# sweeneychris/TheiaSfM

Hardware: NVIDIA H100
Metric: observations/s = N_obs x LM iterations / solve time (10k-cam / 2M-pt / 20M-obs BA, ITERATIVE_SCHUR + SCHUR_JACOBI) (higher is better)
Workload: dtype f64

## Files before the change

### include/theia_ba_b200.h

```cpp
#ifndef THEIA_BA_B200_H_
#define THEIA_BA_B200_H_

#include <stdint.h>

#ifdef __cplusplus
extern "C" {
#endif

#define TBA_EXT_SIZE 6
#define TBA_INTR_STRIDE 10
#define TBA_PT_SIZE 4

enum { TBA_MODEL_PINHOLE = 0, TBA_MODEL_PINHOLE_RADIAL_TANGENTIAL = 1, TBA_MODEL_FISHEYE = 2, TBA_MODEL_FOV = 3,
       TBA_MODEL_DIVISION_UNDISTORTION = 4 };
#define TBA_MODEL_NUM_PARAMETERS(model) \
  ((model) == 0 ? 7 : (model) == 1 ? 10 : (model) == 2 ? 9 : ((model) == 3 || (model) == 4) ? 5 : -1)

enum { TBA_LOSS_TRIVIAL = 0, TBA_LOSS_HUBER = 1, TBA_LOSS_SOFTLONE = 2,
       TBA_LOSS_CAUCHY = 3, TBA_LOSS_ARCTAN = 4, TBA_LOSS_TUKEY = 5 };

enum { TBA_INTR_NONE = 0x00, TBA_INTR_FOCAL_LENGTH = 0x01,
       TBA_INTR_ASPECT_RATIO = 0x02, TBA_INTR_SKEW = 0x04,
       TBA_INTR_PRINCIPAL_POINTS = 0x08, TBA_INTR_RADIAL_DISTORTION = 0x10,
       TBA_INTR_TANGENTIAL_DISTORTION = 0x20, TBA_INTR_ALL = 0x3f };
// ... 101 lines not shown

int tba_device_count(void);

int tba_create(int device, int rank, int world_size, const void* nccl_unique_id,
               tba_context** out);
void tba_destroy(tba_context* ctx);
int tba_nccl_unique_id(void* out_128_bytes);
const char* tba_last_error(tba_context* ctx);

int tba_solve(tba_context* ctx, const tba_options* options,
              tba_problem* problem, tba_summary* summary);

int tba_solve_multi(const tba_options* options, tba_problem* problem, tba_summary* summary, int n_devices);

int tba_upload(tba_context* ctx, const tba_options* options, const tba_problem* problem);
int tba_minimize(tba_context* ctx, tba_summary* summary);
int tba_download(tba_context* ctx, tba_problem* problem);

int tba_filter_tracks(tba_context* ctx, double max_inlier_reprojection_error, double min_triangulation_angle_degrees,
                      uint8_t* status, double* mean_sq_error, int32_t* num_bad_reprojections, int32_t* num_insufficient_angles);

int tba_adjust_tracks(tba_context* ctx, const tba_options* options, uint8_t* status, double* initial_cost, double* final_cost,
                      int32_t* num_failed);
int tba_estimate_tracks(tba_context* ctx, const tba_options* ba_options, double max_acceptable_reprojection_error_pixels,
                        double min_triangulation_angle_degrees, int32_t bundle_adjustment, uint8_t* status, int32_t counts[5]);
enum { TBA_TRACK_ESTIMATED = 0, TBA_TRACK_BAD_ANGLE = 1, TBA_TRACK_TRIANGULATION_FAILED = 2, TBA_TRACK_BA_FAILED = 3,
       TBA_TRACK_BAD_REPROJECTION = 4, TBA_TRACK_SKIPPED = 255 };

int tba_adjust_views(tba_context* ctx, const tba_options* options, const int32_t* views, int32_t n_views, uint8_t* status,
                     double* initial_cost, double* final_cost, int32_t* iterations);

typedef struct tba_two_view_batch {
  int32_t n_pairs;
  const int64_t* pair_off;
  const double* ext1;
  double* ext2;
  double* intr1;
  double* intr2;
  const int32_t* model1;
  const int32_t* model2;
  const uint8_t* constant_intrinsics1;
  const uint8_t* constant_intrinsics2;
  const double* xy1;
  const double* xy2;
  double* points;
  double final_max_reprojection_error_pixels;
  uint8_t* inlier;
} tba_two_view_batch;
int tba_two_view_ba_batch(tba_context* ctx, tba_two_view_batch* batch, uint8_t* termination, double* initial_cost, double* final_cost,
                          int32_t* iterations);
int tba_two_view_ba_batch_multi(tba_two_view_batch* batch, int n_devices, uint8_t* termination, double* initial_cost, double* final_cost,
                                int32_t* iterations);

int tba_reset_parameters(tba_context* ctx, const tba_problem* problem);
int tba_set_max_iterations(tba_context* ctx, int32_t max_num_iterations);

int tba_set_profiling(tba_context* ctx, int enable);
int tba_get_profile(tba_context* ctx, double* out8);
int tba_get_profile_stages(tba_context* ctx, double* out16);

void tba_shard_points(const int32_t* pt_num_obs, int32_t n_pt, int world_size,
                      int rank, int32_t* begin, int32_t* end);

enum { TBA_VEC_GRADIENT_CAM = 0,
       TBA_VEC_GRADIENT_INTR = 1,
       TBA_VEC_GRADIENT_PT = 2,
       TBA_VEC_COLNORM2_CAM = 3,
       TBA_VEC_COLNORM2_INTR = 4,
       TBA_VEC_COLNORM2_PT = 5,
       TBA_VEC_RESIDUALS = 6,
       TBA_VEC_SCHUR_RHS_CAM = 7,
       TBA_VEC_SCHUR_RHS_INTR = 8,
       TBA_VEC_PRECOND_CAM = 9,
       TBA_VEC_PRECOND_INTR = 10,
       TBA_VEC_STEP_CAM = 11,
       TBA_VEC_STEP_INTR = 12,
       TBA_VEC_STEP_PT = 13 };
int tba_debug_pack(const tba_problem* problem, int64_t cap_slots, int64_t* sizes_out, int32_t* slot_cam, int32_t* slot_pt,
                   int16_t* slot_run, uint8_t* slot_flags, double* xy, int64_t* slot_orig, int32_t* pk2caller,
                   int32_t* tile_pt_begin, int32_t* tile_nruns, uint8_t* tile_flags, double* mask);
int tba_debug_linearize(tba_context* ctx, double* cost);
int tba_debug_linearize_raw(tba_context* ctx, int tile_kernel, int64_t* sizes_out, double* J, double* res, double* Hpp,
                            double* gp, double* lin);
int tba_debug_stream_launch(tba_context* ctx, int32_t* out);
int tba_debug_prepare_linear_system(tba_context* ctx, double radius);
int tba_debug_schur_matvec(tba_context* ctx, const double* x_cam ,
                           const double* x_intr ,
                           double* y_cam, double* y_intr);
int tba_debug_solve_linear_system(tba_context* ctx, int32_t* cg_iterations,
                                  double* model_cost_change);
int tba_debug_evaluate_step(tba_context* ctx, double* candidate_cost);
int tba_debug_read(tba_context* ctx, int which, double* out, int64_t n);

#ifdef __cplusplus
}
#endif
#endif
```

### theiasfm_b200/csrc/tba_camera_models.cuh

```cuda
#pragma once
#include <cstdint>
#include <cfloat>

#include "tba_camera_models_ext.cuh"

#ifdef __CUDA_ARCH__
#define TBA_UNROLL _Pragma("unroll")
#else
#define TBA_UNROLL
#endif

namespace tba {

constexpr int kModelPinhole = 0;
constexpr int kModelRadTan = 1;

constexpr int kCamRec = 20;

__host__ __device__ constexpr int popcount10(uint32_t m) {
  int n = 0;
  for (int i = 0; i < 10; ++i) n += (m >> i) & 1u;
  return n;
}
__host__ __device__ constexpr int nth_bit(uint32_t m, int j) {
// ... 33 lines not shown
  R[3] = B01 + Sw2;       R[4] = c + B * w1 * w1; R[5] = B12 - Sw0;
  R[6] = B02 - Sw1;       R[7] = B12 + Sw0;       R[8] = c + B * w2 * w2;
  const double th2 = w0 * w0 + w1 * w1 + w2 * w2;
  const double d = 1.0 - Cc * th2;
  const double Bw0 = B * w0, Bw1 = B * w1, Bw2 = B * w2;
  const double C01 = Cc * w0 * w1, C02 = Cc * w0 * w2, C12 = Cc * w1 * w2;
  L[0] = d + Cc * w0 * w0; L[1] = C01 - Bw2;        L[2] = C02 + Bw1;
  L[3] = C01 + Bw2;        L[4] = d + Cc * w1 * w1; L[5] = C12 - Bw0;
  L[6] = C02 - Bw1;        L[7] = C12 + Bw0;        L[8] = d + Cc * w2 * w2;
  rec[18] = B == 0.0 ? 1.0 : 0.0;
  rec[19] = 0.0;
}
__host__ __device__ inline void cam_prep(const double* __restrict__ w, double* __restrict__ rec, double* __restrict__ s4_out = nullptr) {
  double s4[4];
  cam_scalars(w, s4);
  cam_rec_expand(w[0], w[1], w[2], s4[0], s4[1], s4[2], s4[3], rec);
  if (s4_out) { s4_out[0] = s4[0]; s4_out[1] = s4[1]; s4_out[2] = s4[2]; s4_out[3] = s4[3]; }
}

__host__ __device__ inline void loss_evaluate(int type, double a, double s, double rho[3]) {
  switch (type) {
    case 1: {
      const double b = a * a;
      if (s > b) { const double r = sqrt(s); rho[0] = 2.0 * a * r - b; rho[1] = fmax(DBL_MIN, a / r); rho[2] = -rho[1] / (2.0 * s); }
      else { rho[0] = s; rho[1] = 1.0; rho[2] = 0.0; }
      break; }
    case 2: {
      const double b = a * a, c = 1.0 / b, sum = 1.0 + s * c, tmp = sqrt(sum);
      rho[0] = 2.0 * b * (tmp - 1.0); rho[1] = fmax(DBL_MIN, 1.0 / tmp); rho[2] = -(c * rho[1]) / (2.0 * sum);
      break; }
    case 3: {
      const double b = a * a, c = 1.0 / b, sum = 1.0 + s * c, inv = 1.0 / sum;
      rho[0] = b * log(sum); rho[1] = fmax(DBL_MIN, inv); rho[2] = -c * (inv * inv);
      break; }
    case 4: {
      const double b = 1.0 / (a * a), sum = 1.0 + s * s * b, inv = 1.0 / sum;
      rho[0] = a * atan2(s, a); rho[1] = fmax(DBL_MIN, inv); rho[2] = -2.0 * s * b * (inv * inv);
      break; }
    case 5: {
      const double a2 = a * a;
      if (s <= a2) { const double v = 1.0 - s / a2, v2 = v * v; rho[0] = a2 / 6.0 * (1.0 - v2 * v); rho[1] = 0.5 * v2; rho[2] = -1.0 / a2 * v; }
      else { rho[0] = a2 / 6.0; rho[1] = 0.0; rho[2] = 0.0; }
      break; }
    default: rho[0] = s; rho[1] = 1.0; rho[2] = 0.0;
  }
}

__host__ __device__ inline void project_pixel(int model, const double* __restrict__ C, const double* __restrict__ R,
                                     const double* __restrict__ k, const double X0, const double X1, const double X2, const double h,
                                     double& px, double& py, double& qz, double& a_sq) {
  const double a0 = X0 - h * C[0], a1 = X1 - h * C[1], a2 = X2 - h * C[2];
  a_sq = a0 * a0 + a1 * a1 + a2 * a2;
  const double q0 = R[0] * a0 + R[1] * a1 + R[2] * a2;
  const double q1 = R[3] * a0 + R[4] * a1 + R[5] * a2;
  const double q2 = R[6] * a0 + R[7] * a1 + R[8] * a2;
  qz = q2;
  const double u = q0 / q2, v = q1 / q2;
  const double r2 = u * u + v * v;
  double ud, vd;
  if (model == kModelPinhole) {
    const double d = 1.0 + r2 * (k[5] + k[6] * r2);
    ud = u * d; vd = v * d;
  } else {
    const double rd = 1.0 + k[5] * r2 + k[6] * r2 * r2 + k[7] * r2 * r2 * r2;
    const double tx = k[9] * (r2 + 2.0 * u * u) + 2.0 * k[8] * u * v;
    const double ty = k[8] * (r2 + 2.0 * v * v) + 2.0 * k[9] * u * v;
    ud = u * rd + tx; vd = v * rd + ty;
  }
  px = k[0] * ud + k[2] * vd + k[3];
  py = k[0] * k[1] * vd + k[4];
}

__host__ __device__ inline bool reproject(int model, const double* __restrict__ C, const double* __restrict__ R,
                                 const double* __restrict__ k, const double X0, const double X1, const double X2,
                                 const double h, const double x, const double y, double& r0, double& r1) {
  double px, py, qz, a_sq;
  project_pixel(model, C, R, k, X0, X1, X2, h, px, py, qz, a_sq);
  if (a_sq < 1e-8) return false;
  r0 = px - x;
  r1 = py - y;
  return true;
}

template <uint32_t IMASK>
__host__ __device__ inline bool linearize_obs(int model, const double* __restrict__ C, const double* __restrict__ rec,
                                     const double* __restrict__ k, const double X0, const double X1, const double X2,
                                     const double h, const double x, const double y, int loss_type, double loss_width,
                                     double r[2], double& rho0, double Ja[6], double Jw[6], double Jh[2], double* Ji) {
  constexpr int NI = popcount10(IMASK);
  const double* R = rec;
  const double* L = rec + 9;
  const bool small = rec[18] != 0.0;
  const double a0 = X0 - h * C[0], a1 = X1 - h * C[1], a2 = X2 - h * C[2];
  if (a0 * a0 + a1 * a1 + a2 * a2 < 1e-8) return false;
  const double q0 = R[0] * a0 + R[1] * a1 + R[2] * a2;
  const double q1 = R[3] * a0 + R[4] * a1 + R[5] * a2;
  const double q2 = R[6] * a0 + R[7] * a1 + R[8] * a2;
  const double iz = 1.0 / q2;
  const double u = q0 * iz, v = q1 * iz;
  const double r2 = u * u + v * v;
  double ud, vd, D00, D01, D10, D11;
  double dk[10][2];
  if (model == kModelPinhole) {
    const double d = 1.0 + r2 * (k[5] + k[6] * r2);
    const double dd = 2.0 * k[5] + 4.0 * k[6] * r2;
    ud = u * d; vd = v * d;
    D00 = d + u * u * dd; D01 = u * v * dd; D10 = D01; D11 = d + v * v * dd;
    dk[5][0] = r2 * u; dk[5][1] = r2 * v;
    dk[6][0] = r2 * r2 * u; dk[6][1] = r2 * r2 * v;
    dk[7][0] = dk[7][1] = dk[8][0] = dk[8][1] = dk[9][0] = dk[9][1] = 0.0;
  } else {
    const double r4 = r2 * r2;
    const double rd = 1.0 + k[5] * r2 + k[6] * r4 + k[7] * r4 * r2;
    const double rdp = k[5] + 2.0 * k[6] * r2 + 3.0 * k[7] * r4;
    const double t1 = k[8], t2 = k[9];
    ud = u * rd + t2 * (r2 + 2.0 * u * u) + 2.0 * t1 * u * v;
    vd = v * rd + t1 * (r2 + 2.0 * v * v) + 2.0 * t2 * u * v;
    D00 = rd + 2.0 * u * u * rdp + 6.0 * t2 * u + 2.0 * t1 * v;
    D01 = 2.0 * u * v * rdp + 2.0 * t2 * v + 2.0 * t1 * u;
    D10 = 2.0 * u * v * rdp + 2.0 * t1 * u + 2.0 * t2 * v;
    D11 = rd + 2.0 * v * v * rdp + 6.0 * t1 * v + 2.0 * t2 * u;
    dk[5][0] = r2 * u; dk[5][1] = r2 * v;
    dk[6][0] = r4 * u; dk[6][1] = r4 * v;
    dk[7][0] = r4 * r2 * u; dk[7][1] = r4 * r2 * v;
    dk[8][0] = 2.0 * u * v; dk[8][1] = r2 + 2.0 * v * v;
    dk[9][0] = r2 + 2.0 * u * u; dk[9][1] = 2.0 * u * v;
  }
  const double f = k[0], ar = k[1], sk = k[2];
  const double rr0 = f * ud + sk * vd + k[3] - x;
  const double rr1 = f * ar * vd + k[4] - y;
  const double s = rr0 * rr0 + rr1 * rr1;
  double rho[3];
  loss_evaluate(loss_type, loss_width, s, rho);
  rho0 = rho[0];
  const double sq = sqrt(rho[1]);
  double P00 = sq, P01 = 0.0, P10 = 0.0, P11 = sq, rscale = sq;
  if (!(s == 0.0 || rho[2] <= 0.0)) {
    const double Dd = 1.0 + 2.0 * s * rho[2] / rho[1];
    const double alpha = 1.0 - sqrt(Dd);
    rscale = sq / (1.0 - alpha);
    const double an = alpha / s;
    P00 = sq * (1.0 - an * rr0 * rr0); P01 = -sq * an * rr0 * rr1; P10 = P01; P11 = sq * (1.0 - an * rr1 * rr1);
  }
  r[0] = rr0 * rscale; r[1] = rr1 * rscale;
  const double K00 = f * D00 + sk * D10, K01 = f * D01 + sk * D11;
  const double K10 = f * ar * D10, K11 = f * ar * D11;
  const double A00 = P00 * K00 + P01 * K10, A01 = P00 * K01 + P01 * K11;
  const double A10 = P10 * K00 + P11 * K10, A11 = P10 * K01 + P11 * K11;
  const double Jq00 = A00 * iz, Jq01 = A01 * iz, Jq02 = -(A00 * u + A01 * v) * iz;
  const double Jq10 = A10 * iz, Jq11 = A11 * iz, Jq12 = -(A10 * u + A11 * v) * iz;
  Ja[0] = Jq00 * R[0] + Jq01 * R[3] + Jq02 * R[6];
  Ja[1] = Jq00 * R[1] + Jq01 * R[4] + Jq02 * R[7];
  Ja[2] = Jq00 * R[2] + Jq01 * R[5] + Jq02 * R[8];
  Ja[3] = Jq10 * R[0] + Jq11 * R[3] + Jq12 * R[6];
  Ja[4] = Jq10 * R[1] + Jq11 * R[4] + Jq12 * R[7];
  Ja[5] = Jq10 * R[2] + Jq11 * R[5] + Jq12 * R[8];
  Jh[0] = -(Ja[0] * C[0] + Ja[1] * C[1] + Ja[2] * C[2]);
  Jh[1] = -(Ja[3] * C[0] + Ja[4] * C[1] + Ja[5] * C[2]);
  const double b0 = small ? a0 : q0, b1 = small ? a1 : q1, b2 = small ? a2 : q2;
  const double c00 = Jq01 * b2 - Jq02 * b1, c01 = Jq02 * b0 - Jq00 * b2, c02 = Jq00 * b1 - Jq01 * b0;
  const double c10 = Jq11 * b2 - Jq12 * b1, c11 = Jq12 * b0 - Jq10 * b2, c12 = Jq10 * b1 - Jq11 * b0;
  Jw[0] = -(c00 * L[0] + c01 * L[3] + c02 * L[6]);
  Jw[1] = -(c00 * L[1] + c01 * L[4] + c02 * L[7]);
  Jw[2] = -(c00 * L[2] + c01 * L[5] + c02 * L[8]);
  Jw[3] = -(c10 * L[0] + c11 * L[3] + c12 * L[6]);
  Jw[4] = -(c10 * L[1] + c11 * L[4] + c12 * L[7]);
  Jw[5] = -(c10 * L[2] + c11 * L[5] + c12 * L[8]);
  if (NI > 0) {
    double col[10][2];
    col[0][0] = ud;  col[0][1] = ar * vd;
    col[1][0] = 0.0; col[1][1] = f * vd;
    col[2][0] = vd;  col[2][1] = 0.0;
    col[3][0] = 1.0; col[3][1] = 0.0;
    col[4][0] = 0.0; col[4][1] = 1.0;
    TBA_UNROLL
    for (int j = 5; j < 10; ++j) {
      col[j][0] = f * dk[j][0] + sk * dk[j][1];
      col[j][1] = f * ar * dk[j][1];
    }
    TBA_UNROLL
    for (int j = 0; j < NI; ++j) {
      constexpr uint32_t M = IMASK;
      const int idx = nth_bit(M, j);
      Ji[j] = P00 * col[idx][0] + P01 * col[idx][1];
      Ji[NI + j] = P10 * col[idx][0] + P11 * col[idx][1];
    }
  }
  return true;
}

__host__ __device__ inline void project_pixel_ext(int model, const double* __restrict__ C, const double* __restrict__ R,
                                                  const double* __restrict__ k, const double X0, const double X1, const double X2, const double h,
                                                  double& px, double& py, double& qz, double& a_sq) {
  const double a0 = X0 - h * C[0], a1 = X1 - h * C[1], a2 = X2 - h * C[2];
  a_sq = a0 * a0 + a1 * a1 + a2 * a2;
  double q[3], pix[2];
  q[0] = R[0] * a0 + R[1] * a1 + R[2] * a2;
  q[1] = R[3] * a0 + R[4] * a1 + R[5] * a2;
  q[2] = R[6] * a0 + R[7] * a1 + R[8] * a2;
  qz = q[2];
  camera_to_pixel_ext<double>(model, k, q, pix);
  px = pix[0]; py = pix[1];
}

template <uint32_t IMASK>
__host__ __device__ inline bool linearize_obs_ext(int model, const double* __restrict__ C, const double* __restrict__ rec,
                                                  const double* __restrict__ k, const double X0, const double X1, const double X2,
                                                  const double h, const double x, const double y, int loss_type, double loss_width,
                                                  double r[2], double& rho0, double Ja[6], double Jw[6], double Jh[2], double* Ji) {
  constexpr int NI = popcount10(IMASK);
  const double* R = rec;
  const double* L = rec + 9;
  const bool small = rec[18] != 0.0;
  const double a0 = X0 - h * C[0], a1 = X1 - h * C[1], a2 = X2 - h * C[2];
  if (a0 * a0 + a1 * a1 + a2 * a2 < 1e-8) return false;
  const double q0 = R[0] * a0 + R[1] * a1 + R[2] * a2;
  const double q1 = R[3] * a0 + R[4] * a1 + R[5] * a2;
  const double q2 = R[6] * a0 + R[7] * a1 + R[8] * a2;
  typedef Dual<13> D;
  D qd[3], kd[10], pix[2];
  const double qv[3] = {q0, q1, q2};
  for (int i = 0; i < 3; ++i) { qd[i].v = qv[i]; for (int j = 0; j < 13; ++j) qd[i].d[j] = 0.0; qd[i].d[i] = 1.0; }
  const int K = model_num_parameters(model);
  for (int i = 0; i < 10; ++i) { kd[i].v = i < K ? k[i] : 0.0; for (int j = 0; j < 13; ++j) kd[i].d[j] = 0.0; if (i < K) kd[i].d[3 + i] = 1.0; }
  camera_to_pixel_ext<D>(model, kd, qd, pix);
  const double rr0 = pix[0].v - x, rr1 = pix[1].v - y;
  const double s = rr0 * rr0 + rr1 * rr1;
  double rho[3];
  loss_evaluate(loss_type, loss_width, s, rho);
  rho0 = rho[0];
  const double sq = sqrt(rho[1]);
  double P00 = sq, P01 = 0.0, P10 = 0.0, P11 = sq, rscale = sq;
  if (!(s == 0.0 || rho[2] <= 0.0)) {
    const double Dd = 1.0 + 2.0 * s * rho[2] / rho[1];
    const double alpha = 1.0 - sqrt(Dd);
    rscale = sq / (1.0 - alpha);
    const double an = alpha / s;
    P00 = sq * (1.0 - an * rr0 * rr0); P01 = -sq * an * rr0 * rr1; P10 = P01; P11 = sq * (1.0 - an * rr1 * rr1);
  }
  r[0] = rr0 * rscale; r[1] = rr1 * rscale;
  const double Jq00 = P00 * pix[0].d[0] + P01 * pix[1].d[0], Jq01 = P00 * pix[0].d[1] + P01 * pix[1].d[1], Jq02 = P00 * pix[0].d[2] + P01 * pix[1].d[2];
  const double Jq10 = P10 * pix[0].d[0] + P11 * pix[1].d[0], Jq11 = P10 * pix[0].d[1] + P11 * pix[1].d[1], Jq12 = P10 * pix[0].d[2] + P11 * pix[1].d[2];
  Ja[0] = Jq00 * R[0] + Jq01 * R[3] + Jq02 * R[6];
  Ja[1] = Jq00 * R[1] + Jq01 * R[4] + Jq02 * R[7];
  Ja[2] = Jq00 * R[2] + Jq01 * R[5] + Jq02 * R[8];
  Ja[3] = Jq10 * R[0] + Jq11 * R[3] + Jq12 * R[6];
  Ja[4] = Jq10 * R[1] + Jq11 * R[4] + Jq12 * R[7];
  Ja[5] = Jq10 * R[2] + Jq11 * R[5] + Jq12 * R[8];
  Jh[0] = -(Ja[0] * C[0] + Ja[1] * C[1] + Ja[2] * C[2]);
  Jh[1] = -(Ja[3] * C[0] + Ja[4] * C[1] + Ja[5] * C[2]);
  const double b0 = small ? a0 : q0, b1 = small ? a1 : q1, b2 = small ? a2 : q2;
  const double c00 = Jq01 * b2 - Jq02 * b1, c01 = Jq02 * b0 - Jq00 * b2, c02 = Jq00 * b1 - Jq01 * b0;
  const double c10 = Jq11 * b2 - Jq12 * b1, c11 = Jq12 * b0 - Jq10 * b2, c12 = Jq10 * b1 - Jq11 * b0;
  Jw[0] = -(c00 * L[0] + c01 * L[3] + c02 * L[6]);
  Jw[1] = -(c00 * L[1] + c01 * L[4] + c02 * L[7]);
  Jw[2] = -(c00 * L[2] + c01 * L[5] + c02 * L[8]);
  Jw[3] = -(c10 * L[0] + c11 * L[3] + c12 * L[6]);
  Jw[4] = -(c10 * L[1] + c11 * L[4] + c12 * L[7]);
  Jw[5] = -(c10 * L[2] + c11 * L[5] + c12 * L[8]);
  if (NI > 0) {
    TBA_UNROLL
    for (int j = 0; j < NI; ++j) {
      constexpr uint32_t M = IMASK;
      const int idx = nth_bit(M, j);
      Ji[j] = P00 * pix[0].d[3 + idx] + P01 * pix[1].d[3 + idx];
      Ji[NI + j] = P10 * pix[0].d[3 + idx] + P11 * pix[1].d[3 + idx];
    }
  }
  return true;
}

template <bool EXT>
__host__ __device__ inline void project_pixel_any(int model, const double* __restrict__ C, const double* __restrict__ R,
                                                  const double* __restrict__ k, const double X0, const double X1, const double X2, const double h,
                                                  double& px, double& py, double& qz, double& a_sq) {
  if (EXT) {
    if (model >= kModelFisheye) { project_pixel_ext(model, C, R, k, X0, X1, X2, h, px, py, qz, a_sq); return; }
  }
  project_pixel(model, C, R, k, X0, X1, X2, h, px, py, qz, a_sq);
}
template <bool EXT>
__host__ __device__ inline bool reproject_any(int model, const double* __restrict__ C, const double* __restrict__ R,
                                              const double* __restrict__ k, const double X0, const double X1, const double X2,
                                              const double h, const double x, const double y, double& r0, double& r1) {
  if (EXT) {
    if (model >= kModelFisheye) {
      double px, py, qz, a_sq;
      project_pixel_ext(model, C, R, k, X0, X1, X2, h, px, py, qz, a_sq);
      if (a_sq < 1e-8) return false;
      r0 = px - x; r1 = py - y;
      return true;
    }
  }
  return reproject(model, C, R, k, X0, X1, X2, h, x, y, r0, r1);
}
template <uint32_t IMASK, bool EXT>
__host__ __device__ inline bool linearize_obs_any(int model, const double* __restrict__ C, const double* __restrict__ rec,
                                                  const double* __restrict__ k, const double X0, const double X1, const double X2,
                                                  const double h, const double x, const double y, int loss_type, double loss_width,
                                                  double r[2], double& rho0, double Ja[6], double Jw[6], double Jh[2], double* Ji) {
  if (EXT) {
    if (model >= kModelFisheye) return linearize_obs_ext<IMASK>(model, C, rec, k, X0, X1, X2, h, x, y, loss_type, loss_width, r, rho0, Ja, Jw, Jh, Ji);
  }
  return linearize_obs<IMASK>(model, C, rec, k, X0, X1, X2, h, x, y, loss_type, loss_width, r, rho0, Ja, Jw, Jh, Ji);
}

}
```

### theiasfm_b200/csrc/tba_engine.cu

```cuda
#include <dlfcn.h>
#include <nccl.h>
#include <unistd.h>

#include <algorithm>
#include <chrono>
#include <condition_variable>
#include <cmath>
#include <cstdarg>
#include <cstdio>
#include <cstdlib>
#include <cstring>
#include <atomic>
#include <mutex>
#include <thread>
#include <string>
#include <vector>

#include "../../include/theia_ba_b200.h"
#include "tba_kernels.cuh"
#include "tba_pack.h"
#include "tba_block_lm.h"

namespace tba {

// ... 131 lines not shown
  PcgState* h_st = nullptr;
};

namespace {

void set_err(tba_context* c, const char* fmt, ...) {
  char buf[512];
  va_list ap;
  va_start(ap, fmt);
  vsnprintf(buf, sizeof buf, fmt, ap);
  va_end(ap);
  c->err = buf;
}

#define CUDA_OK(c, expr)                                                                        \
  do {                                                                                          \
    cudaError_t e__ = (expr);                                                                   \
    if (e__ != cudaSuccess) {                                                                   \
      set_err(c, "CUDA error %s at %s:%d (%s)", cudaGetErrorString(e__), __FILE__, __LINE__, #expr); \
      return TBA_ERR_CUDA;                                                                      \
    }                                                                                           \
  } while (0)

#define NCCL_OK(c, expr)                                                                        \
  do {                                                                                          \
    ncclResult_t r__ = (expr);                                                                  \
    if (r__ != ncclSuccess) {                                                                   \
      set_err(c, "NCCL error %s at %s:%d", g_nccl.GetErrorString(r__), __FILE__, __LINE__);     \
      return TBA_ERR_NCCL;                                                                      \
    }                                                                                           \
  } while (0)

#ifdef TBA_EMULATE
#define LAUNCH(c, kern, grid, block, smem, ...)                                              \
  do {                                                                                       \
    if ((unsigned)(grid) == 0u) break;                             \
    emu::launch((const void*)(kern), (unsigned)(grid), (unsigned)(block), (size_t)(smem), [&] { kern(__VA_ARGS__); }); \
    if (cudaGetLastError() != cudaSuccess) {                                                 \
      set_err(c, "kernel launch failed: invalid configuration at %s:%d (%s)", __FILE__, __LINE__, #kern); \
      return TBA_ERR_CUDA;                                                                   \
    }                                                                                        \
    (c)->launches++;                                                                         \
  } while (0)
#else
#define LAUNCH(c, kern, grid, block, smem, ...)                                                              \
  do {                                                                                                       \
    if ((unsigned)(grid) == 0u) break;  \
    kern<<<(grid), (block), (smem), (c)->stream>>>(__VA_ARGS__);                                             \
    const cudaError_t le__ = cudaPeekAtLastError();                                                          \
    if (le__ != cudaSuccess) {                                                                               \
      set_err(c, "kernel launch failed: %s at %s:%d (%s)", cudaGetErrorString(le__), __FILE__, __LINE__, #kern); \
      return TBA_ERR_CUDA;                                                                                   \
    }                                                                                                        \
    (c)->launches++;                                                                                         \
  } while (0)
#endif

int prof_begin(tba_context* c) {
  if (!c->profiling) return -1;
  cudaEvent_t e;
  if (cudaEventCreate(&e) != cudaSuccess) return -1;
  c->ev_pool.push_back(e);
  cudaEventRecord(e, c->stream);
  return (int)c->ev_pool.size() - 1;
}
void prof_end(tba_context* c, int which, int begin) {
  if (begin < 0) return;
  cudaEvent_t e;
  if (cudaEventCreate(&e) != cudaSuccess) return;
  c->ev_pool.push_back(e);
  cudaEventRecord(e, c->stream);
  c->ev_spans[which].push_back({begin, (int)c->ev_pool.size() - 1});
}

const uint32_t kMasks[] = {0x000u, 0x001u, 0x061u, 0x0E1u, 0x07Fu, 0x3FFu};

#define DISPATCH_IMASK(mask, F) \
  switch (mask) {               \
    case 0x000u: F(0x000u); break; \
    case 0x001u: F(0x001u); break; \
    case 0x061u: F(0x061u); break; \
    case 0x0E1u: F(0x0E1u); break; \
    case 0x07Fu: F(0x07Fu); break; \
    default: F(0x3FFu); break;  \
  }

int allreduce_sum(tba_context* c, double* buf, size_t n) {
  if (c->world == 1) return TBA_OK;
  NCCL_OK(c, g_nccl.AllReduce(buf, buf, n, ncclDouble, ncclSum, c->comm, c->stream));
  return TBA_OK;
}
size_t schur_smem(const tba_context* c) { return (size_t)(c->NJ + 2) * TILE * sizeof(double); }

double* lin_g(tba_context* c) { return c->lin.p; }
double* lin_cn(tba_context* c) { return c->lin.p + c->P.ncs; }
double* lin_scal(tba_context* c) { return c->lin.p + 2 * (size_t)c->P.ncs; }
int small_grid(const tba_context* c, int64_t n_items) { return (int)std::max<int64_t>(1, std::min<int64_t>((n_items + 255) / 256, (int64_t)c->n_sm * 8)); }
int stream_grid(const tba_context* c, int n_slices, int NW) { return std::max(1, std::min(c->n_sm, (n_slices + NW - 1) / NW)); }

int read_scal(tba_context* c, const double* dev, int n, double* out) {
  CUDA_OK(c, cudaMemcpyAsync(c->h_scal, dev, n * sizeof(double), cudaMemcpyDeviceToHost, c->stream));
  CUDA_OK(c, cudaStreamSynchronize(c->stream));
  memcpy(out, c->h_scal, n * sizeof(double));
  return TBA_OK;
}

int stage_linearize(tba_context* c, double* cost, double* fixed, bool* ok, double* gmax = nullptr, bool tile_kernel = false) {
  DevProblem& P = c->P;
  const size_t n_lin = 2 * (size_t)P.ncs + 16 + (size_t)c->world;
  CUDA_OK(c, cudaMemsetAsync(c->lin.p, 0, n_lin * sizeof(double), c->stream));
  LAUNCH(c, k_cam_prep, (P.n_cam + 127) / 128, 128, 0, P.n_cam, P.ext, P.cam_rec, P.cam_s4);
  if (P.n_tiles > 0) {
    const int pb = prof_begin(c);
    if (c->has_ext_models) {
      auto kfn = k_linearize<0x3FFu, true>;
      LAUNCH(c, kfn, P.n_tiles, TILE, 0, P, lin_g(c), lin_cn(c), c->rep.p, 0);
    } else {
      int first_tile = 0;
      if (c->n_normal_tiles > 0 && !tile_kernel) {
        const int n_slices = c->n_normal_tiles * (TILE / 32);
#define F(M) { using Cfg = LinCfg<M>; auto kfn = k_linearize_stream<M>; \
               const int grid = stream_grid(c, n_slices, Cfg::NW); \
               LAUNCH(c, kfn, grid, Cfg::NW * 32, Cfg::SMEM, P, lin_g(c), lin_cn(c), c->rep.p, n_slices); }
        DISPATCH_IMASK(c->imask, F)
#undef F
        first_tile = c->n_normal_tiles;
      }
      const int rest = P.n_tiles - first_tile;
#define F(M) { auto kfn = k_linearize<M, false>; LAUNCH(c, kfn, rest, TILE, 0, P, lin_g(c), lin_cn(c), c->rep.p, first_tile); }
      DISPATCH_IMASK(c->imask, F)
#undef F
    }
    prof_end(c, 1, pb);
    LAUNCH(c, k_fold, 1, REPW, 0, c->rep.p, lin_g(c) + P.ne, lin_cn(c) + P.ne, lin_scal(c));
  }
  if (gmax && P.n_pt > 0) LAUNCH(c, k_gradmax_pt, small_grid(c, P.n_pt), 256, 0, P, lin_scal(c) + 16 + c->rank);
  int rc = allreduce_sum(c, c->lin.p, n_lin);
  if (rc) return rc;
  if (gmax) LAUNCH(c, k_gradmax_cs, VB, VT, 0, P.ncs, lin_g(c), c->mask.p, lin_scal(c) + 16, c->world, lin_scal(c) + 3);
  if (!c->have_scale) {
    LAUNCH(c, k_cs_scale, VB, VT, 0, P.ncs, lin_cn(c), c->mask.p, c->opt.jacobi_scaling, c->sm.p);
    if (P.n_pt > 0) LAUNCH(c, k_point_scale, (P.n_pt + 255) / 256, 256, 0, P, c->opt.jacobi_scaling);
    c->have_scale = true;
  }
  double s[4];
  rc = read_scal(c, lin_scal(c), 4, s);
  if (rc) return rc;
  *cost = s[0]; *fixed = s[1]; *ok = s[2] == 0.0;
  if (gmax) *gmax = s[3];
  return TBA_OK;
}

void p2p_release(tba_context* c) {
#ifndef TBA_EMULATE
  for (void* q : c->p2p_opened) cudaIpcCloseMemHandle(q);
#endif
  c->p2p_opened.clear();
  if (c->p2p_inbox) cudaFree(c->p2p_inbox);
  if (c->p2p_flags) cudaFree(c->p2p_flags);
  if (c->p2p_ctr) cudaFree(c->p2p_ctr);
  c->p2p_inbox = nullptr; c->p2p_flags = nullptr; c->p2p_ctr = nullptr; c->p2p_cap = 0; c->p2p_ok = false;
}

#ifndef TBA_EMULATE
struct P2pInfo {
  long long pid;
// ... 601 lines not shown
  c->opt = *options;
  if (options->linear_solver_type != TBA_ITERATIVE_SCHUR) {
    c->opt.eta = 1e-13;
    c->opt.min_linear_solver_iterations = 0;
    c->opt.max_linear_solver_iterations = std::max(c->opt.max_linear_solver_iterations, 2000);
    c->opt.preconditioner_type = TBA_PRECOND_SCHUR_JACOBI;
  }
  const int nc = p->n_cam, ng = p->n_group, np = p->n_pt;
  const int64_t no = p->n_obs;
  if (nc < 0 || ng < 0 || np < 0 || no < 0) { set_err(c, "negative sizes"); return TBA_ERR_INVALID_ARGUMENT; }
  c->has_ext_models = false;
  for (int g = 0; g < ng; ++g) {
    if (TBA_MODEL_NUM_PARAMETERS(p->group_model[g]) < 0) {
      set_err(c, "camera intrinsics model %d of group %d is not a CameraIntrinsicsModelType (0..4)", p->group_model[g], g);
      return TBA_ERR_UNSUPPORTED;
    }
    if (p->group_model[g] >= TBA_MODEL_FISHEYE) c->has_ext_models = true;
  }
  for (int i = 0; i < nc; ++i) if (p->cam_group[i] < 0 || p->cam_group[i] >= ng) { set_err(c, "cam_group out of range"); return TBA_ERR_INVALID_ARGUMENT; }
  const int T = std::max(1, std::min<int>(64, (int)std::thread::hardware_concurrency() / std::max(1, c->world)));
  HostPack& H = c->pack;
  c->slot_orig.clear();
  const bool trace = getenv("TBA_UPLOAD_TRACE") != nullptr;
  auto t_prev = std::chrono::steady_clock::now();
  auto lap = [&](const char* what) {
    if (!trace) return;
    auto t = std::chrono::steady_clock::now();
    fprintf(stderr, "[tba_upload r%d] %-28s %8.2f ms\n", c->rank, what, std::chrono::duration<double, std::milli>(t - t_prev).count());
    t_prev = t;
  };
  pack_count_and_sort(p, T, &H);
  lap("count_and_sort (A-C)");
  int local_err = TBA_OK;
  if (H.bad >= 0) { set_err(c, "observation %lld references camera %d / point %d out of range", (long long)H.bad, p->obs_cam[H.bad], p->obs_pt[H.bad]); local_err = TBA_ERR_INVALID_ARGUMENT; }
  else if (H.maxlen > TILE) { set_err(c, "track with %d observations exceeds the engine limit of %d per track", H.maxlen, TILE); local_err = TBA_ERR_UNSUPPORTED; }
  const bool collective_upload = c->world > 1 && c->preset_cnt_cam == nullptr;
  if (local_err != TBA_OK && !collective_upload) return local_err;
  if (local_err == TBA_OK) pack_points(p, &H);
  lap("pack_points");
  std::vector<double> cnt_c(nc, 0.0), cnt_g(ng, 0.0);
  if (local_err == TBA_OK) for (int i = 0; i < nc; ++i) { cnt_c[i] = H.cnt_cam[i]; cnt_g[p->cam_group[i]] += H.cnt_cam[i]; }
  c->n_free_pt = local_err == TBA_OK ? H.n_free_pt : 0;
  c->n_free_pt_global = c->n_free_pt;
  if (c->world > 1 && c->preset_cnt_cam != nullptr) {
    std::fill(cnt_g.begin(), cnt_g.end(), 0.0);
    for (int i = 0; i < nc; ++i) { cnt_c[i] = c->preset_cnt_cam[i]; cnt_g[p->cam_group[i]] += cnt_c[i]; }
    c->n_free_pt_global = c->preset_free_pt;
  } else if (c->world > 1) {
    std::vector<double> tmp(cnt_c);
    tmp.insert(tmp.end(), cnt_g.begin(), cnt_g.end());
    tmp.push_back((double)c->n_free_pt);
    tmp.push_back(local_err != TBA_OK ? 1.0 : 0.0);
    rc = [&]() -> int {
      CUDA_OK(c, c->scal2.alloc(std::max<size_t>(tmp.size(), 16)));
      CUDA_OK(c, cudaMemcpyAsync(c->scal2.p, tmp.data(), tmp.size() * 8, cudaMemcpyHostToDevice, c->stream));
      int r2 = allreduce_sum(c, c->scal2.p, tmp.size());
      if (r2) return r2;
      CUDA_OK(c, cudaMemcpyAsync(tmp.data(), c->scal2.p, tmp.size() * 8, cudaMemcpyDeviceToHost, c->stream));
      CUDA_OK(c, cudaStreamSynchronize(c->stream));
      return TBA_OK;
    }();
    if (rc) return rc;
    if (tmp.back() != 0.0) {
      if (local_err == TBA_OK) { set_err(c, "upload failed on %d other rank(s) (invalid observation indices or over-long track in their shard)", (int)tmp.back()); return TBA_ERR_INVALID_ARGUMENT; }
      return local_err;
    }
    std::copy(tmp.begin(), tmp.begin() + nc, cnt_c.begin());
    std::copy(tmp.begin() + nc, tmp.begin() + nc + ng, cnt_g.begin());
    c->n_free_pt_global = (int64_t)tmp[tmp.size() - 2];
  }
  pack_masks_and_tiles(p, cnt_c, cnt_g, &H);
  lap("masks_and_tiles (D)");
  const int ne = nc * 6, ncs = ne + ng * 10;
  const std::vector<double>& mask = H.mask;
  const std::vector<double>& blk_free = H.blk_free;
  std::vector<int>& tile_pt_begin = H.tile_pt_begin;
  std::vector<int>& tile_nruns = H.tile_nruns;
  std::vector<uint8_t>& tile_flags = H.tile_flags;
  c->n_free_cs = H.n_free_cs;
  c->imask = 0x3FFu;
  for (uint32_t m : kMasks) if ((H.union_free & ~m) == 0) { c->imask = m; break; }
  if (c->has_ext_models) c->imask = 0x3FFu;
  c->NI = popcount10(c->imask);
  c->NJ = 14 + 2 * c->NI;
  const int npk = (int)H.pk2caller.size();
  const int n_long = H.n_long;
  const int n_tiles = H.n_tiles;
  const int64_t n_slots = H.n_slots;
  const size_t stage_bytes = (size_t)n_slots * (4 + 4 + 2 + 1 + 16) + (size_t)npk * (32 + 1 + 8 + 4) + 10 * 256;
  if (c->stage_cap < stage_bytes) {
    if (c->stage) cudaFreeHost(c->stage);
    c->stage = nullptr; c->stage_cap = 0;
    CUDA_OK(c, cudaMallocHost(&c->stage, stage_bytes + stage_bytes / 8));
    c->stage_cap = stage_bytes + stage_bytes / 8;
  }
  uint8_t* sp8 = (uint8_t*)c->stage;
  auto carve = [&](size_t bytes) { uint8_t* r0 = sp8; sp8 += (bytes + 255) / 256 * 256; return r0; };
  double* h_xy = (double*)carve((size_t)n_slots * 16);
  double* h_pt = (double*)carve((size_t)npk * 32);
  int* h_slot_cam = (int*)carve((size_t)n_slots * 4);
  int* h_slot_pt = (int*)carve((size_t)n_slots * 4);
  int16_t* h_slot_run = (int16_t*)carve((size_t)n_slots * 2);
  uint8_t* h_slot_flags = carve((size_t)n_slots);
  uint8_t* h_pt_const = carve((size_t)npk);
  long long* h_pt_slot = (long long*)carve((size_t)npk * 8);
  int* h_pt_len = (int*)carve((size_t)npk * 4);
  lap("staging");
  PackDest d;
  d.xy = h_xy; d.pt = h_pt; d.slot_cam = h_slot_cam; d.slot_pt = h_slot_pt; d.slot_run = h_slot_run; d.slot_flags = h_slot_flags;
  d.pt_const = h_pt_const; d.slot_orig = nullptr;
  c->n_long_points = n_long;
  c->n_cam = nc; c->n_group = ng; c->n_pt = npk; c->n_pt_caller = np; c->n_tiles = n_tiles; c->n_obs = no; c->n_slots = n_slots;
  const int npd = npk;
  c->h2d_bytes = 0; c->d2h_bytes = 0; c->launches = 0;
#define ALLOC(buf, n) CUDA_OK(c, c->buf.alloc(n))
  ALLOC(ext, (size_t)ne); ALLOC(ext_c, (size_t)ne); ALLOC(intr, (size_t)ng * 10); ALLOC(intr_c, (size_t)ng * 10);
  ALLOC(pt, (size_t)npd * 4); ALLOC(pt_c, (size_t)npd * 4); ALLOC(cam_rec, (size_t)nc * kCamRec); ALLOC(cam_rec_c, (size_t)nc * kCamRec); ALLOC(cam_s4, (size_t)nc * 4); ALLOC(cam_s4_c, (size_t)nc * 4);
  ALLOC(xy, (size_t)n_slots * 2); ALLOC(J, (size_t)n_slots * c->NJ); ALLOC(res, (size_t)n_slots * 2);
  ALLOC(Hpp, (size_t)npd * 10); ALLOC(gp, (size_t)npd * 4); ALLOC(Mp, (size_t)npd * 10); ALLOC(sp, (size_t)npd * 4); ALLOC(dpt, (size_t)npd * 4);
  ALLOC(cam_group, (size_t)nc); ALLOC(group_model, (size_t)ng); ALLOC(slot_cam, (size_t)n_slots); ALLOC(slot_pt, (size_t)n_slots);
  ALLOC(tile_pt_begin, (size_t)n_tiles + 1); ALLOC(tile_nruns, (size_t)n_tiles); ALLOC(slot_flags, (size_t)n_slots);
  ALLOC(slot_run, (size_t)n_slots); ALLOC(pt_const, (size_t)npd); ALLOC(tile_flags, (size_t)n_tiles);
  ALLOC(pt_slot, (size_t)npd); ALLOC(pt_len, (size_t)npd); ALLOC(pt_stat, (size_t)npd);
  ALLOC(lin, 2 * (size_t)ncs + 16 + (size_t)std::max(1, c->world)); ALLOC(mask, (size_t)ncs); ALLOC(blk_free, (size_t)nc + ng); ALLOC(sm, (size_t)ncs); ALLOC(D2, (size_t)ncs);
  ALLOC(Sblk, (size_t)nc * 21 + (size_t)ng * 55 + 2 + (size_t)ncs); ALLOC(Minv_c, (size_t)nc * 36); ALLOC(Minv_i, (size_t)ng * 100);
  ALLOC(b, (size_t)ncs); ALLOC(x, (size_t)ncs); ALLOC(r, (size_t)ncs); ALLOC(p, (size_t)ncs); ALLOC(z, (size_t)ncs); ALLOC(z2, (size_t)ncs); ALLOC(xs, (size_t)ncs); ALLOC(y, (size_t)ncs);
  ALLOC(part, 3 * VB); ALLOC(gmax, 2); ALLOC(flag, 1); ALLOC(scal2, std::max<size_t>(16, (size_t)nc + ng)); ALLOC(st, 2); ALLOC(done_flag, 1); ALLOC(pcg_bar, 2); ALLOC(rep, (size_t)NREP * REPW);
#undef ALLOC
  lap("device alloc");
#define H2D(buf, src, n)                                                                                      \
  do {                                                                                                        \
    CUDA_OK(c, cudaMemcpyAsync(c->buf.p, (src), (n) * sizeof(*c->buf.p), cudaMemcpyHostToDevice, c->stream)); \
    c->h2d_bytes += (double)((n) * sizeof(*c->buf.p));                                                        \
  } while (0)
  H2D(ext, p->ext, (size_t)ne); H2D(intr, p->intr, (size_t)ng * 10);
  H2D(ext_c, p->ext, (size_t)ne); H2D(intr_c, p->intr, (size_t)ng * 10);
  H2D(cam_group, p->cam_group, (size_t)nc); H2D(group_model, p->group_model, (size_t)ng);
  H2D(tile_pt_begin, tile_pt_begin.data(), (size_t)n_tiles + 1); H2D(tile_nruns, tile_nruns.data(), (size_t)n_tiles);
  H2D(tile_flags, tile_flags.data(), (size_t)n_tiles);
  CUDA_OK(c, cudaMemsetAsync(c->rep.p, 0, (size_t)NREP * REPW * sizeof(double), c->stream));
  CUDA_OK(c, cudaMemsetAsync(c->pcg_bar.p, 0, 2 * sizeof(int), c->stream));
  CUDA_OK(c, cudaMemsetAsync(c->J.p, 0, (size_t)n_slots * c->NJ * sizeof(double), c->stream));
  CUDA_OK(c, cudaMemsetAsync(c->dpt.p, 0, (size_t)npd * 4 * sizeof(double), c->stream));
  CUDA_OK(c, cudaMemsetAsync(c->Mp.p, 0, (size_t)npd * 10 * sizeof(double), c->stream));
  CUDA_OK(c, cudaMemsetAsync(c->Hpp.p, 0, (size_t)npd * 10 * sizeof(double), c->stream));
  CUDA_OK(c, cudaMemsetAsync(c->gp.p, 0, (size_t)npd * 4 * sizeof(double), c->stream));
  CUDA_OK(c, cudaMemsetAsync(c->Minv_c.p, 0, (size_t)nc * 36 * sizeof(double), c->stream));
  CUDA_OK(c, cudaMemsetAsync(c->Minv_i.p, 0, (size_t)ng * 100 * sizeof(double), c->stream));
  {
    int n_chunks = n_tiles >= 32768 ? 16 : n_tiles >= 8192 ? 8 : 1;
    if (const char* e = getenv("TBA_UPLOAD_CHUNKS")) n_chunks = std::max(1, std::min(atoi(e), std::max(1, n_tiles)));
#define H2D_RANGE(buf, src, off, n)                                                                                              \
  do {                                                                                                                           \
    if ((n) > 0) {                                                                                                               \
      CUDA_OK(c, cudaMemcpyAsync(c->buf.p + (off), (src) + (off), (n) * sizeof(*c->buf.p), cudaMemcpyHostToDevice, c->stream));  \
      c->h2d_bytes += (double)((n) * sizeof(*c->buf.p));                                                                         \
    }                                                                                                                            \
  } while (0)
    for (int ch = 0; ch < n_chunks; ++ch) {
      const int64_t t0 = (int64_t)n_tiles * ch / n_chunks, t1 = (int64_t)n_tiles * (ch + 1) / n_chunks;
      if (t1 <= t0) continue;
      pack_fill(p, H, T, d, t0, t1);
      const size_t s0 = (size_t)t0 * TILE, ns = (size_t)(t1 - t0) * TILE;
      const size_t q0 = (size_t)tile_pt_begin[t0], nq = (size_t)tile_pt_begin[t1] - q0;
      H2D_RANGE(slot_cam, h_slot_cam, s0, ns); H2D_RANGE(slot_pt, h_slot_pt, s0, ns);
      H2D_RANGE(slot_flags, h_slot_flags, s0, ns); H2D_RANGE(slot_run, h_slot_run, s0, ns);
      H2D_RANGE(xy, h_xy, s0 * 2, ns * 2);
// ... 750 lines not shown
    });
  for (auto& t : th) t.join();
  for (int r = 0; r < n_devices; ++r)
    if (sh[r].rc != TBA_OK) { *summary = sh[r].s; summary->iterations = itbuf; summary->iterations_capacity = itcap; return sh[r].rc; }
  memcpy(problem->ext, sh[0].ext.data(), (size_t)problem->n_cam * 48);
  memcpy(problem->intr, sh[0].intr.data(), (size_t)problem->n_group * 80);
  for (int r = 0; r < n_devices; ++r) memcpy(problem->pt + (size_t)sh[r].b * 4, sh[r].pt.data(), (size_t)(sh[r].e - sh[r].b) * 32);
  *summary = sh[0].s;
  for (int r = 1; r < n_devices; ++r) {
    summary->num_kernel_launches += sh[r].s.num_kernel_launches;
    summary->h2d_bytes += sh[r].s.h2d_bytes;
    summary->d2h_bytes += sh[r].s.d2h_bytes;
    summary->setup_time_in_seconds = std::max(summary->setup_time_in_seconds, sh[r].s.setup_time_in_seconds);
    summary->solve_time_in_seconds = std::max(summary->solve_time_in_seconds, sh[r].s.solve_time_in_seconds);
  }
  return TBA_OK;
}

int tba_debug_pack(const tba_problem* p, int64_t cap_slots, int64_t* sizes_out, int32_t* slot_cam, int32_t* slot_pt, int16_t* slot_run,
                   uint8_t* slot_flags, double* xy, int64_t* slot_orig, int32_t* pk2caller, int32_t* tile_pt_begin,
                   int32_t* tile_nruns, uint8_t* tile_flags, double* mask) {
  if (!p || !sizes_out) return TBA_ERR_INVALID_ARGUMENT;
  for (int i = 0; i < p->n_cam; ++i) if (p->cam_group[i] < 0 || p->cam_group[i] >= p->n_group) return TBA_ERR_INVALID_ARGUMENT;
  static std::mutex mu;
  static HostPack H;
  std::lock_guard<std::mutex> lk(mu);
  pack_count_and_sort(p, 4, &H);
  if (H.bad >= 0) return TBA_ERR_INVALID_ARGUMENT;
  if (H.maxlen > TILE) return TBA_ERR_UNSUPPORTED;
  pack_points(p, &H);
  std::vector<double> cnt_c(p->n_cam, 0.0), cnt_g(p->n_group, 0.0);
  for (int i = 0; i < p->n_cam; ++i) { cnt_c[i] = H.cnt_cam[i]; cnt_g[p->cam_group[i]] += H.cnt_cam[i]; }
  pack_masks_and_tiles(p, cnt_c, cnt_g, &H);
  uint32_t imask = 0x3FFu;
  for (uint32_t m : kMasks) if ((H.union_free & ~m) == 0) { imask = m; break; }
  sizes_out[0] = H.n_tiles; sizes_out[1] = H.n_slots; sizes_out[2] = (int64_t)H.pk2caller.size(); sizes_out[3] = H.n_long;
  sizes_out[4] = popcount10(imask); sizes_out[5] = imask;
  if (H.n_slots > cap_slots) return TBA_ERR_INVALID_ARGUMENT;
  std::vector<double> pt((size_t)H.pk2caller.size() * 4);
  std::vector<uint8_t> ptc(H.pk2caller.size());
  for (int64_t s = 0; s < H.n_slots; ++s) slot_orig[s] = -1;
  PackDest d;
  d.xy = xy; d.pt = pt.data(); d.slot_cam = slot_cam; d.slot_pt = slot_pt; d.slot_run = slot_run; d.slot_flags = slot_flags;
  d.pt_const = ptc.data(); d.slot_orig = slot_orig;
  pack_fill(p, H, 4, d);
  for (size_t k = 0; k < H.pk2caller.size(); ++k) pk2caller[k] = H.pk2caller[k];
  for (int t = 0; t <= H.n_tiles; ++t) tile_pt_begin[t] = H.tile_pt_begin[t];
  for (int t = 0; t < H.n_tiles; ++t) { tile_nruns[t] = H.tile_nruns[t]; tile_flags[t] = H.tile_flags[t]; }
  for (size_t i = 0; i < H.mask.size(); ++i) mask[i] = H.mask[i];
  return TBA_OK;
}

int tba_debug_linearize(tba_context* c, double* cost) {
  if (!c || !c->uploaded) return TBA_ERR_INVALID_ARGUMENT;
  CUDA_OK(c, cudaSetDevice(c->device));
  bool ok;
  double x, f;
  int rc = stage_linearize(c, &x, &f, &ok);
  if (rc) return rc;
  c->x_cost = x; c->fixed_cost = f;
  if (cost) *cost = x + f;
  return ok ? TBA_OK : TBA_ERR_INVALID_ARGUMENT;
}

int tba_debug_linearize_raw(tba_context* c, int tile_kernel, int64_t* sizes_out, double* J, double* res, double* Hpp, double* gp, double* lin) {
  if (!c || !c->uploaded || !sizes_out) return TBA_ERR_INVALID_ARGUMENT;
  CUDA_OK(c, cudaSetDevice(c->device));
  const DevProblem& P = c->P;
  sizes_out[0] = c->n_slots; sizes_out[1] = c->NJ; sizes_out[2] = P.n_pt; sizes_out[3] = P.ncs;
  if (!J || !res || !Hpp || !gp || !lin) return TBA_OK;
  bool ok;
  double x, f;
  const int rc = stage_linearize(c, &x, &f, &ok, nullptr, tile_kernel != 0);
  if (rc) return rc;
  CUDA_OK(c, cudaMemcpyAsync(J, P.J, (size_t)c->n_slots * c->NJ * 8, cudaMemcpyDeviceToHost, c->stream));
  CUDA_OK(c, cudaMemcpyAsync(res, P.res, (size_t)c->n_slots * 2 * 8, cudaMemcpyDeviceToHost, c->stream));
  CUDA_OK(c, cudaMemcpyAsync(Hpp, P.Hpp, (size_t)P.n_pt * 10 * 8, cudaMemcpyDeviceToHost, c->stream));
  CUDA_OK(c, cudaMemcpyAsync(gp, P.gp, (size_t)P.n_pt * 4 * 8, cudaMemcpyDeviceToHost, c->stream));
  CUDA_OK(c, cudaMemcpyAsync(lin, c->lin.p, (2 * (size_t)P.ncs + 3) * 8, cudaMemcpyDeviceToHost, c->stream));
  CUDA_OK(c, cudaStreamSynchronize(c->stream));
  return TBA_OK;
}

int tba_debug_stream_launch(tba_context* c, int32_t* out) {
  if (!c || !c->uploaded || !out) return TBA_ERR_INVALID_ARGUMENT;
  const int n_slices = c->n_normal_tiles * (TILE / 32);
  out[0] = c->n_sm; out[1] = n_slices; out[2] = (int32_t)c->imask; out[3] = c->has_ext_models ? 1 : 0;
  auto put = [&](int k, int NW, int NS) { out[4 + 3 * k] = stream_grid(c, n_slices, NW); out[5 + 3 * k] = NW; out[6 + 3 * k] = NS; };
#define F(M) { put(0, LinCfg<M>::NW, LinCfg<M>::NS); put(1, PrepCfg<M>::NW, PrepCfg<M>::NS); \
               put(2, StreamCfg<M, 0>::NW, StreamCfg<M, 0>::NS); put(3, StreamCfg<M, 1>::NW, StreamCfg<M, 1>::NS); }
  DISPATCH_IMASK(c->imask, F)
#undef F
  return TBA_OK;
}

int tba_debug_prepare_linear_system(tba_context* c, double radius) {
  if (!c || !c->uploaded) return TBA_ERR_INVALID_ARGUMENT;
  CUDA_OK(c, cudaSetDevice(c->device));
  bool ok;
  int rc = stage_prepare(c, radius, &ok);
  if (rc) return rc;
  return ok ? TBA_OK : TBA_ERR_INVALID_ARGUMENT;
}

int tba_debug_schur_matvec(tba_context* c, const double* x_cam, const double* x_intr, double* y_cam, double* y_intr) {
  if (!c || !c->uploaded) return TBA_ERR_INVALID_ARGUMENT;
  CUDA_OK(c, cudaSetDevice(c->device));
  DevProblem& P = c->P;
  CUDA_OK(c, cudaMemcpyAsync(c->p.p, x_cam, (size_t)P.ne * 8, cudaMemcpyHostToDevice, c->stream));
  CUDA_OK(c, cudaMemcpyAsync(c->p.p + P.ne, x_intr, (size_t)P.n_group * 10 * 8, cudaMemcpyHostToDevice, c->stream));
  LAUNCH(c, k_cs_mul, VB, VT, 0, P.ncs, c->sm.p, c->p.p, c->xs.p);
  CUDA_OK(c, cudaMemsetAsync(c->y.p, 0, (size_t)P.ncs * 8, c->stream));
  LAUNCH(c, k_set_flag, 1, 1, 0, c->done_flag.p, 0);
  int rc = launch_matvec(c, c->done_flag.p);
  if (rc) return rc;
  LAUNCH(c, k_set_flag, 1, 1, 0, const_cast<int*>(st_done(c->st.p)), 0);
  PcgVectors V = pcg_vectors(c);
  V.fold_rep = nullptr;
  int cur = 0;
  rc = launch_pcg(c, V, cur, PCG_A, 0, p2p_none());
  if (rc) return rc;
  CUDA_OK(c, cudaMemcpyAsync(y_cam, c->z.p, (size_t)P.ne * 8, cudaMemcpyDeviceToHost, c->stream));
  CUDA_OK(c, cudaMemcpyAsync(y_intr, c->z.p + P.ne, (size_t)P.n_group * 10 * 8, cudaMemcpyDeviceToHost, c->stream));
  CUDA_OK(c, cudaStreamSynchronize(c->stream));
  return TBA_OK;
}

int tba_debug_solve_linear_system(tba_context* c, int32_t* cg_iterations, double* model_cost_change) {
  if (!c || !c->uploaded) return TBA_ERR_INVALID_ARGUMENT;
  CUDA_OK(c, cudaSetDevice(c->device));
  int iters = 0, status = 0;
  int rc = stage_pcg(c, &iters, &status);
  if (rc) return rc;
  rc = stage_backsub(c);
  if (rc) return rc;
  int r2 = allreduce_sum(c, c->scal2.p + 3, 1);
  if (r2) return r2;
  double s[8];
  rc = read_scal(c, c->scal2.p, 8, s);
  if (rc) return rc;
  if (cg_iterations) *cg_iterations = iters;
  if (model_cost_change) *model_cost_change = s[3];
  return status == 2 ? TBA_ERR_INVALID_ARGUMENT : TBA_OK;
}

int tba_debug_evaluate_step(tba_context* c, double* candidate_cost) {
  if (!c || !c->uploaded) return TBA_ERR_INVALID_ARGUMENT;
  CUDA_OK(c, cudaSetDevice(c->device));
  DevProblem& P = c->P;
  CUDA_OK(c, cudaMemsetAsync(c->scal2.p, 0, 3 * sizeof(double), c->stream));
  LAUNCH(c, k_cam_prep, (P.n_cam + 127) / 128, 128, 0, P.n_cam, P.ext_c, P.cam_rec_c, P.cam_s4_c);
  if (P.n_tiles > 0) {
    if (c->has_ext_models) { auto kfn = k_cost<true>; LAUNCH(c, kfn, P.n_tiles, TILE, 0, P, P.ext_c, P.cam_s4_c, P.intr_c, P.pt_c, c->rep.p); }
    else { auto kfn = k_cost<false>; LAUNCH(c, kfn, P.n_tiles, TILE, 0, P, P.ext_c, P.cam_s4_c, P.intr_c, P.pt_c, c->rep.p); }
    LAUNCH(c, k_fold, 1, REPW, 0, c->rep.p, nullptr, nullptr, c->scal2.p);
  }
  int rc = allreduce_sum(c, c->scal2.p, 3);
  if (rc) return rc;
  double s[3];
  rc = read_scal(c, c->scal2.p, 3, s);
  if (rc) return rc;
  if (candidate_cost) *candidate_cost = s[0] + s[1];
  return s[2] == 0.0 ? TBA_OK : TBA_ERR_INVALID_ARGUMENT;
}

int tba_debug_read(tba_context* c, int which, double* out, int64_t n) {
  if (!c || !c->uploaded || !out) return TBA_ERR_INVALID_ARGUMENT;
  CUDA_OK(c, cudaSetDevice(c->device));
  DevProblem& P = c->P;
  const int64_t ne = P.ne, ni = (int64_t)P.n_group * 10, np4 = (int64_t)P.n_pt * 4;
// ... 63 lines not shown
```

### theiasfm_b200/csrc/tba_kernels.cuh

```cuda
#pragma once
#include <cstdint>
#include <cuda_runtime.h>

#include "tba_camera_models.cuh"
#include "tba_segments.h"
#include "tba_filter.cuh"
#include "tba_track_estimator.cuh"
#include "tba_two_view.cuh"
#include "tba_view_ba.cuh"

namespace tba {

constexpr int TILE = 256;
constexpr int MAXP = 256;
constexpr int VB = 64;
constexpr int VT = 256;

struct DevProblem {
  int n_cam, n_group, n_pt, n_tiles;
  int ne;
  int ncs;
  int single_group;
  int loss_type; double loss_width;
  int ablate;
  double *ext, *intr, *pt, *ext_c, *intr_c, *pt_c;
  const int* cam_group; const int* group_model;
  double* cam_rec;
  double* cam_rec_c;
  double* cam_s4;
  double* cam_s4_c;
  const int* slot_cam;
  const int* slot_pt;
  const uint8_t* slot_flags;
  const int16_t* slot_run;
  const int* tile_pt_begin;
  const int* tile_nruns;
  const uint8_t* tile_flags;
  const double* xy;
  double* J;
  double* res;
  double* Hpp;
  double* gp;
  double* Mp;
  double* sp;
  double* dpt;
  const uint8_t* pt_const;
};

__device__ __forceinline__ double warp_sum(double v) {
#pragma unroll
  for (int o = 16; o > 0; o >>= 1) v += __shfl_down_sync(0xffffffffu, v, o);
  return v;
}

__device__ __forceinline__ double block_sum(double v, double* s_red ) {
  const int lane = threadIdx.x & 31, wid = threadIdx.x >> 5;
  v = warp_sum(v);
  __syncthreads();
  if (lane == 0) s_red[wid] = v;
  __syncthreads();
  double t = 0.0;
  if (wid == 0) {
    t = lane < (blockDim.x >> 5) ? s_red[lane] : 0.0;
    t = warp_sum(t);
  }
  return t;
}

__device__ __forceinline__ double seg_reduce(double v, int key, int lane) {
#pragma unroll
  for (int o = 1; o < 32; o <<= 1) {
    const double ov = __shfl_down_sync(0xffffffffu, v, o);
    const int ok = __shfl_down_sync(0xffffffffu, key, o);
    if (lane + o < 32 && ok == key) v += ov;
  }
  return v;
}

__device__ __forceinline__ double seg_reduce_to(double v, int run_last, int lane) {
#pragma unroll
  for (int o = 1; o < 32; o <<= 1) {
    const double ov = __shfl_down_sync(0xffffffffu, v, o);
    if (lane + o <= run_last) v += ov;
  }
  return v;
}

__device__ __forceinline__ void red_add(double* p, double v) {
#ifdef TBA_EMULATE
  atomicAdd(p, v);
#else
  asm volatile("red.global.add.f64 [%0], %1;" ::"l"(p), "d"(v) : "memory");
#endif
}

template <int N>
__device__ __forceinline__ void warp_stage_row(double* __restrict__ stage, int* __restrict__ sbase, const double (&v)[N], int base, int lane) {
#pragma unroll
  for (int j = 0; j < N; ++j) stage[lane * N + j] = v[j];
  sbase[lane] = base;
}
template <int N>
__device__ __forceinline__ void warp_red_rows(double* __restrict__ dst, const double* __restrict__ stage, const int* __restrict__ sbase, int lane) {
#pragma unroll
  for (int k = 0; k < N; ++k) {
    const int e = k * 32 + lane;
    const int o = e / N;
    const int b = sbase[o];
    if (b >= 0) red_add(dst + (size_t)b + (e - o * N), stage[e]);
  }
}

__global__ void k_cam_prep(int n_cam, const double* __restrict__ ext, double* __restrict__ rec, double* __restrict__ s4 = nullptr) {
  const int c = blockIdx.x * blockDim.x + threadIdx.x;
  if (c < n_cam) cam_prep(ext + (size_t)c * 6 + 3, rec + (size_t)c * kCamRec, s4 ? s4 + (size_t)c * 4 : nullptr);
}
__device__ __forceinline__ void gather_camera(const double* __restrict__ ext, const double* __restrict__ s4, int cam, double Cw[6], double rec[kCamRec]) {
  const double2* e2 = reinterpret_cast<const double2*>(ext + (size_t)cam * 6);
  const double2 e0 = __ldg(e2), e1 = __ldg(e2 + 1), e3 = __ldg(e2 + 2);
  const double2* q2 = reinterpret_cast<const double2*>(s4 + (size_t)cam * 4);
  const double2 q0 = __ldg(q2), q1 = __ldg(q2 + 1);
  Cw[0] = e0.x; Cw[1] = e0.y; Cw[2] = e1.x; Cw[3] = e1.y; Cw[4] = e3.x; Cw[5] = e3.y;
  cam_rec_expand(e1.y, e3.x, e3.y, q0.x, q0.y, q1.x, q1.y, rec);
}

constexpr int NREP = 256;
constexpr int REPW = 32;
__device__ __forceinline__ double* rep_row(double* rep) {
  return rep + (size_t)((blockIdx.x * (TILE / 32) + (threadIdx.x >> 5)) & (NREP - 1)) * REPW;
}
__global__ void k_fold(double* __restrict__ rep, double* __restrict__ dst_a, double* __restrict__ dst_b, double* __restrict__ dst_s) {
  const int j = threadIdx.x;
  if (j >= REPW) return;
  double v = 0.0;
  for (int r = 0; r < NREP; ++r) { v += rep[(size_t)r * REPW + j]; rep[(size_t)r * REPW + j] = 0.0; }
  if (j < 10) { if (dst_a) dst_a[j] += v; }
  else if (j < 20) { if (dst_b) dst_b[j - 10] += v; }
  else if (j < 24) { if (dst_s) dst_s[j - 20] += v; }
}

__device__ __forceinline__ int run_head_lane(unsigned heads, int lane) { return 31 - __clz(heads & (0xffffffffu >> (31 - lane))); }

__device__ __forceinline__ size_t wslice(int tile, int warp, int rows) { return ((size_t)tile * (TILE / 32) + warp) * rows * 32; }

__device__ __forceinline__ void sym4_mul(const double* __restrict__ M, const double t[4], double u[4]) {
  u[0] = M[0] * t[0] + M[1] * t[1] + M[2] * t[2] + M[3] * t[3];
  u[1] = M[1] * t[0] + M[4] * t[1] + M[5] * t[2] + M[6] * t[3];
  u[2] = M[2] * t[0] + M[5] * t[1] + M[7] * t[2] + M[8] * t[3];
  u[3] = M[3] * t[0] + M[6] * t[1] + M[8] * t[2] + M[9] * t[3];
}


template <int NI, int SP, int SC>
__device__ __forceinline__ void obs_apply_F(const double* ja, const double* jw, const double* ji, double h, double2 xa, double2 xb,
                                            double2 xc, const double* xi, double& w0, double& w1) {
  w0 = -h * (ja[0] * xa.x + ja[SP] * xa.y + ja[2 * SP] * xb.x) + jw[0] * xb.y + jw[SC] * xc.x + jw[2 * SC] * xc.y;
  w1 = -h * (ja[3 * SP] * xa.x + ja[4 * SP] * xa.y + ja[5 * SP] * xb.x) + jw[3 * SC] * xb.y + jw[4 * SC] * xc.x + jw[5 * SC] * xc.y;
#pragma unroll
  for (int j = 0; j < NI; ++j) { w0 += ji[j * SC] * xi[j]; w1 += ji[(NI + j) * SC] * xi[j]; }
}
template <int SP>
__device__ __forceinline__ void obs_JpT(const double* ja, const double* jh, double w0, double w1, double t[4]) {
  t[0] = ja[0] * w0 + ja[3 * SP] * w1; t[1] = ja[SP] * w0 + ja[4 * SP] * w1; t[2] = ja[2 * SP] * w0 + ja[5 * SP] * w1;
  t[3] = jh[0] * w0 + jh[SP] * w1;
}
template <int SP>
__device__ __forceinline__ void obs_sub_Jp(const double* ja, const double* jh, double w0, double w1, const double u[4], double& z0, double& z1) {
  z0 = w0 - (ja[0] * u[0] + ja[SP] * u[1] + ja[2 * SP] * u[2] + jh[0] * u[3]);
  z1 = w1 - (ja[3 * SP] * u[0] + ja[4 * SP] * u[1] + ja[5 * SP] * u[2] + jh[SP] * u[3]);
}
template <int SP, int SC>
__device__ __forceinline__ void obs_JcT(const double* ja, const double* jw, double h, double z0, double z1, double y[6]) {
#pragma unroll
  for (int j = 0; j < 3; ++j) y[j] = -h * (ja[j * SP] * z0 + ja[(3 + j) * SP] * z1);
#pragma unroll
  for (int j = 0; j < 3; ++j) y[3 + j] = jw[j * SC] * z0 + jw[(3 + j) * SC] * z1;
}
template <int NI, int SC>
__device__ __forceinline__ void obs_JiT(const double* ji, double z0, double z1, double y[]) {
#pragma unroll
  for (int j = 0; j < NI; ++j) y[j] = ji[j * SC] * z0 + ji[(NI + j) * SC] * z1;
}
__device__ __forceinline__ double obs_model_cost_change(double r0, double r1, double z0, double z1) {
  const double m0 = -(r0 - z0), m1 = -(r1 - z1);
  return -(m0 * (r0 + 0.5 * m0) + m1 * (r1 + 0.5 * m1));
}
__device__ __forceinline__ void obs_cam_block(const double* __restrict__ M, const double ja[6], const double jh[2], const double jw[6], double h,
                                              double v[21]) {
  const double jp0[4] = {ja[0], ja[1], ja[2], jh[0]}, jp1[4] = {ja[3], ja[4], ja[5], jh[1]};
  double m0[4], m1[4];
  sym4_mul(M, jp0, m0);
  sym4_mul(M, jp1, m1);
  const double q00 = 1.0 - (jp0[0] * m0[0] + jp0[1] * m0[1] + jp0[2] * m0[2] + jp0[3] * m0[3]);
  const double q01 = -(jp0[0] * m1[0] + jp0[1] * m1[1] + jp0[2] * m1[2] + jp0[3] * m1[3]);
  const double q11 = 1.0 - (jp1[0] * m1[0] + jp1[1] * m1[1] + jp1[2] * m1[2] + jp1[3] * m1[3]);
  double c0[6], c1[6];
#pragma unroll
  for (int j = 0; j < 3; ++j) { c0[j] = -h * ja[j]; c1[j] = -h * ja[3 + j]; c0[3 + j] = jw[j]; c1[3 + j] = jw[3 + j]; }
  int n = 0;
#pragma unroll
  for (int a = 0; a < 6; ++a) {
    const double qa0 = q00 * c0[a] + q01 * c1[a], qa1 = q01 * c0[a] + q11 * c1[a];
#pragma unroll
    for (int b = a; b < 6; ++b) { v[n] = qa0 * c0[b] + qa1 * c1[b]; ++n; }
  }
}
template <int NI>
__device__ __forceinline__ void obs_JiT_Ji(const double* ji, double g[]) {
  int n = 0;
#pragma unroll
  for (int a = 0; a < NI; ++a)
#pragma unroll
    for (int b = a; b < NI; ++b) { g[n] = ji[a] * ji[b] + ji[NI + a] * ji[NI + b]; ++n; }
}
template <int NI>
__device__ __forceinline__ void run_WT_M_W(const double* __restrict__ M, const double* W, double sub[]) {
  double MW[4][NI + 1];
#pragma unroll
  for (int j = 0; j < NI; ++j) {
    const double t[4] = {W[0 * NI + j], W[1 * NI + j], W[2 * NI + j], W[3 * NI + j]};
    double u[4];
    sym4_mul(M, t, u);
    MW[0][j] = u[0]; MW[1][j] = u[1]; MW[2][j] = u[2]; MW[3][j] = u[3];
  }
  int n = 0;
#pragma unroll
  for (int a = 0; a < NI; ++a)
#pragma unroll
    for (int b = a; b < NI; ++b) {
      sub[n] = W[0 * NI + a] * MW[0][b] + W[1 * NI + a] * MW[1][b] + W[2 * NI + a] * MW[2][b] + W[3 * NI + a] * MW[3][b];
      ++n;
    }
}
__device__ __forceinline__ int tri10(int ia, int ib) { return ia * 10 - ia * (ia - 1) / 2 + (ib - ia); }

template <int NI>
__device__ __forceinline__ void obs_settle(bool ok, bool is_fixed, double rho0, double& cost, double& fixed, double& failed, double Ja[6],
                                           double Jw[6], double Jh[2], double Ji[], double r[2]) {
  if (!ok) failed += 1.0;
  else if (is_fixed) fixed += 0.5 * rho0;
  else cost += 0.5 * rho0;
  if (!ok || is_fixed) {
#pragma unroll
    for (int j = 0; j < 6; ++j) { Ja[j] = 0.0; Jw[j] = 0.0; }
    Jh[0] = Jh[1] = 0.0; r[0] = r[1] = 0.0;
#pragma unroll
    for (int j = 0; j < 2 * NI; ++j) Ji[j] = 0.0;
  }
}
template <int NI>
__device__ __forceinline__ void obs_store(double* Jt, double* rt, const double Ja[6], const double Jw[6], const double Jh[2], const double Ji[],
                                          const double r[2]) {
#pragma unroll
  for (int j = 0; j < 6; ++j) Jt[j * 32] = Ja[j];
#pragma unroll
  for (int j = 0; j < 6; ++j) Jt[(6 + j) * 32] = Jw[j];
  Jt[12 * 32] = Jh[0];
  Jt[13 * 32] = Jh[1];
#pragma unroll
  for (int j = 0; j < 2 * NI; ++j) Jt[(14 + j) * 32] = Ji[j];
  rt[0] = r[0];
  rt[32] = r[1];
}
__device__ __forceinline__ void obs_point_terms(const double Ja[6], const double Jh[2], const double r[2], double acc[14]) {
  const double jp0[4] = {Ja[0], Ja[1], Ja[2], Jh[0]}, jp1[4] = {Ja[3], Ja[4], Ja[5], Jh[1]};
  int n = 0;
#pragma unroll
  for (int a = 0; a < 4; ++a)
#pragma unroll
    for (int b = a; b < 4; ++b) acc[n++] = jp0[a] * jp0[b] + jp1[a] * jp1[b];
#pragma unroll
  for (int a = 0; a < 4; ++a) acc[10 + a] = jp0[a] * r[0] + jp1[a] * r[1];
}
__device__ __forceinline__ void obs_cam_grad(const double Ja[6], const double Jw[6], double h, const double r[2], double g[6], double cn[6]) {
#pragma unroll
  for (int j = 0; j < 3; ++j) {
    const double c0 = -h * Ja[j], c1 = -h * Ja[3 + j];
    g[j] = c0 * r[0] + c1 * r[1];
    cn[j] = c0 * c0 + c1 * c1;
    g[3 + j] = Jw[j] * r[0] + Jw[3 + j] * r[1];
    cn[3 + j] = Jw[j] * Jw[j] + Jw[3 + j] * Jw[3 + j];
  }
}
template <int NI>
__device__ __forceinline__ void obs_intr_grad(const double Ji[], const double r[2], int j, double& g, double& cn) {
  g = Ji[j] * r[0] + Ji[NI + j] * r[1];
  cn = Ji[j] * Ji[j] + Ji[NI + j] * Ji[NI + j];
}

template <uint32_t IMASK, bool EXT = false>
__global__ void __launch_bounds__(TILE, EXT ? 1 : 3) k_linearize(DevProblem P, double* __restrict__ g_cs, double* __restrict__ cn_cs,
                                                           double* __restrict__ rep, int tile0) {
  constexpr bool STAGED_RED = !EXT;
  constexpr int NI = popcount10(IMASK);
  constexpr int NJ = 14 + 2 * NI;
  __shared__ double s_acc[MAXP][14];
  const int tile = tile0 + blockIdx.x, tid = threadIdx.x, lane = tid & 31, warp = tid >> 5;
  const bool long_tile = (P.tile_flags[tile] & 1) != 0;
  const int p0 = P.tile_pt_begin[tile], npt = P.tile_pt_begin[tile + 1] - p0;
  if (long_tile) {
    for (int i = tid; i < npt * 14; i += TILE) (&s_acc[0][0])[i] = 0.0;
    __syncthreads();
  }
  const size_t slot = (size_t)tile * TILE + tid;
  const int cam = P.slot_cam[slot];
  const bool valid = cam >= 0;
  double cost = 0.0, fixed = 0.0, failed = 0.0;
  double Ja[6] = {0, 0, 0, 0, 0, 0}, Jw[6] = {0, 0, 0, 0, 0, 0}, Jh[2] = {0, 0}, r[2] = {0, 0};
  double Ji[2 * NI + 1];
#pragma unroll
  for (int j = 0; j < 2 * NI; ++j) Ji[j] = 0.0;
  int pl = -1 - lane, grp = 0;
  double h = 0.0;
  if (valid) {
    const int pt = P.slot_pt[slot];
    pl = pt - p0;
    grp = P.cam_group[cam];
    const double4 X = *reinterpret_cast<const double4*>(P.pt + (size_t)pt * 4);
    h = X.w;
    const double* xyw = P.xy + wslice(tile, warp, 2) + lane;
    const double x = xyw[0], y = xyw[32];
    double rho0 = 0.0;
    double Cw[6], rec[kCamRec];
    gather_camera(P.ext, P.cam_s4, cam, Cw, rec);
    const bool ok = linearize_obs_any<IMASK, EXT>(P.group_model[grp], Cw, rec,
                                         P.intr + (size_t)grp * 10, X.x, X.y, X.z, X.w, x, y, P.loss_type, P.loss_width,
                                         r, rho0, Ja, Jw, Jh, Ji);
    obs_settle<NI>(ok, (P.slot_flags[slot] & 1) != 0, rho0, cost, fixed, failed, Ja, Jw, Jh, Ji, r);
  }
  obs_store<NI>(P.J + wslice(tile, warp, NJ) + lane, P.res + wslice(tile, warp, 2) + lane, Ja, Jw, Jh, Ji, r);
  {
    double acc[14];
    obs_point_terms(Ja, Jh, r, acc);
    const int prev = __shfl_up_sync(0xffffffffu, pl, 1);
    const bool head = valid && (lane == 0 || prev != pl);
#pragma unroll
    for (int j = 0; j < 14; ++j) acc[j] = seg_reduce(acc[j], pl, lane);
    if (head) {
      if (long_tile) {
#pragma unroll
        for (int j = 0; j < 14; ++j) atomicAdd(&s_acc[pl][j], acc[j]);
      } else {
        double2* H2 = reinterpret_cast<double2*>(P.Hpp + (size_t)(p0 + pl) * 10);
#pragma unroll
        for (int j = 0; j < 5; ++j) H2[j] = make_double2(acc[2 * j], acc[2 * j + 1]);
        double2* G2 = reinterpret_cast<double2*>(P.gp + (size_t)(p0 + pl) * 4);
        G2[0] = make_double2(acc[10], acc[11]);
        G2[1] = make_double2(acc[12], acc[13]);
      }
    }
  }
  double gv[6], cv[6];
  if (STAGED_RED && !long_tile) {
    obs_cam_grad(Ja, Jw, h, r, gv, cv);
    static_assert(MAXP * 14 >= (TILE / 32) * (2 * 32 * 6 + 16), "s_acc too small for the row staging");
    double* stage = &s_acc[0][0] + warp * (2 * 32 * 6 + 16);
    int* sbase = reinterpret_cast<int*>(stage + 2 * 32 * 6);
    warp_stage_row<6>(stage, sbase, gv, valid ? cam * 6 : -1, lane);
    warp_stage_row<6>(stage + 32 * 6, sbase, cv, valid ? cam * 6 : -1, lane);
    __syncwarp();
    warp_red_rows<6>(g_cs, stage, sbase, lane);
    warp_red_rows<6>(cn_cs, stage + 32 * 6, sbase, lane);
  } else if (valid) {
    obs_cam_grad(Ja, Jw, h, r, gv, cv);
#pragma unroll
    for (int j = 0; j < 6; ++j) {
      red_add(g_cs + (size_t)cam * 6 + j, gv[j]);
      red_add(cn_cs + (size_t)cam * 6 + j, cv[j]);
    }
  }
  double* rr = rep_row(rep);
  if (NI > 0) {
    double g, c;
    if (P.single_group) {
#pragma unroll
      for (int j = 0; j < NI; ++j) {
        obs_intr_grad<NI>(Ji, r, j, g, c);
        const double gsum = warp_sum(g);
        const double csum = warp_sum(c);
        if (lane == 0) { red_add(rr + nth_bit(IMASK, j), gsum); red_add(rr + 10 + nth_bit(IMASK, j), csum); }
      }
    } else if (valid) {
#pragma unroll
      for (int j = 0; j < NI; ++j) {
        obs_intr_grad<NI>(Ji, r, j, g, c);
        red_add(g_cs + P.ne + (size_t)grp * 10 + nth_bit(IMASK, j), g);
        red_add(cn_cs + P.ne + (size_t)grp * 10 + nth_bit(IMASK, j), c);
      }
    }
  }
  {
    const double c = warp_sum(cost), f = warp_sum(fixed), e = warp_sum(failed);
    if (lane == 0) {
      red_add(rr + 20, c);
      if (f != 0.0) red_add(rr + 21, f);
      if (e != 0.0) red_add(rr + 22, e);
    }
  }
  if (long_tile) {
    __syncthreads();
    for (int i = tid; i < npt * 14; i += TILE) {
      const int p = i / 14, j = i - p * 14;
      if (j < 10) P.Hpp[(size_t)(p0 + p) * 10 + j] = s_acc[p][j];
      else P.gp[(size_t)(p0 + p) * 4 + (j - 10)] = s_acc[p][j];
    }
  }
}

template <bool EXT = false>
__global__ void __launch_bounds__(TILE) k_cost(DevProblem P, const double* __restrict__ ext, const double* __restrict__ s4,
                                               const double* __restrict__ intr, const double* __restrict__ pt,
                                               double* __restrict__ rep) {
  const int tile = blockIdx.x, tid = threadIdx.x, lane = tid & 31, warp = tid >> 5;
// ... 166 lines not shown
  for (int j = 0; j < 4; ++j) P.sp[(size_t)p * 4 + j] = c ? 0.0 : (use_scaling ? 1.0 / (1.0 + sqrt(d[j])) : 1.0);
}

__global__ void k_point_blocks(DevProblem P, double radius, double lo, double hi, double* __restrict__ flag) {
  const int p = blockIdx.x * blockDim.x + threadIdx.x;
  if (p >= P.n_pt) return;
  double* M = P.Mp + (size_t)p * 10;
  if (P.pt_const[p]) {
#pragma unroll
    for (int j = 0; j < 10; ++j) M[j] = 0.0;
    return;
  }
  const double* H = P.Hpp + (size_t)p * 10;
  const double4 s4 = *reinterpret_cast<const double4*>(P.sp + (size_t)p * 4);
  const double s[4] = {s4.x, s4.y, s4.z, s4.w};
  double A[10], Ai[10];
  int n = 0;
#pragma unroll
  for (int a = 0; a < 4; ++a)
#pragma unroll
    for (int b = a; b < 4; ++b) { A[n] = s[a] * H[n] * s[b]; ++n; }
  const int dg[4] = {0, 4, 7, 9};
#pragma unroll
  for (int a = 0; a < 4; ++a) A[dg[a]] += fmin(fmax(A[dg[a]], lo), hi) / radius;
  if (!spd4_inverse(A, Ai)) {
    atomicAdd(flag, 1.0);
#pragma unroll
    for (int j = 0; j < 10; ++j) M[j] = 0.0;
    return;
  }
  n = 0;
#pragma unroll
  for (int a = 0; a < 4; ++a)
#pragma unroll
    for (int b = a; b < 4; ++b) { M[n] = s[a] * Ai[n] * s[b]; ++n; }
}

#ifdef TBA_EMULATE
__device__ __forceinline__ void mbar_init(uint64_t* bar, uint32_t) { *bar = 0; }
__device__ __forceinline__ void mbar_expect_tx(uint64_t* bar, uint32_t) { *bar += 1; }
__device__ __forceinline__ void bulk_g2s(void* dst, const void* src, uint32_t bytes, uint64_t*) { memcpy(dst, src, bytes); }
__device__ __forceinline__ void mbar_wait(uint64_t* bar, uint32_t parity) { while ((*bar & 1u) == parity) emu_yield(); }
__device__ __forceinline__ void fence_proxy_async_smem() {}
#else
__device__ __forceinline__ uint32_t smem_u32(const void* p) { return (uint32_t)__cvta_generic_to_shared(p); }
__device__ __forceinline__ void mbar_init(uint64_t* bar, uint32_t count) {
  asm volatile("mbarrier.init.shared::cta.b64 [%0], %1;" ::"r"(smem_u32(bar)), "r"(count) : "memory");
  asm volatile("fence.mbarrier_init.release.cluster;" ::: "memory");
}
__device__ __forceinline__ void mbar_expect_tx(uint64_t* bar, uint32_t bytes) {
  asm volatile("mbarrier.arrive.expect_tx.shared::cta.b64 _, [%0], %1;" ::"r"(smem_u32(bar)), "r"(bytes) : "memory");
}
__device__ __forceinline__ void bulk_g2s(void* dst, const void* src, uint32_t bytes, uint64_t* bar) {
  asm volatile("cp.async.bulk.shared::cluster.global.mbarrier::complete_tx::bytes [%0], [%1], %2, [%3];" ::"r"(smem_u32(dst)),
               "l"(src), "r"(bytes), "r"(smem_u32(bar))
               : "memory");
}
__device__ __forceinline__ bool mbar_try_wait(uint64_t* bar, uint32_t parity) {
  uint32_t ok;
  asm volatile(
      "{\n\t.reg .pred p;\n\t"
      "mbarrier.try_wait.parity.shared::cta.b64 p, [%1], %2;\n\t"
      "selp.u32 %0, 1, 0, p;\n\t}"
      : "=r"(ok)
      : "r"(smem_u32(bar)), "r"(parity)
      : "memory");
  return ok != 0;
}
__device__ __forceinline__ void mbar_wait(uint64_t* bar, uint32_t parity) {
  if (mbar_try_wait(bar, parity)) return;
  const long long t0 = clock64();
  while (!mbar_try_wait(bar, parity)) {
    if (clock64() - t0 > 4000000000ll) {
      printf("tba: mbarrier wait timed out (block %d thread %d parity %u)\n", (int)blockIdx.x, (int)threadIdx.x, parity);
      __trap();
    }
  }
}
__device__ __forceinline__ void fence_proxy_async_smem() { asm volatile("fence.proxy.async.shared::cta;" ::: "memory"); }

#endif

template <uint32_t IMASK, int MODE>
__global__ void __launch_bounds__(TILE, (14 + 2 * popcount10(IMASK)) <= 20 ? 4 : 2) k_schur(DevProblem P, const double* __restrict__ xs, double* __restrict__ y,
                                                double* __restrict__ rep, const int* __restrict__ done_flag, int tile0) {
  constexpr int NI = popcount10(IMASK);
  constexpr int NJ = 14 + 2 * NI;
  constexpr int WS = (NJ + 2) * 32;
  if (done_flag != nullptr && *done_flag) return;
#ifdef TBA_EMULATE
  double* s_dyn = emu::dyn_smem<double>();
#else
  extern __shared__ __align__(128) double s_dyn[];
#endif
  __shared__ double s_t[MAXP][4];
  __shared__ __align__(8) uint64_t s_bar[TILE / 32];
  const int tile = tile0 + blockIdx.x, tid = threadIdx.x, lane = tid & 31, warp = tid >> 5;
  double* sJ = s_dyn + (size_t)warp * WS;
  double* sR = sJ + NJ * 32;
  if (lane == 0) {
    mbar_init(&s_bar[warp], 1);
    constexpr uint32_t jbytes = NJ * 32 * 8, rbytes = (MODE != 0) ? 2 * 32 * 8 : 0;
    mbar_expect_tx(&s_bar[warp], jbytes + rbytes);
    bulk_g2s(sJ, P.J + wslice(tile, warp, NJ), jbytes, &s_bar[warp]);
    if (MODE != 0) bulk_g2s(sR, P.res + wslice(tile, warp, 2), rbytes, &s_bar[warp]);
  }
  const int p0 = P.tile_pt_begin[tile], npt = P.tile_pt_begin[tile + 1] - p0;
  for (int i = tid; i < npt * 4; i += TILE) (&s_t[0][0])[i] = 0.0;
  const size_t slot = (size_t)tile * TILE + tid;
  const int cam = P.slot_cam[slot];
  const bool valid = cam >= 0;
  int pl = -1 - lane, grp = 0;
  double h = 0.0;
  double2 xa = make_double2(0.0, 0.0), xb = xa, xc = xa;
  double xi[NI + 1];
  if (valid) {
    pl = P.slot_pt[slot] - p0;
    grp = P.single_group ? 0 : P.cam_group[cam];
    h = P.pt[(size_t)(p0 + pl) * 4 + 3];
    if (MODE != 1) {
      const double2* x2 = reinterpret_cast<const double2*>(xs + (size_t)cam * 6);
      xa = __ldg(x2); xb = __ldg(x2 + 1); xc = __ldg(x2 + 2);
      if (NI > 0) {
        const double* xg = xs + P.ne + (size_t)grp * 10;
#pragma unroll
        for (int j = 0; j < NI; ++j) xi[j] = __ldg(xg + nth_bit(IMASK, j));
      }
    }
  }
  const int prev = __shfl_up_sync(0xffffffffu, pl, 1);
  const bool head = lane == 0 || prev != pl;
  __syncthreads();
  mbar_wait(&s_bar[warp], 0);
  const double *ja = sJ + lane, *jw = ja + 6 * 32, *jh = ja + 12 * 32, *ji = ja + 14 * 32;
  double w0 = 0.0, w1 = 0.0, r0 = 0.0, r1 = 0.0;
  if (valid) {
    if (MODE != 0) { r0 = sR[lane]; r1 = sR[32 + lane]; }
    if (MODE != 1) obs_apply_F<NI, 32, 32>(ja, jw, ji, h, xa, xb, xc, xi, w0, w1);
    if (MODE == 1) { w0 = r0; w1 = r1; }
    if (MODE == 2) { w0 = r0 - w0; w1 = r1 - w1; }
  }
  double t[4] = {0.0, 0.0, 0.0, 0.0};
  if (valid) obs_JpT<32>(ja, jh, w0, w1, t);
#pragma unroll
  for (int j = 0; j < 4; ++j) t[j] = seg_reduce(t[j], pl, lane);
  if (head && valid) {
#pragma unroll
    for (int j = 0; j < 4; ++j) atomicAdd(&s_t[pl][j], t[j]);
  }
  __syncthreads();
  if (tid < npt) {
    const double tt[4] = {s_t[tid][0], s_t[tid][1], s_t[tid][2], s_t[tid][3]};
    double uu[4];
    sym4_mul(P.Mp + (size_t)(p0 + tid) * 10, tt, uu);
    s_t[tid][0] = uu[0]; s_t[tid][1] = uu[1]; s_t[tid][2] = uu[2]; s_t[tid][3] = uu[3];
    if (MODE == 2) {
      double* d = P.dpt + (size_t)(p0 + tid) * 4;
      d[0] = -uu[0]; d[1] = -uu[1]; d[2] = -uu[2]; d[3] = -uu[3];
    }
  }
  __syncthreads();
  double u[4] = {0.0, 0.0, 0.0, 0.0};
  if (valid) { u[0] = s_t[pl][0]; u[1] = s_t[pl][1]; u[2] = s_t[pl][2]; u[3] = s_t[pl][3]; }
  double z0 = 0.0, z1 = 0.0;
  if (valid) obs_sub_Jp<32>(ja, jh, w0, w1, u, z0, z1);
  double* rr = rep_row(rep);
  if (MODE == 2) {
    double mcc = 0.0;
    if (valid && !(P.slot_flags[slot] & 1)) mcc = obs_model_cost_change(r0, r1, z0, z1);
    mcc = warp_sum(mcc);
    if (lane == 0) red_add(rr + 23, mcc);
  } else {
    double yv[6], yi[NI + 1];
    obs_JcT<32, 32>(ja, jw, h, z0, z1, yv);
    obs_JiT<NI, 32>(ji, z0, z1, yi);
#pragma unroll
    for (int j = 0; j < 6; ++j) yv[j] = valid ? yv[j] : 0.0;
#pragma unroll
    for (int j = 0; j < NI; ++j) yi[j] = valid ? yi[j] : 0.0;
    __syncwarp();
    int* sbase = reinterpret_cast<int*>(sJ + 32 * 6);
    warp_stage_row<6>(sJ, sbase, yv, valid ? cam * 6 : -1, lane);
    __syncwarp();
    warp_red_rows<6>(y, sJ, sbase, lane);
    if (NI > 0) {
      if (P.single_group) {
#pragma unroll
        for (int j = 0; j < NI; ++j) {
          const double v = warp_sum(yi[j]);
          if (lane == 0) red_add(rr + nth_bit(IMASK, j), v);
        }
      } else if (valid) {
#pragma unroll
        for (int j = 0; j < NI; ++j) red_add(y + P.ne + (size_t)grp * 10 + nth_bit(IMASK, j), yi[j]);
      }
    }
  }
}

struct P2pDev {
  int world = 1, rank = 0;
  unsigned long long seq = 0;
  size_t cap = 0;
  double* const* inbox = nullptr;
  unsigned long long* const* flags = nullptr;
  int* ctr = nullptr;
};
#ifdef TBA_EMULATE
__device__ __forceinline__ void st_release_sys(unsigned long long* p, unsigned long long v) { *p = v; }
__device__ __forceinline__ unsigned long long ld_acquire_sys(const unsigned long long* p) { return *p; }
__device__ __forceinline__ double ld_cg(const double* p) { return *p; }
#else
__device__ __forceinline__ void st_release_sys(unsigned long long* p, unsigned long long v) {
  asm volatile("st.release.sys.global.u64 [%0], %1;" ::"l"(p), "l"(v) : "memory");
}
__device__ __forceinline__ unsigned long long ld_acquire_sys(const unsigned long long* p) {
  unsigned long long v;
  asm volatile("ld.acquire.sys.global.u64 %0, [%1];" : "=l"(v) : "l"(p) : "memory");
  return v;
}
__device__ __forceinline__ double ld_cg(const double* p) { return __ldcg(p); }
#endif
__device__ __forceinline__ void p2p_wait(const P2pDev& pp) {
  if ((int)threadIdx.x < pp.world) {
    const unsigned long long* f = pp.flags[pp.rank] + threadIdx.x;
#ifndef TBA_EMULATE
    const long long t0 = clock64();
#endif
    while (ld_acquire_sys(f) < pp.seq) {
#ifdef TBA_EMULATE
      emu_yield();
#else
      if (clock64() - t0 > 20000000000ll) { printf("tba: rank %d waited 10 s for the partial sums of rank %d (exchange %llu)\n", pp.rank, (int)threadIdx.x, pp.seq); __trap(); }
#endif
    }
  }
  __syncthreads();
}
__device__ __forceinline__ double p2p_sum(const P2pDev& pp, int i) {
  const double* base = pp.inbox[pp.rank] + (size_t)(pp.seq & 1ull) * pp.world * pp.cap + i;
  double v = 0.0;
  for (int q = 0; q < pp.world; ++q) v += ld_cg(base + (size_t)q * pp.cap);
  return v;
}

__device__ __forceinline__ int run_last_lane_dev(unsigned heads, int lane) {
#ifdef TBA_EMULATE
  return run_last_lane(heads, lane);
#else
  const unsigned above = lane >= 31 ? 0u : (heads & ~((2u << lane) - 1u));
  return above == 0u ? 31 : __ffs(above) - 2;
#endif
}

template <uint32_t IMASK, int N>
__device__ __forceinline__ void warp_red_rows_cols(double* __restrict__ dst, const double* __restrict__ stage, const int* __restrict__ sbase, int lane) {
#pragma unroll
  for (int k = 0; k < N; ++k) {
    const int e = k * 32 + lane;
    const int o = e / N, j = e - o * N;
    const int b = sbase[o];
    int col = 0;
#pragma unroll
    for (int q = 0; q < N; ++q) if (q == j) col = nth_bit(IMASK, q);
    if (b >= 0) red_add(dst + (size_t)b + col, stage[e]);
  }
}

template <uint32_t IMASK, int MODE>
struct StreamCfg {
  static constexpr int NI = popcount10(IMASK);
  static constexpr int NJ = 14 + 2 * NI;
  static constexpr int STG = NJ * 32 + (MODE != 0 ? 64 : 0) + 32;
  static constexpr int NS = 3;
  static constexpr int NW = (220 * 1024 / (NS * STG * 8)) > 12 ? 12 : (220 * 1024 / (NS * STG * 8));
  static constexpr size_t SMEM = (size_t)NW * NS * STG * 8 + (size_t)NW * NS * 8;
};

template <uint32_t IMASK, int MODE>
__global__ void __launch_bounds__(StreamCfg<IMASK, MODE>::NW * 32, 1)
k_schur_stream(DevProblem P, const double* __restrict__ xs, double* __restrict__ y, double* __restrict__ rep,
               const int* __restrict__ done_flag, int n_slices, P2pDev pp) {
  using Cfg = StreamCfg<IMASK, MODE>;
  constexpr int NI = Cfg::NI, NJ = Cfg::NJ, STG = Cfg::STG, NS = Cfg::NS, NW = Cfg::NW;
  if (done_flag != nullptr && *done_flag) return;
#ifdef TBA_EMULATE
  double* s_dyn = emu::dyn_smem<double>();
#else
  extern __shared__ __align__(128) double s_dyn[];
#endif
  const int lane = threadIdx.x & 31, warp = threadIdx.x >> 5;
  const int gw = blockIdx.x * NW + warp, GW = gridDim.x * NW;
  const int s_begin = (int)((long long)n_slices * gw / GW), s_end = (int)((long long)n_slices * (gw + 1) / GW);
  const bool active = s_begin < s_end;
  double* ring = s_dyn + (size_t)warp * NS * STG;
  uint64_t* bars = reinterpret_cast<uint64_t*>(s_dyn + (size_t)NW * NS * STG) + warp * NS;
  constexpr uint32_t jbytes = NJ * 32 * 8, rbytes = (MODE != 0) ? 2 * 32 * 8 : 0;
  auto issue = [&](int stage, int slice) {
    double* st = ring + (size_t)stage * STG;
    mbar_expect_tx(&bars[stage], jbytes + rbytes + 256);
    bulk_g2s(st, P.J + (size_t)slice * NJ * 32, jbytes, &bars[stage]);
    if (MODE != 0) bulk_g2s(st + NJ * 32, P.res + (size_t)slice * 64, rbytes, &bars[stage]);
    int* idx = reinterpret_cast<int*>(st + NJ * 32 + (MODE != 0 ? 64 : 0));
    bulk_g2s(idx, P.slot_cam + (size_t)slice * 32, 128, &bars[stage]);
    bulk_g2s(idx + 32, P.slot_pt + (size_t)slice * 32, 128, &bars[stage]);
  };
  if (lane == 0 && active) {
#pragma unroll
    for (int k = 0; k < NS; ++k) mbar_init(&bars[k], 1);
#pragma unroll
    for (int k = 0; k < NS; ++k) if (s_begin + k < s_end) issue(k, s_begin + k);
  }
  __syncwarp();
  double xi_u[NI + 1];
  if (NI > 0 && MODE != 1 && P.single_group) {
#pragma unroll
    for (int j = 0; j < NI; ++j) xi_u[j] = __ldg(xs + P.ne + nth_bit(IMASK, j));
  }
  double yi_acc[NI + 1];
#pragma unroll
  for (int j = 0; j < NI; ++j) yi_acc[j] = 0.0;
  double mcc_acc = 0.0;
  int cam_n = -1, pt_n = 0, grp_n = 0;
  unsigned heads_n = 0xffffffffu;
  double2 xa_n = make_double2(0.0, 0.0), xb_n = xa_n, xc_n = xa_n;
  double xi_n[NI + 1];
  double h_n = 0.0;
  double2 m01_n = xa_n, m23_n = xa_n, m45_n = xa_n, m67_n = xa_n, m89_n = xa_n;
  uint8_t flag_n = 0;
  auto prefetch = [&](int slice, int it) {
    const int stage = it % NS;
    mbar_wait(&bars[stage], (uint32_t)((it / NS) & 1));
    const int* idx = reinterpret_cast<const int*>(ring + (size_t)stage * STG + NJ * 32 + (MODE != 0 ? 64 : 0));
    cam_n = idx[lane];
    pt_n = idx[32 + lane];
    const bool valid = cam_n >= 0;
    const int key = valid ? pt_n : -1 - lane;
    const int prev = __shfl_up_sync(0xffffffffu, key, 1);
    const bool head = lane == 0 || prev != key;
    heads_n = __ballot_sync(0xffffffffu, head);
    if (valid) {
      h_n = __ldg(P.pt + (size_t)pt_n * 4 + 3);
      if (MODE != 1) {
        const double2* x2 = reinterpret_cast<const double2*>(xs + (size_t)((MODE == 0 && (P.ablate & 2)) ? lane : cam_n) * 6);
        xa_n = __ldg(x2); xb_n = __ldg(x2 + 1); xc_n = __ldg(x2 + 2);
      }
      if (NI > 0 && !P.single_group) {
        grp_n = __ldg(P.cam_group + cam_n);
        if (MODE != 1) {
          const double* xg = xs + P.ne + (size_t)grp_n * 10;
#pragma unroll
          for (int j = 0; j < NI; ++j) xi_n[j] = __ldg(xg + nth_bit(IMASK, j));
        }
      }
      if (head) {
        const double2* M2 = reinterpret_cast<const double2*>(P.Mp + (size_t)pt_n * 10);
        m01_n = __ldg(M2); m23_n = __ldg(M2 + 1); m45_n = __ldg(M2 + 2); m67_n = __ldg(M2 + 3); m89_n = __ldg(M2 + 4);
      }
      if (MODE == 2) flag_n = P.slot_flags[(size_t)slice * 32 + lane];
    }
  };
  if (active) prefetch(s_begin, 0);
  for (int s = s_begin, it = 0; s < s_end; ++s, ++it) {
    const int cam = cam_n, pt = pt_n, grp = grp_n;
    const unsigned heads = heads_n;
    const double2 xa = xa_n, xb = xb_n, xc = xc_n, m01 = m01_n, m23 = m23_n, m45 = m45_n, m67 = m67_n, m89 = m89_n;
    const double h = h_n;
    const uint8_t flag = flag_n;
    double xi[NI + 1];
#pragma unroll
    for (int j = 0; j < NI; ++j) xi[j] = (NI > 0 && MODE != 1) ? (P.single_group ? xi_u[j] : xi_n[j]) : 0.0;
    const bool valid = cam >= 0;
    if (s + 1 < s_end) prefetch(s + 1, it + 1);
    const int stage = it % NS;
    double* sJ = ring + (size_t)stage * STG;
    const double* sR = sJ + NJ * 32;
    const double *jw = sJ + lane + 6 * 32, *ji = sJ + lane + 14 * 32;
    double w0 = 0.0, w1 = 0.0, r0 = 0.0, r1 = 0.0;
    double ja[6], jh[2];
#pragma unroll
    for (int j = 0; j < 6; ++j) ja[j] = sJ[j * 32 + lane];
    jh[0] = sJ[12 * 32 + lane]; jh[1] = sJ[13 * 32 + lane];
    if (valid) {
      if (MODE != 0) { r0 = sR[lane]; r1 = sR[32 + lane]; }
      if (MODE != 1) obs_apply_F<NI, 1, 32>(ja, jw, ji, h, xa, xb, xc, xi, w0, w1);
      if (MODE == 1) { w0 = r0; w1 = r1; }
      if (MODE == 2) { w0 = r0 - w0; w1 = r1 - w1; }
    }
    double t[4] = {0.0, 0.0, 0.0, 0.0};
    if (valid) obs_JpT<1>(ja, jh, w0, w1, t);
    if (!(MODE == 0 && (P.ablate & 8))) {
      const int last = run_last_lane_dev(heads, lane);
#pragma unroll
      for (int j = 0; j < 4; ++j) t[j] = seg_reduce_to(t[j], last, lane);
    }
    double u[4];
    u[0] = m01.x * t[0] + m01.y * t[1] + m23.x * t[2] + m23.y * t[3];
    u[1] = m01.y * t[0] + m45.x * t[1] + m45.y * t[2] + m67.x * t[3];
    u[2] = m23.x * t[0] + m45.y * t[1] + m67.y * t[2] + m89.x * t[3];
    u[3] = m23.y * t[0] + m67.x * t[1] + m89.x * t[2] + m89.y * t[3];
    const bool head = (heads >> lane) & 1u;
    if (MODE == 2 && head && valid) {
      double2* d = reinterpret_cast<double2*>(P.dpt + (size_t)pt * 4);
      d[0] = make_double2(-u[0], -u[1]);
      d[1] = make_double2(-u[2], -u[3]);
    }
    const int hl = run_head_lane(heads, lane);
#pragma unroll
    for (int j = 0; j < 4; ++j) u[j] = __shfl_sync(0xffffffffu, u[j], hl);
    double z0 = 0.0, z1 = 0.0;
    if (valid) obs_sub_Jp<1>(ja, jh, w0, w1, u, z0, z1);
    if (MODE == 2) {
      if (valid && !(flag & 1)) mcc_acc += obs_model_cost_change(r0, r1, z0, z1);
    } else {
      double yv[6], yi[NI + 1];
      obs_JcT<1, 32>(ja, jw, h, z0, z1, yv);
      obs_JiT<NI, 32>(ji, z0, z1, yi);
#pragma unroll
      for (int j = 0; j < 6; ++j) yv[j] = valid ? yv[j] : 0.0;
#pragma unroll
      for (int j = 0; j < NI; ++j) yi[j] = valid ? yi[j] : 0.0;
      __syncwarp();
      int* sbase = reinterpret_cast<int*>(sJ + 32 * 6);
      warp_stage_row<6>(sJ, sbase, yv, valid ? cam * 6 : -1, lane);
      __syncwarp();
      if (!(MODE == 0 && (P.ablate & 1))) warp_red_rows<6>(y, sJ, sbase, lane);
      if (NI > 0) {
        if (P.single_group) {
#pragma unroll
          for (int j = 0; j < NI; ++j) yi_acc[j] += yi[j];
        } else {
          static_assert(32 * 6 + 16 + 32 * NI + 16 <= NJ * 32, "stage too small for the intrinsics staging");
          double* si = sJ + 32 * 6 + 16;
          int* sibase = reinterpret_cast<int*>(si + 32 * NI);
          __syncwarp();
#pragma unroll
          for (int j = 0; j < NI; ++j) si[lane * NI + j] = yi[j];
          sibase[lane] = valid ? P.ne + grp * 10 : -1;
          __syncwarp();
          if (!(MODE == 0 && (P.ablate & 1))) warp_red_rows_cols<IMASK, (NI > 0 ? NI : 1)>(y, si, sibase, lane);
        }
      }
    }
    __syncwarp();
    if (lane == 0 && s + NS < s_end) {
      fence_proxy_async_smem();
      issue(stage, s + NS);
    }
  }
  double* rr = rep + (size_t)(gw & (NREP - 1)) * REPW;
  if (!active) {
  } else if (MODE == 2) {
    const double m = warp_sum(mcc_acc);
    if (lane == 0) red_add(rr + 23, m);
  } else if (NI > 0 && P.single_group) {
#pragma unroll
    for (int j = 0; j < NI; ++j) {
      const double v = warp_sum(yi_acc[j]);
      if (lane == 0) red_add(rr + nth_bit(IMASK, j), v);
    }
  }
  if (MODE == 0 && pp.world > 1) {
    __shared__ int s_last;
    __threadfence();
    __syncthreads();
    if (threadIdx.x == 0) {
      atomicAdd(pp.ctr, 1);
#ifndef TBA_EMULATE
      const long long t0 = clock64();
      while (atomicAdd(pp.ctr, 0) < (int)gridDim.x) {
        if (clock64() - t0 > 4000000000ll) { printf("tba: grid barrier of the matvec timed out (block %d)\n", (int)blockIdx.x); __trap(); }
      }
#endif
    }
    __syncthreads();
    __threadfence();
    const size_t slot = ((size_t)(pp.seq & 1ull) * pp.world + pp.rank) * pp.cap;
    const bool fold = NI > 0 && P.single_group;
    if (fold && blockIdx.x == 0 && threadIdx.x < 10) {
      double v = ld_cg(y + P.ne + threadIdx.x);
      for (int r = 0; r < NREP; ++r) { v += ld_cg(rep + (size_t)r * REPW + threadIdx.x); rep[(size_t)r * REPW + threadIdx.x] = 0.0; }
      y[P.ne + threadIdx.x] = v;
      for (int q = 0; q < pp.world; ++q) pp.inbox[q][slot + P.ne + threadIdx.x] = v;
    }
    const int n_push = fold ? P.ne : P.ncs;
    const int n2 = (n_push + 1) / 2;
    const int per = (n2 + (int)gridDim.x - 1) / (int)gridDim.x;
    const int i0 = (int)blockIdx.x * per, i1 = (i0 + per < n2) ? i0 + per : n2;
    for (int i = i0 + (int)threadIdx.x; i < i1; i += (int)blockDim.x) {
      const double a = ld_cg(y + 2 * i), b = 2 * i + 1 < n_push ? ld_cg(y + 2 * i + 1) : 0.0;
      for (int q = 0; q < pp.world; ++q) reinterpret_cast<double2*>(pp.inbox[q] + slot)[i] = make_double2(a, b);
    }
    __syncthreads();
    if (threadIdx.x == 0) { __threadfence_system(); s_last = atomicAdd(pp.ctr + 1, 1) == (int)gridDim.x - 1; }
    __syncthreads();
    if (s_last) {
      __threadfence_system();
      if ((int)threadIdx.x < pp.world) st_release_sys(pp.flags[threadIdx.x] + pp.rank, pp.seq);
    }
  }
}

template <uint32_t IMASK>
struct PrepCfg {
  static constexpr int NI = popcount10(IMASK);
  static constexpr int NJ = 14 + 2 * NI;
  static constexpr int NSI = NI * (NI + 1) / 2;
  static constexpr int STG = NJ * 32 + 64 + 32;
  static constexpr int NS = 3;
  static constexpr int NWMAX = NI <= 4 ? 10 : 6;
  static constexpr int NW = (216 * 1024 / (NS * STG * 8)) > NWMAX ? NWMAX : (216 * 1024 / (NS * STG * 8));
  static constexpr size_t SMEM = (size_t)NW * NS * STG * 8 + (size_t)NW * NS * 8 + (size_t)NW * (NSI + 1) * 8;
};

template <uint32_t IMASK>
__global__ void __launch_bounds__(PrepCfg<IMASK>::NW * 32, 1)
k_prepare_stream(DevProblem P, double* __restrict__ y, double* __restrict__ Sc, double* __restrict__ Si, double* __restrict__ rep, int n_slices) {
  using Cfg = PrepCfg<IMASK>;
  constexpr int NI = Cfg::NI, NJ = Cfg::NJ, STG = Cfg::STG, NS = Cfg::NS, NW = Cfg::NW, NSI = Cfg::NSI;
#ifdef TBA_EMULATE
  double* s_dyn = emu::dyn_smem<double>();
#else
  extern __shared__ __align__(128) double s_dyn[];
#endif
  const int lane = threadIdx.x & 31, warp = threadIdx.x >> 5;
  const int gw = blockIdx.x * NW + warp, GW = gridDim.x * NW;
  const int s_begin = (int)((long long)n_slices * gw / GW), s_end = (int)((long long)n_slices * (gw + 1) / GW);
  double* ring = s_dyn + (size_t)warp * NS * STG;
  uint64_t* bars = reinterpret_cast<uint64_t*>(s_dyn + (size_t)NW * NS * STG) + warp * NS;
  double* s_si = s_dyn + (size_t)NW * NS * STG + (size_t)NW * NS;
  constexpr uint32_t jbytes = NJ * 32 * 8, rbytes = 2 * 32 * 8;
  auto issue = [&](int stage, int slice) {
    double* st = ring + (size_t)stage * STG;
    mbar_expect_tx(&bars[stage], jbytes + rbytes + 256);
    bulk_g2s(st, P.J + (size_t)slice * NJ * 32, jbytes, &bars[stage]);
    bulk_g2s(st + NJ * 32, P.res + (size_t)slice * 64, rbytes, &bars[stage]);
    int* idx = reinterpret_cast<int*>(st + NJ * 32 + 64);
    bulk_g2s(idx, P.slot_cam + (size_t)slice * 32, 128, &bars[stage]);
    bulk_g2s(idx + 32, P.slot_pt + (size_t)slice * 32, 128, &bars[stage]);
  };
  if (lane == 0 && s_begin < s_end) {
#pragma unroll
    for (int k = 0; k < NS; ++k) mbar_init(&bars[k], 1);
#pragma unroll
    for (int k = 0; k < NS; ++k) if (s_begin + k < s_end) issue(k, s_begin + k);
  }
  __syncwarp();
  double yi_acc[NI + 1], si_acc[NSI + 1];
#pragma unroll
  for (int j = 0; j < NI; ++j) yi_acc[j] = 0.0;
#pragma unroll
  for (int j = 0; j < NSI; ++j) si_acc[j] = 0.0;
  int cam_n = -1, pt_n = 0, grp_n = 0;
  unsigned heads_n = 0xffffffffu, rheads_n = 0xffffffffu;
  double h_n = 0.0;
  double2 m01_n = make_double2(0.0, 0.0), m23_n = m01_n, m45_n = m01_n, m67_n = m01_n, m89_n = m01_n;
  auto prefetch = [&](int it) {
    const int stage = it % NS;
    mbar_wait(&bars[stage], (uint32_t)((it / NS) & 1));
    const int* idx = reinterpret_cast<const int*>(ring + (size_t)stage * STG + NJ * 32 + 64);
    cam_n = idx[lane];
    pt_n = idx[32 + lane];
    const bool valid = cam_n >= 0;
    grp_n = 0;
    if (valid && NI > 0 && !P.single_group) grp_n = __ldg(P.cam_group + cam_n);
    const int key = valid ? pt_n : -1 - lane;
    const int prev = __shfl_up_sync(0xffffffffu, key, 1);
    const int prevg = __shfl_up_sync(0xffffffffu, grp_n, 1);
    const bool head = lane == 0 || prev != key;
    heads_n = __ballot_sync(0xffffffffu, head);
    rheads_n = __ballot_sync(0xffffffffu, head || prevg != grp_n);
    if (valid) {
      h_n = __ldg(P.pt + (size_t)pt_n * 4 + 3);
      const double2* M2 = reinterpret_cast<const double2*>(P.Mp + (size_t)pt_n * 10);
      m01_n = __ldg(M2); m23_n = __ldg(M2 + 1); m45_n = __ldg(M2 + 2); m67_n = __ldg(M2 + 3); m89_n = __ldg(M2 + 4);
    }
  };
  if (s_begin < s_end) prefetch(0);
  for (int s = s_begin, it = 0; s < s_end; ++s, ++it) {
    const int cam = cam_n, grp = grp_n;
    const unsigned heads = heads_n, rheads = rheads_n;
    const double M[10] = {m01_n.x, m01_n.y, m23_n.x, m23_n.y, m45_n.x, m45_n.y, m67_n.x, m67_n.y, m89_n.x, m89_n.y};
    const double h = h_n;
    const bool valid = cam >= 0;
    if (s + 1 < s_end) prefetch(it + 1);
    const int stage = it % NS;
    double* sJ = ring + (size_t)stage * STG;
    const double* sR = sJ + NJ * 32;
    const double* Jt = sJ + lane;
    double ja[6], jh[2], jw[6], ji[2 * NI + 1];
#pragma unroll
    for (int j = 0; j < 6; ++j) { ja[j] = Jt[j * 32]; jw[j] = Jt[(6 + j) * 32]; }
    jh[0] = Jt[12 * 32]; jh[1] = Jt[13 * 32];
#pragma unroll
    for (int j = 0; j < 2 * NI; ++j) ji[j] = Jt[(14 + j) * 32];
    double r0 = 0.0, r1 = 0.0;
    if (valid) { r0 = sR[lane]; r1 = sR[32 + lane]; }
    if (!valid) {
#pragma unroll
      for (int j = 0; j < 6; ++j) { ja[j] = 0.0; jw[j] = 0.0; }
      jh[0] = jh[1] = 0.0;
#pragma unroll
      for (int j = 0; j < 2 * NI; ++j) ji[j] = 0.0;
    }
    __syncwarp();
    const int last = run_last_lane_dev(heads, lane);
    const int hl = run_head_lane(heads, lane);
    {
      double t[4];
      obs_JpT<1>(ja, jh, r0, r1, t);
#pragma unroll
      for (int j = 0; j < 4; ++j) t[j] = seg_reduce_to(t[j], last, lane);
      double u[4];
      sym4_mul(M, t, u);
#pragma unroll
      for (int j = 0; j < 4; ++j) u[j] = __shfl_sync(0xffffffffu, u[j], hl);
      double z0, z1, yv[6], yi[NI + 1];
      obs_sub_Jp<1>(ja, jh, r0, r1, u, z0, z1);
      obs_JcT<1, 1>(ja, jw, h, z0, z1, yv);
      obs_JiT<NI, 1>(ji, z0, z1, yi);
      int* sbase = reinterpret_cast<int*>(sJ + 32 * 6);
      warp_stage_row<6>(sJ, sbase, yv, valid ? cam * 6 : -1, lane);
      __syncwarp();
      warp_red_rows<6>(y, sJ, sbase, lane);
      if (NI > 0) {
        if (P.single_group) {
#pragma unroll
          for (int j = 0; j < NI; ++j) yi_acc[j] += yi[j];
        } else if (valid) {
#pragma unroll
          for (int j = 0; j < NI; ++j) red_add(y + P.ne + (size_t)grp * 10 + nth_bit(IMASK, j), yi[j]);
        }
      }
      __syncwarp();
    }
    {
      double v[21];
      obs_cam_block(M, ja, jh, jw, h, v);
      int* sbase = reinterpret_cast<int*>(sJ + 32 * 7);
#pragma unroll
      for (int g3 = 0; g3 < 3; ++g3) {
        const double vv[7] = {v[7 * g3], v[7 * g3 + 1], v[7 * g3 + 2], v[7 * g3 + 3], v[7 * g3 + 4], v[7 * g3 + 5], v[7 * g3 + 6]};
        warp_stage_row<7>(sJ, sbase, vv, valid ? cam * 21 + 7 * g3 : -1, lane);
        __syncwarp();
        warp_red_rows<7>(Sc, sJ, sbase, lane);
        __syncwarp();
      }
    }
    if (NI > 0) {
      const int rlast = run_last_lane_dev(rheads, lane);
      const bool rhead = (rheads >> lane) & 1u;
      double W[4 * NI + 1];
#pragma unroll
      for (int a = 0; a < 4; ++a) {
        const double p0 = a < 3 ? ja[a] : jh[0], p1 = a < 3 ? ja[3 + a] : jh[1];
#pragma unroll
        for (int j = 0; j < NI; ++j) W[a * NI + j] = seg_reduce_to(p0 * ji[j] + p1 * ji[NI + j], rlast, lane);
      }
      double sub[NSI + 1], acc[NSI + 1];
#pragma unroll
      for (int j = 0; j < NSI; ++j) sub[j] = 0.0;
      if (rhead && valid) run_WT_M_W<NI>(M, W, sub);
      obs_JiT_Ji<NI>(ji, acc);
      int n = 0;
#pragma unroll
      for (int a = 0; a < NI; ++a)
#pragma unroll
        for (int b = a; b < NI; ++b) {
          if (P.single_group) si_acc[n] += acc[n] - sub[n];
          else if (valid) red_add(Si + (size_t)grp * 55 + tri10(nth_bit(IMASK, a), nth_bit(IMASK, b)), acc[n] - sub[n]);
          ++n;
        }
    }
    __syncwarp();
    if (lane == 0 && s + NS < s_end) {
      fence_proxy_async_smem();
      issue(stage, s + NS);
    }
  }
  if (NI > 0 && P.single_group) {
    double* rr = rep + (size_t)(gw & (NREP - 1)) * REPW;
#pragma unroll
    for (int j = 0; j < NI; ++j) {
      const double vsum = warp_sum(yi_acc[j]);
      if (lane == 0) red_add(rr + nth_bit(IMASK, j), vsum);
    }
#pragma unroll
    for (int j = 0; j < NSI; ++j) {
      const double vsum = warp_sum(si_acc[j]);
      if (lane == 0) s_si[warp * (NSI + 1) + j] = vsum;
    }
    __syncthreads();
    if ((int)threadIdx.x < NSI) {
      double vsum = 0.0;
      for (int w = 0; w < NW; ++w) vsum += s_si[w * (NSI + 1) + threadIdx.x];
      int n = 0, idx = 0;
      for (int a = 0; a < NI; ++a)
        for (int b = a; b < NI; ++b) {
          if (n == (int)threadIdx.x) idx = tri10(nth_bit(IMASK, a), nth_bit(IMASK, b));
          ++n;
        }
      red_add(Si + idx, vsum);
    }
  }
}

template <uint32_t IMASK>
struct LinCfg {
  static constexpr int NI = popcount10(IMASK);
  static constexpr int NJ = 14 + 2 * NI;
  static constexpr int STG = 64 + 16 + 16 + 4;
  static constexpr int RSTG = 2 * 32 * 6 + 16;
  static constexpr int NS = 4;
  static constexpr int NW = 8;
  static constexpr size_t SMEM = (size_t)NW * (NS * STG + RSTG) * 8 + (size_t)NW * NS * 8;
};

template <uint32_t IMASK>
__global__ void __launch_bounds__(LinCfg<IMASK>::NW * 32, 1)
k_linearize_stream(DevProblem P, double* __restrict__ g_cs, double* __restrict__ cn_cs, double* __restrict__ rep, int n_slices) {
  using Cfg = LinCfg<IMASK>;
  constexpr int NI = Cfg::NI, NJ = Cfg::NJ, STG = Cfg::STG, RSTG = Cfg::RSTG, NS = Cfg::NS, NW = Cfg::NW;
#ifdef TBA_EMULATE
  double* s_dyn = emu::dyn_smem<double>();
#else
  extern __shared__ __align__(128) double s_dyn[];
#endif
  const int lane = threadIdx.x & 31, warp = threadIdx.x >> 5;
  const int gw = blockIdx.x * NW + warp, GW = gridDim.x * NW;
  const int s_begin = (int)((long long)n_slices * gw / GW), s_end = (int)((long long)n_slices * (gw + 1) / GW);
  double* ring = s_dyn + (size_t)warp * NS * STG;
  double* rows = s_dyn + (size_t)NW * NS * STG + (size_t)warp * RSTG;
  int* rbase = reinterpret_cast<int*>(rows + 2 * 32 * 6);
  uint64_t* bars = reinterpret_cast<uint64_t*>(s_dyn + (size_t)NW * (NS * STG + RSTG)) + warp * NS;
  auto issue = [&](int stage, int slice) {
    double* st = ring + (size_t)stage * STG;
    mbar_expect_tx(&bars[stage], 512 + 128 + 128 + 32);
    bulk_g2s(st, P.xy + (size_t)slice * 64, 512, &bars[stage]);
    int* idx = reinterpret_cast<int*>(st + 64);
    bulk_g2s(idx, P.slot_cam + (size_t)slice * 32, 128, &bars[stage]);
    bulk_g2s(idx + 32, P.slot_pt + (size_t)slice * 32, 128, &bars[stage]);
    bulk_g2s(st + 96, P.slot_flags + (size_t)slice * 32, 32, &bars[stage]);
  };
  if (lane == 0 && s_begin < s_end) {
#pragma unroll
    for (int k = 0; k < NS; ++k) mbar_init(&bars[k], 1);
#pragma unroll
    for (int k = 0; k < NS; ++k) if (s_begin + k < s_end) issue(k, s_begin + k);
  }
  __syncwarp();
  double gi_acc[NI + 1], ci_acc[NI + 1];
#pragma unroll
  for (int j = 0; j < NI; ++j) { gi_acc[j] = 0.0; ci_acc[j] = 0.0; }
  double cost_acc = 0.0, fixed_acc = 0.0, failed_acc = 0.0;
  int cam_n = -1, pt_n = 0, grp_n = 0;
  unsigned heads_n = 0xffffffffu;
  double2 e0_n = make_double2(0.0, 0.0), e1_n = e0_n, e3_n = e0_n, q0_n = e0_n, q1_n = e0_n, X01_n = e0_n, X23_n = e0_n;
  auto prefetch = [&](int it) {
    const int stage = it % NS;
    mbar_wait(&bars[stage], (uint32_t)((it / NS) & 1));
    const int* idx = reinterpret_cast<const int*>(ring + (size_t)stage * STG + 64);
    cam_n = idx[lane];
    pt_n = idx[32 + lane];
    const bool valid = cam_n >= 0;
    const int key = valid ? pt_n : -1 - lane;
    const int prev = __shfl_up_sync(0xffffffffu, key, 1);
    heads_n = __ballot_sync(0xffffffffu, lane == 0 || prev != key);
    if (valid) {
      const double2* e2 = reinterpret_cast<const double2*>(P.ext + (size_t)cam_n * 6);
      e0_n = __ldg(e2); e1_n = __ldg(e2 + 1); e3_n = __ldg(e2 + 2);
      const double2* q2 = reinterpret_cast<const double2*>(P.cam_s4 + (size_t)cam_n * 4);
      q0_n = __ldg(q2); q1_n = __ldg(q2 + 1);
      const double2* X2 = reinterpret_cast<const double2*>(P.pt + (size_t)pt_n * 4);
      X01_n = __ldg(X2); X23_n = __ldg(X2 + 1);
      grp_n = P.single_group ? 0 : __ldg(P.cam_group + cam_n);
    }
  };
  if (s_begin < s_end) prefetch(0);
  for (int s = s_begin, it = 0; s < s_end; ++s, ++it) {
    const int cam = cam_n, pt = pt_n, grp = grp_n;
    const unsigned heads = heads_n;
    const double2 e0 = e0_n, e1 = e1_n, e3 = e3_n, q0 = q0_n, q1 = q1_n, X01 = X01_n, X23 = X23_n;
    const bool valid = cam >= 0;
    if (s + 1 < s_end) prefetch(it + 1);
    const int stage = it % NS;
    const double* st = ring + (size_t)stage * STG;
    double Ja[6] = {0, 0, 0, 0, 0, 0}, Jw[6] = {0, 0, 0, 0, 0, 0}, Jh[2] = {0, 0}, r[2] = {0, 0};
    double Ji[2 * NI + 1];
#pragma unroll
    for (int j = 0; j < 2 * NI; ++j) Ji[j] = 0.0;
    if (valid) {
      const double Cw[6] = {e0.x, e0.y, e1.x, e1.y, e3.x, e3.y};
      double rec[kCamRec];
      cam_rec_expand(e1.y, e3.x, e3.y, q0.x, q0.y, q1.x, q1.y, rec);
#ifndef TBA_EMULATE
      {
        const double w0 = e1.y, w1 = e3.x, w2 = e3.y, B = q1.x, Cc = q1.y;
        const double C02 = __dmul_rn(__dmul_rn(Cc, w0), w2);
        rec[9 + 2] = fma(B, w1, C02);
        rec[9 + 6] = fma(-B, w1, C02);
      }
#endif
      double rho0 = 0.0;
      const bool ok = linearize_obs_any<IMASK, false>(P.group_model[grp], Cw, rec, P.intr + (size_t)grp * 10, X01.x, X01.y, X23.x,
                                                      X23.y, st[lane], st[32 + lane], P.loss_type, P.loss_width, r, rho0, Ja, Jw, Jh, Ji);
      obs_settle<NI>(ok, (reinterpret_cast<const uint8_t*>(st + 96)[lane] & 1) != 0, rho0, cost_acc, fixed_acc, failed_acc, Ja, Jw, Jh,
                     Ji, r);
    }
    obs_store<NI>(P.J + (size_t)s * NJ * 32 + lane, P.res + (size_t)s * 64 + lane, Ja, Jw, Jh, Ji, r);
    {
      double acc[14];
      obs_point_terms(Ja, Jh, r, acc);
      const int last = run_last_lane_dev(heads, lane);
#pragma unroll
      for (int j = 0; j < 14; ++j) acc[j] = seg_reduce_to(acc[j], last, lane);
      if (valid && ((heads >> lane) & 1u)) {
        double2* H2 = reinterpret_cast<double2*>(P.Hpp + (size_t)pt * 10);
#pragma unroll
        for (int j = 0; j < 5; ++j) H2[j] = make_double2(acc[2 * j], acc[2 * j + 1]);
        double2* G2 = reinterpret_cast<double2*>(P.gp + (size_t)pt * 4);
        G2[0] = make_double2(acc[10], acc[11]);
        G2[1] = make_double2(acc[12], acc[13]);
      }
    }
    {
      double gv[6], cv[6];
      obs_cam_grad(Ja, Jw, X23.y, r, gv, cv);
      __syncwarp();
      warp_stage_row<6>(rows, rbase, gv, valid ? cam * 6 : -1, lane);
      warp_stage_row<6>(rows + 32 * 6, rbase, cv, valid ? cam * 6 : -1, lane);
      __syncwarp();
      warp_red_rows<6>(g_cs, rows, rbase, lane);
      warp_red_rows<6>(cn_cs, rows + 32 * 6, rbase, lane);
    }
    if (NI > 0) {
      double g, c;
      if (P.single_group) {
#pragma unroll
        for (int j = 0; j < NI; ++j) {
          obs_intr_grad<NI>(Ji, r, j, g, c);
          gi_acc[j] += g;
          ci_acc[j] += c;
        }
      } else if (valid) {
#pragma unroll
        for (int j = 0; j < NI; ++j) {
          obs_intr_grad<NI>(Ji, r, j, g, c);
          red_add(g_cs + P.ne + (size_t)grp * 10 + nth_bit(IMASK, j), g);
          red_add(cn_cs + P.ne + (size_t)grp * 10 + nth_bit(IMASK, j), c);
        }
      }
    }
    __syncwarp();
    if (lane == 0 && s + NS < s_end) {
      fence_proxy_async_smem();
      issue(stage, s + NS);
    }
  }
  if (s_begin < s_end) {
    double* rr = rep + (size_t)(gw & (NREP - 1)) * REPW;
    if (NI > 0 && P.single_group) {
#pragma unroll
      for (int j = 0; j < NI; ++j) {
        const double gsum = warp_sum(gi_acc[j]), csum = warp_sum(ci_acc[j]);
        if (lane == 0) { red_add(rr + nth_bit(IMASK, j), gsum); red_add(rr + 10 + nth_bit(IMASK, j), csum); }
      }
    }
    const double c = warp_sum(cost_acc), f = warp_sum(fixed_acc), e = warp_sum(failed_acc);
    if (lane == 0) {
      red_add(rr + 20, c);
      if (f != 0.0) red_add(rr + 21, f);
      if (e != 0.0) red_add(rr + 22, e);
    }
  }
}

template <uint32_t IMASK>
__global__ void __launch_bounds__(TILE) k_precond_ext(DevProblem P, double* __restrict__ Sc, int tile0) {
  constexpr int NI = popcount10(IMASK);
  constexpr int NJ = 14 + 2 * NI;
  const int tile = tile0 + blockIdx.x, tid = threadIdx.x, lane = tid & 31, warp = tid >> 5;
  const size_t slot = (size_t)tile * TILE + tid;
  const int cam = P.slot_cam[slot];
  __shared__ double s_stage[TILE / 32][32 * 21];
  __shared__ int s_base[TILE / 32][32];
  double v[21];
#pragma unroll
  for (int j = 0; j < 21; ++j) v[j] = 0.0;
  if (cam >= 0) {
    const double* Jt = P.J + wslice(tile, warp, NJ) + lane;
    double Ja[6], Jw[6], Jh[2];
#pragma unroll
    for (int j = 0; j < 6; ++j) Ja[j] = Jt[j * 32];
#pragma unroll
    for (int j = 0; j < 6; ++j) Jw[j] = Jt[(6 + j) * 32];
    Jh[0] = Jt[12 * 32];
    Jh[1] = Jt[13 * 32];
    const int pt = P.slot_pt[slot];
    obs_cam_block(P.Mp + (size_t)pt * 10, Ja, Jh, Jw, P.pt[(size_t)pt * 4 + 3], v);
  }
  warp_stage_row<21>(s_stage[warp], s_base[warp], v, cam >= 0 ? cam * 21 : -1, lane);
  __syncwarp();
  warp_red_rows<21>(Sc, s_stage[warp], s_base[warp], lane);
}

template <uint32_t IMASK>
__global__ void __launch_bounds__(TILE) k_precond_intr(DevProblem P, double* __restrict__ Si, int tile0) {
  constexpr int NI = popcount10(IMASK);
  constexpr int NJ = 14 + 2 * NI;
  constexpr int NW = 4 * NI;
  constexpr int NS = NI * (NI + 1) / 2;
#ifdef TBA_EMULATE
  double* s_w = emu::dyn_smem<double>();
#else
  extern __shared__ double s_w[];
#endif
  __shared__ double s_red[32];
  const int tile = tile0 + blockIdx.x, tid = threadIdx.x, lane = tid & 31, warp = tid >> 5;
  const int nruns = P.tile_nruns[tile];
  int* s_grp = reinterpret_cast<int*>(s_w + (size_t)TILE * NW);
  int* s_pt = s_grp + TILE;
  for (int i = tid; i < nruns * NW; i += TILE) s_w[i] = 0.0;
  __syncthreads();
  const size_t slot = (size_t)tile * TILE + tid;
  const int cam = P.slot_cam[slot];
  const bool valid = cam >= 0;
  double acc[NS + 1];
#pragma unroll
  for (int j = 0; j < NS; ++j) acc[j] = 0.0;
  int grp = 0;
  if (valid) {
    const double* Jt = P.J + wslice(tile, warp, NJ) + lane;
    double jp0[4], jp1[4], Ji[2 * NI + 1];
#pragma unroll
    for (int j = 0; j < 3; ++j) { jp0[j] = Jt[j * 32]; jp1[j] = Jt[(3 + j) * 32]; }
    jp0[3] = Jt[12 * 32];
    jp1[3] = Jt[13 * 32];
#pragma unroll
    for (int j = 0; j < 2 * NI; ++j) Ji[j] = Jt[(14 + j) * 32];
    grp = P.cam_group[cam];
    const int run = P.slot_run[slot];
    if (run >= 0) {
      s_grp[run] = grp;
      s_pt[run] = P.slot_pt[slot];
      double* W = s_w + (size_t)run * NW;
#pragma unroll
      for (int a = 0; a < 4; ++a)
#pragma unroll
        for (int j = 0; j < NI; ++j) atomicAdd(W + a * NI + j, jp0[a] * Ji[j] + jp1[a] * Ji[NI + j]);
    }
    obs_JiT_Ji<NI>(Ji, acc);
  }
  __syncthreads();
  int rgrp = grp;
  double sub[NS + 1];
#pragma unroll
  for (int j = 0; j < NS; ++j) sub[j] = 0.0;
  const bool has_run = tid < nruns;
  if (has_run) {
    rgrp = s_grp[tid];
    run_WT_M_W<NI>(P.Mp + (size_t)s_pt[tid] * 10, s_w + (size_t)tid * NW, sub);
  }
  int n = 0;
#pragma unroll
  for (int a = 0; a < NI; ++a)
#pragma unroll
    for (int b = a; b < NI; ++b) {
      const int idx = tri10(nth_bit(IMASK, a), nth_bit(IMASK, b));
      if (P.single_group) {
        const double v = block_sum(acc[n] - sub[n], s_red);
        if (tid == 0) red_add(Si + idx, v);
      } else {
        if (valid) red_add(Si + (size_t)grp * 55 + idx, acc[n]);
        if (has_run) red_add(Si + (size_t)rgrp * 55 + idx, -sub[n]);
      }
      ++n;
    }
}

template <int N>
__device__ inline bool spd_inverse_n(double* A) {
  double L[N * N], Li[N * N];
#pragma unroll
  for (int i = 0; i < N; ++i)
#pragma unroll
    for (int j = 0; j <= i; ++j) {
      double s = A[i * N + j];
      for (int k = 0; k < j; ++k) s -= L[i * N + k] * L[j * N + k];
      if (i == j) { if (!(s > 0.0)) return false; L[i * N + i] = sqrt(s); }
      else L[i * N + j] = s / L[j * N + j];
    }
  for (int i = 0; i < N * N; ++i) Li[i] = 0.0;
  for (int j = 0; j < N; ++j) {
    Li[j * N + j] = 1.0 / L[j * N + j];
    for (int i = j + 1; i < N; ++i) {
      double s = 0.0;
      for (int k = j; k < i; ++k) s -= L[i * N + k] * Li[k * N + j];
      Li[i * N + j] = s / L[i * N + i];
    }
  }
  for (int i = 0; i < N; ++i)
    for (int j = 0; j < N; ++j) {
      double s = 0.0;
      for (int k = (i > j ? i : j); k < N; ++k) s += Li[k * N + i] * Li[k * N + j];
      A[i * N + j] = s;
    }
  return true;
}

__global__ void k_precond_finish(DevProblem P, const double* __restrict__ Sc, const double* __restrict__ Si,
                                 const double* __restrict__ sm, const double* __restrict__ D2, double* __restrict__ Minv_c,
                                 double* __restrict__ Minv_i, double* __restrict__ flag) {
  const int i = blockIdx.x * blockDim.x + threadIdx.x;
  if (i < P.n_cam) {
    double A[36];
    const double* S = Sc + (size_t)i * 21;
    const double* s = sm + (size_t)i * 6;
    const double* d = D2 + (size_t)i * 6;
    int n = 0;
    for (int a = 0; a < 6; ++a)
      for (int b = a; b < 6; ++b) { const double v = s[a] * S[n] * s[b]; A[a * 6 + b] = v; A[b * 6 + a] = v; ++n; }
    for (int a = 0; a < 6; ++a) { if (s[a] != 0.0) A[a * 6 + a] += d[a]; else A[a * 6 + a] = 1.0; }
    if (!spd_inverse_n<6>(A)) { atomicAdd(flag, 1.0); for (int a = 0; a < 36; ++a) A[a] = (a % 7 == 0) ? 1.0 : 0.0; }
    for (int a = 0; a < 36; ++a) Minv_c[(size_t)i * 36 + a] = A[a];
  } else if (i < P.n_cam + P.n_group) {
    const int g = i - P.n_cam;
    double A[100];
    const double* S = Si + (size_t)g * 55;
    const double* s = sm + P.ne + (size_t)g * 10;
    const double* d = D2 + P.ne + (size_t)g * 10;
    int n = 0;
    for (int a = 0; a < 10; ++a)
      for (int b = a; b < 10; ++b) { const double v = s[a] * S[n] * s[b]; A[a * 10 + b] = v; A[b * 10 + a] = v; ++n; }
    for (int a = 0; a < 10; ++a) { if (s[a] != 0.0) A[a * 10 + a] += d[a]; else A[a * 10 + a] = 1.0; }
    if (!spd_inverse_n<10>(A)) { atomicAdd(flag, 1.0); for (int a = 0; a < 100; ++a) A[a] = (a % 11 == 0) ? 1.0 : 0.0; }
    for (int a = 0; a < 100; ++a) Minv_i[(size_t)g * 100 + a] = A[a];
  }
}

__global__ void k_cs_scale(int ncs, const double* __restrict__ cn, const double* __restrict__ mask, int use_scaling,
                           double* __restrict__ sm) {
  for (int i = blockIdx.x * blockDim.x + threadIdx.x; i < ncs; i += gridDim.x * blockDim.x)
    sm[i] = mask[i] != 0.0 ? (use_scaling ? 1.0 / (1.0 + sqrt(cn[i])) : 1.0) : 0.0;
}
__global__ void k_cs_diag(int ncs, const double* __restrict__ cn, const double* __restrict__ sm, double radius, double lo,
                          double hi, double* __restrict__ D2) {
  for (int i = blockIdx.x * blockDim.x + threadIdx.x; i < ncs; i += gridDim.x * blockDim.x)
    D2[i] = sm[i] != 0.0 ? fmin(fmax(sm[i] * sm[i] * cn[i], lo), hi) / radius : 0.0;
}

struct PcgState {
  double rho, last_rho, beta, alpha, pq, Q0, Q1, norm_b2;
  int iters;
  int done;
  int status;
  int pending_q;
  int min_iters, max_iters;
  double eta;
};

// ... 393 lines not shown
```

### theiasfm_b200/engine.py

```python
import ctypes as C
import os

import numpy as np

from . import _abi

_HERE = os.path.dirname(os.path.abspath(__file__))
LIB_PATH = os.environ.get("THEIA_BA_B200_LIB") or os.path.join(_HERE, "libtheia_ba_b200.so")
_LIB = None

EXPORTED_SYMBOLS = [
    "tba_options_init", "tba_device_count", "tba_create", "tba_destroy", "tba_nccl_unique_id", "tba_last_error",
    "tba_solve", "tba_upload", "tba_minimize", "tba_download", "tba_shard_points", "tba_debug_linearize", "tba_debug_linearize_raw",
    "tba_debug_stream_launch",
    "tba_debug_prepare_linear_system", "tba_debug_schur_matvec", "tba_debug_solve_linear_system",
    "tba_debug_evaluate_step", "tba_debug_read", "tba_reset_parameters", "tba_set_max_iterations", "tba_set_profiling", "tba_get_profile", "tba_get_profile_stages", "tba_solve_multi", "tba_debug_pack", "tba_filter_tracks", "tba_adjust_tracks", "tba_adjust_views", "tba_estimate_tracks", "tba_two_view_ba_batch", "tba_two_view_ba_batch_multi",
]


class EngineError(RuntimeError):
    def __init__(self, code, message):
        super().__init__("tba error %d: %s" % (code, message))
        self.code = code


def lib():
    global _LIB
    if _LIB is None:
        if not os.path.exists(LIB_PATH):
            raise ImportError("%s is missing: build it with `python -c 'import __graft_entry__ as g; g.build()'` "
                              "(make -C theiasfm_b200/csrc). There is no CPU fallback." % LIB_PATH)
        L = C.CDLL(LIB_PATH)
        dp = C.POINTER(C.c_double)
        L.tba_options_init.argtypes = [C.POINTER(_abi.tba_options)]
        L.tba_device_count.restype = C.c_int
        L.tba_create.argtypes = [C.c_int, C.c_int, C.c_int, C.c_void_p, C.POINTER(C.c_void_p)]
        L.tba_destroy.argtypes = [C.c_void_p]
        L.tba_nccl_unique_id.argtypes = [C.c_void_p]
        L.tba_last_error.restype = C.c_char_p
        L.tba_last_error.argtypes = [C.c_void_p]
        L.tba_solve.argtypes = [C.c_void_p, C.POINTER(_abi.tba_options), C.POINTER(_abi.tba_problem), C.POINTER(_abi.tba_summary)]
        L.tba_upload.argtypes = [C.c_void_p, C.POINTER(_abi.tba_options), C.POINTER(_abi.tba_problem)]
        L.tba_minimize.argtypes = [C.c_void_p, C.POINTER(_abi.tba_summary)]
        L.tba_download.argtypes = [C.c_void_p, C.POINTER(_abi.tba_problem)]
        L.tba_shard_points.argtypes = [C.POINTER(C.c_int32), C.c_int32, C.c_int, C.c_int, C.POINTER(C.c_int32), C.POINTER(C.c_int32)]
        L.tba_debug_linearize.argtypes = [C.c_void_p, dp]
        L.tba_debug_linearize_raw.argtypes = [C.c_void_p, C.c_int, C.POINTER(C.c_int64), dp, dp, dp, dp, dp]
        L.tba_debug_stream_launch.argtypes = [C.c_void_p, C.POINTER(C.c_int32)]
        L.tba_debug_prepare_linear_system.argtypes = [C.c_void_p, C.c_double]
        L.tba_debug_schur_matvec.argtypes = [C.c_void_p, dp, dp, dp, dp]
        L.tba_debug_solve_linear_system.argtypes = [C.c_void_p, C.POINTER(C.c_int32), dp]
        L.tba_debug_evaluate_step.argtypes = [C.c_void_p, dp]
        L.tba_debug_read.argtypes = [C.c_void_p, C.c_int, dp, C.c_int64]
        L.tba_abi_sizes.argtypes = [C.POINTER(C.c_int32)]
        L.tba_solve_multi.argtypes = [C.POINTER(_abi.tba_options), C.POINTER(_abi.tba_problem), C.POINTER(_abi.tba_summary), C.c_int]
        L.tba_debug_pack.restype = C.c_int
        L.tba_adjust_tracks.argtypes = [C.c_void_p, C.POINTER(_abi.tba_options), C.POINTER(C.c_uint8), dp, dp, C.POINTER(C.c_int32)]
        L.tba_adjust_views.argtypes = [C.c_void_p, C.POINTER(_abi.tba_options), C.POINTER(C.c_int32), C.c_int32, C.POINTER(C.c_uint8), dp, dp,
                                       C.POINTER(C.c_int32)]
        L.tba_estimate_tracks.argtypes = [C.c_void_p, C.POINTER(_abi.tba_options), C.c_double, C.c_double, C.c_int32, C.POINTER(C.c_uint8), C.POINTER(C.c_int32)]
        L.tba_two_view_ba_batch_multi.argtypes = [C.POINTER(_abi.tba_two_view_batch), C.c_int, C.POINTER(C.c_uint8), dp, dp, C.POINTER(C.c_int32)]
        L.tba_two_view_ba_batch.argtypes = [C.c_void_p, C.POINTER(_abi.tba_two_view_batch), C.POINTER(C.c_uint8), dp, dp, C.POINTER(C.c_int32)]
        L.tba_filter_tracks.argtypes = [C.c_void_p, C.c_double, C.c_double, C.POINTER(C.c_uint8), dp, C.POINTER(C.c_int32), C.POINTER(C.c_int32)]
        L.tba_reset_parameters.argtypes = [C.c_void_p, C.POINTER(_abi.tba_problem)]
        L.tba_set_max_iterations.argtypes = [C.c_void_p, C.c_int32]
        L.tba_set_profiling.argtypes = [C.c_void_p, C.c_int]
        L.tba_get_profile.argtypes = [C.c_void_p, dp]
        L.tba_get_profile_stages.argtypes = [C.c_void_p, dp]
        _LIB = L
    return _LIB


def _dp(a):
    return a.ctypes.data_as(C.POINTER(C.c_double))


def default_options(**kw):
    o = _abi.tba_options()
    lib().tba_options_init(C.byref(o))
    for k, v in kw.items():
        if not hasattr(o, k):
            raise AttributeError(k)
        setattr(o, k, v)
    return o


def device_count():
    return lib().tba_device_count()


def nccl_unique_id():
    buf = C.create_string_buffer(128)
    rc = lib().tba_nccl_unique_id(buf)
    if rc != 0:
        raise EngineError(rc, "ncclGetUniqueId failed")
    return buf.raw


def shard_points(pt_num_obs, world_size, rank):
    a = np.ascontiguousarray(pt_num_obs, dtype=np.int32)
    b, e = C.c_int32(), C.c_int32()
    lib().tba_shard_points(a.ctypes.data_as(C.POINTER(C.c_int32)), len(a), world_size, rank, C.byref(b), C.byref(e))
    return b.value, e.value


class Summary:
    def __init__(self, s, iters):
        for f, _ in _abi.tba_summary._fields_:
            if f not in ("iterations", "message"):
                setattr(self, f, getattr(s, f))
        self.message = s.message.decode(errors="replace")
        n = min(s.num_iterations, len(iters))
        self.iterations = [{f: getattr(iters[i], f) for f, _ in _abi.tba_iteration._fields_} for i in range(n)]

    @property
    def costs(self):
        return np.array([it["cost"] for it in self.iterations])


def debug_pack(problem):
    cap = (problem.n_obs // 200 + problem.n_pt // 8 + 8) * 256 + problem.n_obs * 2
    sizes = np.zeros(6, np.int64)
    out = dict(slot_cam=np.zeros(cap, np.int32), slot_pt=np.zeros(cap, np.int32), slot_run=np.zeros(cap, np.int16),
               slot_flags=np.zeros(cap, np.uint8), xy=np.zeros(cap * 2), slot_orig=np.zeros(cap, np.int64),
               pk2caller=np.zeros(max(problem.n_pt, 1), np.int32), tile_pt_begin=np.zeros(cap // 256 + 2, np.int32),
               tile_nruns=np.zeros(cap // 256 + 2, np.int32), tile_flags=np.zeros(cap // 256 + 2, np.uint8),
               mask=np.zeros(problem.n_cam * 6 + problem.n_group * 10))
    st = problem.as_struct()
    P = C.POINTER
    rc = lib().tba_debug_pack(C.byref(st), cap, sizes.ctypes.data_as(P(C.c_int64)), out["slot_cam"].ctypes.data_as(P(C.c_int32)),
                              out["slot_pt"].ctypes.data_as(P(C.c_int32)), out["slot_run"].ctypes.data_as(P(C.c_int16)),
# ... 103 lines not shown
    def download(self, problem=None):
        problem = problem or self._problem
        st = problem.as_struct()
        self._check(lib().tba_download(self._h, C.byref(st)))

    def filter_tracks(self, max_inlier_reprojection_error, min_triangulation_angle_degrees):
        n = self._problem.n_pt
        status = np.zeros(max(n, 1), np.uint8); mean = np.zeros(max(n, 1))
        nb, ni = C.c_int32(), C.c_int32()
        self._check(lib().tba_filter_tracks(self._h, max_inlier_reprojection_error, min_triangulation_angle_degrees,
                                            status.ctypes.data_as(C.POINTER(C.c_uint8)), _dp(mean), C.byref(nb), C.byref(ni)))
        return status[:n], mean[:n], nb.value, ni.value

    def adjust_tracks(self, options):
        n = max(self._problem.n_pt, 1)
        status = np.zeros(n, np.uint8); ic = np.zeros(n); fc = np.zeros(n); nf = C.c_int32()
        self._check(lib().tba_adjust_tracks(self._h, C.byref(options), status.ctypes.data_as(C.POINTER(C.c_uint8)), _dp(ic), _dp(fc), C.byref(nf)))
        n = self._problem.n_pt
        return status[:n], ic[:n], fc[:n], nf.value

    def adjust_views(self, options, views):
        v = np.ascontiguousarray(views, dtype=np.int32).reshape(-1)
        n = len(v)
        status = np.zeros(max(n, 1), np.uint8); ic = np.zeros(max(n, 1)); fc = np.zeros(max(n, 1)); it = np.zeros(max(n, 1), np.int32)
        self._check(lib().tba_adjust_views(self._h, C.byref(options), v.ctypes.data_as(C.POINTER(C.c_int32)), n,
                                           status.ctypes.data_as(C.POINTER(C.c_uint8)), _dp(ic), _dp(fc), it.ctypes.data_as(C.POINTER(C.c_int32))))
        return status[:n], ic[:n], fc[:n], it[:n]

    def estimate_tracks(self, options, max_reprojection_error_pixels=5.0, min_triangulation_angle_degrees=3.0, bundle_adjustment=True):
        status = np.zeros(max(self._problem.n_pt, 1), np.uint8); counts = np.zeros(5, np.int32)
        self._check(lib().tba_estimate_tracks(self._h, C.byref(options), max_reprojection_error_pixels, min_triangulation_angle_degrees,
                                              int(bundle_adjustment), status.ctypes.data_as(C.POINTER(C.c_uint8)),
                                              counts.ctypes.data_as(C.POINTER(C.c_int32))))
        return status[:self._problem.n_pt], counts

    def two_view_ba_batch(self, batch):
        n = max(batch.n_pairs, 1)
        term = np.zeros(n, np.uint8); ic = np.zeros(n); fc = np.zeros(n); it = np.zeros(n, np.int32)
        st = batch.as_struct()
        self._check(lib().tba_two_view_ba_batch(self._h, C.byref(st), term.ctypes.data_as(C.POINTER(C.c_uint8)), _dp(ic), _dp(fc),
                                                it.ctypes.data_as(C.POINTER(C.c_int32))))
        n = batch.n_pairs
        return term[:n], ic[:n], fc[:n], it[:n]

    def reset_parameters(self, problem):
        st = problem.as_struct()
        self._check(lib().tba_reset_parameters(self._h, C.byref(st)))

    def set_max_iterations(self, n):
        self._check(lib().tba_set_max_iterations(self._h, int(n)))

    def set_profiling(self, enable=True):
        self._check(lib().tba_set_profiling(self._h, int(enable)))

    def profile(self):
        out = np.zeros(8)
        self._check(lib().tba_get_profile(self._h, _dp(out)))
        return dict(matvec_ms=out[0], matvec_launches=int(out[1]), linearize_ms=out[2], linearize_launches=int(out[3]),
                    slots=int(out[4]), observations=int(out[5]), points=int(out[6]), doubles_per_obs=int(out[7]))

    STAGES = ("matvec", "linearize", "precond_ext", "precond_intr", "rhs", "backsub", "candidate_cost", "prepare_fused")

    def profile_stages(self):
        out = np.zeros(16)
        self._check(lib().tba_get_profile_stages(self._h, _dp(out)))
        return {k: {"ms": float(out[2 * i]), "launches": int(out[2 * i + 1])} for i, k in enumerate(self.STAGES)}

    def linearize(self):
        c = C.c_double()
        rc = lib().tba_debug_linearize(self._h, C.byref(c))
        return rc == 0, c.value

    def linearize_raw(self, tile_kernel=False):
        sizes = np.zeros(4, np.int64)
        self._check(lib().tba_debug_linearize_raw(self._h, int(tile_kernel), sizes.ctypes.data_as(C.POINTER(C.c_int64)), None, None, None, None, None))
        n_slots, nj, n_pt, ncs = (int(v) for v in sizes)
        J, res = np.zeros((n_slots // 32, nj, 32)), np.zeros((n_slots // 32, 2, 32))
        Hpp, gp, lin = np.zeros((n_pt, 10)), np.zeros((n_pt, 4)), np.zeros(2 * ncs + 3)
        self._check(lib().tba_debug_linearize_raw(self._h, int(tile_kernel), sizes.ctypes.data_as(C.POINTER(C.c_int64)),
                                                  _dp(J), _dp(res), _dp(Hpp), _dp(gp), _dp(lin)))
        return dict(J=J, res=res, Hpp=Hpp, gp=gp, g=lin[:ncs], cn=lin[ncs:2 * ncs], cost=lin[2 * ncs], fixed=lin[2 * ncs + 1],
                    failed=lin[2 * ncs + 2])

    STREAM_KERNELS = ("linearize", "prepare", "matvec", "rhs_backsub")

    def stream_launch(self):
        out = np.zeros(16, np.int32)
        self._check(lib().tba_debug_stream_launch(self._h, out.ctypes.data_as(C.POINTER(C.c_int32))))
        d = dict(n_sm=int(out[0]), n_slices=int(out[1]), imask=int(out[2]), has_ext_models=bool(out[3]))
        for k, name in enumerate(self.STREAM_KERNELS):
            d[name] = dict(grid=int(out[4 + 3 * k]), NW=int(out[5 + 3 * k]), NS=int(out[6 + 3 * k]))
        return d

    def prepare_linear_system(self, radius):
        return lib().tba_debug_prepare_linear_system(self._h, radius) == 0

    def schur_matvec(self, x_cam, x_intr):
        x_cam = np.ascontiguousarray(x_cam, np.float64); x_intr = np.ascontiguousarray(x_intr, np.float64)
        y_cam = np.zeros_like(x_cam); y_intr = np.zeros_like(x_intr)
        self._check(lib().tba_debug_schur_matvec(self._h, _dp(x_cam), _dp(x_intr), _dp(y_cam), _dp(y_intr)))
        return y_cam, y_intr

    def solve_linear_system(self):
        it, m = C.c_int32(), C.c_double()
        rc = lib().tba_debug_solve_linear_system(self._h, C.byref(it), C.byref(m))
        return rc == 0, it.value, m.value

    def evaluate_step(self):
        c = C.c_double()
        rc = lib().tba_debug_evaluate_step(self._h, C.byref(c))
        return rc == 0, c.value

    def read(self, which):
        p = self._problem
        n = {_abi.VEC_GRADIENT_CAM: p.n_cam * 6, _abi.VEC_GRADIENT_INTR: p.n_group * 10, _abi.VEC_GRADIENT_PT: p.n_pt * 4,
             _abi.VEC_COLNORM2_CAM: p.n_cam * 6, _abi.VEC_COLNORM2_INTR: p.n_group * 10, _abi.VEC_COLNORM2_PT: p.n_pt * 4,
             _abi.VEC_RESIDUALS: p.n_obs * 2, _abi.VEC_SCHUR_RHS_CAM: p.n_cam * 6, _abi.VEC_SCHUR_RHS_INTR: p.n_group * 10,
             _abi.VEC_PRECOND_CAM: p.n_cam * 36, _abi.VEC_PRECOND_INTR: p.n_group * 100, _abi.VEC_STEP_CAM: p.n_cam * 6,
             _abi.VEC_STEP_INTR: p.n_group * 10, _abi.VEC_STEP_PT: p.n_pt * 4}[which]
        out = np.zeros(n)
        self._check(lib().tba_debug_read(self._h, which, _dp(out), n))
        return out
```

Baseline: 653.2 million.

## Store normalized (u,v) instead of intrinsic Jacobian columns and rebuild on the fly

When there is a single camera group, no extended models, trivial loss and at least two free intrinsics, the stored per-observation Jacobian slice keeps only the two normalized coordinates (u,v) in place of 2*NI intrinsic columns. The Schur matvec, prepare and preconditioner kernels recompute the intrinsic columns from (u,v) and the shared intrinsics. This cuts Jacobian storage and the memory bandwidth spent re-reading it on every CG iteration, at the cost of extra FLOPs per observation. Explicitly rounded intrinsics keep the rebuilt values bit-identical to the stored ones, and a debug entry point is added for checking.

```diff
diff --git a/include/theia_ba_b200.h b/include/theia_ba_b200.h
--- a/include/theia_ba_b200.h
+++ b/include/theia_ba_b200.h
@@ -207,6 +207,7 @@
 int tba_debug_linearize(tba_context* ctx, double* cost);
 int tba_debug_linearize_raw(tba_context* ctx, int tile_kernel, int64_t* sizes_out, double* J, double* res, double* Hpp,
                             double* gp, double* lin);
+int tba_debug_intr_cols(tba_context* ctx, int64_t* sizes_out, double* Ji);
 int tba_debug_stream_launch(tba_context* ctx, int32_t* out);
 int tba_debug_prepare_linear_system(tba_context* ctx, double radius);
 int tba_debug_schur_matvec(tba_context* ctx, const double* x_cam ,
diff --git a/theiasfm_b200/csrc/tba_camera_models.cuh b/theiasfm_b200/csrc/tba_camera_models.cuh
--- a/theiasfm_b200/csrc/tba_camera_models.cuh
+++ b/theiasfm_b200/csrc/tba_camera_models.cuh
@@ -139,11 +139,83 @@
   return true;
 }
 
+__host__ __device__ inline double mul_rn(double a, double b) {
+#ifdef __CUDA_ARCH__
+  return __dmul_rn(a, b);
+#else
+  return a * b;
+#endif
+}
+__host__ __device__ inline double add_rn(double a, double b) {
+#ifdef __CUDA_ARCH__
+  return __dadd_rn(a, b);
+#else
+  return a + b;
+#endif
+}
+__host__ __device__ inline double fma_rn(double a, double b, double c) {
+#ifdef __CUDA_ARCH__
+  return __fma_rn(a, b, c);
+#else
+  return fma(a, b, c);
+#endif
+}
+
+template <uint32_t IMASK>
+__host__ __device__ inline void obs_intr_cols(int model, double u, double v, const double* __restrict__ k, double P00, double P01,
+                                              double P10, double P11, double* Ji) {
+  constexpr int NI = popcount10(IMASK);
+  if (NI == 0) return;
+  const double f = k[0], ar = k[1], sk = k[2];
+  const double r2 = add_rn(mul_rn(u, u), mul_rn(v, v));
+  double ud, vd, dk[10][2];
+  if (model == kModelPinhole) {
+    const double d = fma_rn(r2, fma_rn(k[6], r2, k[5]), 1.0);
+    ud = mul_rn(u, d); vd = mul_rn(v, d);
+    const double r4 = mul_rn(r2, r2);
+    dk[5][0] = mul_rn(r2, u); dk[5][1] = mul_rn(r2, v);
+    dk[6][0] = mul_rn(r4, u); dk[6][1] = mul_rn(r4, v);
+    dk[7][0] = dk[7][1] = dk[8][0] = dk[8][1] = dk[9][0] = dk[9][1] = 0.0;
+  } else {
+    const double r4 = mul_rn(r2, r2), r6 = mul_rn(r4, r2);
+    const double rd = fma_rn(mul_rn(k[7], r4), r2, fma_rn(k[6], r4, fma_rn(k[5], r2, 1.0)));
+    const double t1 = k[8], t2 = k[9];
+    const double uv2 = mul_rn(2.0 * u, v), eu = fma_rn(2.0 * u, u, r2), ev = fma_rn(2.0 * v, v, r2);
+    ud = fma_rn(mul_rn(2.0 * t1, u), v, fma_rn(u, rd, mul_rn(t2, eu)));
+    vd = fma_rn(mul_rn(2.0 * t2, u), v, fma_rn(v, rd, mul_rn(t1, ev)));
+    dk[5][0] = mul_rn(r2, u); dk[5][1] = mul_rn(r2, v);
+    dk[6][0] = mul_rn(r4, u); dk[6][1] = mul_rn(r4, v);
+    dk[7][0] = mul_rn(r6, u); dk[7][1] = mul_rn(r6, v);
+    dk[8][0] = uv2; dk[8][1] = ev;
+    dk[9][0] = add_rn(r2, mul_rn(2.0 * u, u)); dk[9][1] = uv2;
+  }
+  const double far = mul_rn(f, ar);
+  double col[10][2];
+  col[0][0] = ud;  col[0][1] = mul_rn(ar, vd);
+  col[1][0] = 0.0; col[1][1] = mul_rn(f, vd);
+  col[2][0] = vd;  col[2][1] = 0.0;
+  col[3][0] = 1.0; col[3][1] = 0.0;
+  col[4][0] = 0.0; col[4][1] = 1.0;
+  TBA_UNROLL
+  for (int j = 5; j < 10; ++j) {
+    col[j][0] = fma_rn(f, dk[j][0], mul_rn(sk, dk[j][1]));
+    col[j][1] = mul_rn(far, dk[j][1]);
+  }
+  TBA_UNROLL
+  for (int j = 0; j < NI; ++j) {
+    constexpr uint32_t M = IMASK;
+    const int idx = nth_bit(M, j);
+    Ji[j] = fma_rn(P00, col[idx][0], mul_rn(P01, col[idx][1]));
+    Ji[NI + j] = fma_rn(P10, col[idx][0], mul_rn(P11, col[idx][1]));
+  }
+}
+
 template <uint32_t IMASK>
 __host__ __device__ inline bool linearize_obs(int model, const double* __restrict__ C, const double* __restrict__ rec,
                                      const double* __restrict__ k, const double X0, const double X1, const double X2,
                                      const double h, const double x, const double y, int loss_type, double loss_width,
-                                     double r[2], double& rho0, double Ja[6], double Jw[6], double Jh[2], double* Ji) {
+                                     double r[2], double& rho0, double Ja[6], double Jw[6], double Jh[2], double* Ji,
+                                     double* uv = nullptr) {
   constexpr int NI = popcount10(IMASK);
   const double* R = rec;
   const double* L = rec + 9;
@@ -157,15 +229,11 @@
   const double u = q0 * iz, v = q1 * iz;
   const double r2 = u * u + v * v;
   double ud, vd, D00, D01, D10, D11;
-  double dk[10][2];
   if (model == kModelPinhole) {
     const double d = 1.0 + r2 * (k[5] + k[6] * r2);
     const double dd = 2.0 * k[5] + 4.0 * k[6] * r2;
     ud = u * d; vd = v * d;
     D00 = d + u * u * dd; D01 = u * v * dd; D10 = D01; D11 = d + v * v * dd;
-    dk[5][0] = r2 * u; dk[5][1] = r2 * v;
-    dk[6][0] = r2 * r2 * u; dk[6][1] = r2 * r2 * v;
-    dk[7][0] = dk[7][1] = dk[8][0] = dk[8][1] = dk[9][0] = dk[9][1] = 0.0;
   } else {
     const double r4 = r2 * r2;
     const double rd = 1.0 + k[5] * r2 + k[6] * r4 + k[7] * r4 * r2;
@@ -177,11 +245,6 @@
     D01 = 2.0 * u * v * rdp + 2.0 * t2 * v + 2.0 * t1 * u;
     D10 = 2.0 * u * v * rdp + 2.0 * t1 * u + 2.0 * t2 * v;
     D11 = rd + 2.0 * v * v * rdp + 6.0 * t1 * v + 2.0 * t2 * u;
-    dk[5][0] = r2 * u; dk[5][1] = r2 * v;
-    dk[6][0] = r4 * u; dk[6][1] = r4 * v;
-    dk[7][0] = r4 * r2 * u; dk[7][1] = r4 * r2 * v;
-    dk[8][0] = 2.0 * u * v; dk[8][1] = r2 + 2.0 * v * v;
-    dk[9][0] = r2 + 2.0 * u * u; dk[9][1] = 2.0 * u * v;
   }
   const double f = k[0], ar = k[1], sk = k[2];
   const double rr0 = f * ud + sk * vd + k[3] - x;
@@ -223,26 +286,8 @@
   Jw[3] = -(c10 * L[0] + c11 * L[3] + c12 * L[6]);
   Jw[4] = -(c10 * L[1] + c11 * L[4] + c12 * L[7]);
   Jw[5] = -(c10 * L[2] + c11 * L[5] + c12 * L[8]);
-  if (NI > 0) {
-    double col[10][2];
-    col[0][0] = ud;  col[0][1] = ar * vd;
-    col[1][0] = 0.0; col[1][1] = f * vd;
-    col[2][0] = vd;  col[2][1] = 0.0;
-    col[3][0] = 1.0; col[3][1] = 0.0;
-    col[4][0] = 0.0; col[4][1] = 1.0;
-    TBA_UNROLL
-    for (int j = 5; j < 10; ++j) {
-      col[j][0] = f * dk[j][0] + sk * dk[j][1];
-      col[j][1] = f * ar * dk[j][1];
-    }
-    TBA_UNROLL
-    for (int j = 0; j < NI; ++j) {
-      constexpr uint32_t M = IMASK;
-      const int idx = nth_bit(M, j);
-      Ji[j] = P00 * col[idx][0] + P01 * col[idx][1];
-      Ji[NI + j] = P10 * col[idx][0] + P11 * col[idx][1];
-    }
-  }
+  obs_intr_cols<IMASK>(model, u, v, k, P00, P01, P10, P11, Ji);
+  if (uv) { uv[0] = u; uv[1] = v; }
   return true;
 }
 
@@ -355,11 +400,12 @@
 __host__ __device__ inline bool linearize_obs_any(int model, const double* __restrict__ C, const double* __restrict__ rec,
                                                   const double* __restrict__ k, const double X0, const double X1, const double X2,
                                                   const double h, const double x, const double y, int loss_type, double loss_width,
-                                                  double r[2], double& rho0, double Ja[6], double Jw[6], double Jh[2], double* Ji) {
+                                                  double r[2], double& rho0, double Ja[6], double Jw[6], double Jh[2], double* Ji,
+                                                  double* uv = nullptr) {
   if (EXT) {
     if (model >= kModelFisheye) return linearize_obs_ext<IMASK>(model, C, rec, k, X0, X1, X2, h, x, y, loss_type, loss_width, r, rho0, Ja, Jw, Jh, Ji);
   }
-  return linearize_obs<IMASK>(model, C, rec, k, X0, X1, X2, h, x, y, loss_type, loss_width, r, rho0, Ja, Jw, Jh, Ji);
-}
-
-}
+  return linearize_obs<IMASK>(model, C, rec, k, X0, X1, X2, h, x, y, loss_type, loss_width, r, rho0, Ja, Jw, Jh, Ji, uv);
+}
+
+}
diff --git a/theiasfm_b200/csrc/tba_engine.cu b/theiasfm_b200/csrc/tba_engine.cu
--- a/theiasfm_b200/csrc/tba_engine.cu
+++ b/theiasfm_b200/csrc/tba_engine.cu
@@ -237,6 +237,10 @@
     case 0x061u: F(0x061u); break; \
     case 0x0E1u: F(0x0E1u); break; \
     case 0x07Fu: F(0x07Fu); break; \
+    case 0x061u | kCompactIntr: F(0x061u | kCompactIntr); break; \
+    case 0x0E1u | kCompactIntr: F(0x0E1u | kCompactIntr); break; \
+    case 0x07Fu | kCompactIntr: F(0x07Fu | kCompactIntr); break; \
+    case 0x3FFu | kCompactIntr: F(0x3FFu | kCompactIntr); break; \
     default: F(0x3FFu); break;  \
   }
 
@@ -1004,7 +1008,8 @@
   for (uint32_t m : kMasks) if ((H.union_free & ~m) == 0) { c->imask = m; break; }
   if (c->has_ext_models) c->imask = 0x3FFu;
   c->NI = popcount10(c->imask);
-  c->NJ = 14 + 2 * c->NI;
+  if (!c->has_ext_models && ng == 1 && options->loss_function_type == TBA_LOSS_TRIVIAL && c->NI >= 2) c->imask |= kCompactIntr;
+  c->NJ = nj_of(c->imask);
   const int npk = (int)H.pk2caller.size();
   const int n_long = H.n_long;
   const int n_tiles = H.n_tiles;
@@ -1921,10 +1926,26 @@
   return TBA_OK;
 }
 
+int tba_debug_intr_cols(tba_context* c, int64_t* sizes_out, double* Ji) {
+  if (!c || !c->uploaded || !sizes_out) return TBA_ERR_INVALID_ARGUMENT;
+  CUDA_OK(c, cudaSetDevice(c->device));
+  sizes_out[0] = c->n_slots; sizes_out[1] = c->NI;
+  if (!Ji || c->NI == 0 || c->n_slots == 0) return TBA_OK;
+  DevBuf<double> d;
+  CUDA_OK(c, d.alloc((size_t)c->n_slots * 2 * c->NI));
+  const int grid = (int)((c->n_slots + 255) / 256);
+#define F(M) { auto kfn = k_debug_intr_cols<M>; LAUNCH(c, kfn, grid, 256, 0, c->P, (long long)c->n_slots, d.p); }
+  DISPATCH_IMASK(c->imask, F)
+#undef F
+  CUDA_OK(c, cudaMemcpyAsync(Ji, d.p, (size_t)c->n_slots * 2 * c->NI * 8, cudaMemcpyDeviceToHost, c->stream));
+  CUDA_OK(c, cudaStreamSynchronize(c->stream));
+  return TBA_OK;
+}
+
 int tba_debug_stream_launch(tba_context* c, int32_t* out) {
   if (!c || !c->uploaded || !out) return TBA_ERR_INVALID_ARGUMENT;
   const int n_slices = c->n_normal_tiles * (TILE / 32);
-  out[0] = c->n_sm; out[1] = n_slices; out[2] = (int32_t)c->imask; out[3] = c->has_ext_models ? 1 : 0;
+  out[0] = c->n_sm; out[1] = n_slices; out[2] = (int32_t)(c->imask & ~kCompactIntr); out[3] = c->has_ext_models ? 1 : 0;
   auto put = [&](int k, int NW, int NS) { out[4 + 3 * k] = stream_grid(c, n_slices, NW); out[5 + 3 * k] = NW; out[6 + 3 * k] = NS; };
 #define F(M) { put(0, LinCfg<M>::NW, LinCfg<M>::NS); put(1, PrepCfg<M>::NW, PrepCfg<M>::NS); \
                put(2, StreamCfg<M, 0>::NW, StreamCfg<M, 0>::NS); put(3, StreamCfg<M, 1>::NW, StreamCfg<M, 1>::NS); }
diff --git a/theiasfm_b200/csrc/tba_kernels.cuh b/theiasfm_b200/csrc/tba_kernels.cuh
--- a/theiasfm_b200/csrc/tba_kernels.cuh
+++ b/theiasfm_b200/csrc/tba_kernels.cuh
@@ -15,6 +15,10 @@
 constexpr int MAXP = 256;
 constexpr int VB = 64;
 constexpr int VT = 256;
+
+constexpr uint32_t kCompactIntr = 1u << 16;
+__host__ __device__ constexpr bool compact_intr(uint32_t imask) { return (imask & kCompactIntr) != 0; }
+__host__ __device__ constexpr int nj_of(uint32_t imask) { return compact_intr(imask) ? 16 : 14 + 2 * popcount10(imask); }
 
 struct DevProblem {
   int n_cam, n_group, n_pt, n_tiles;
@@ -151,13 +155,13 @@
 }
 
 
-template <int NI, int SP, int SC>
+template <int NI, int SP, int SC, int SI = SC>
 __device__ __forceinline__ void obs_apply_F(const double* ja, const double* jw, const double* ji, double h, double2 xa, double2 xb,
                                             double2 xc, const double* xi, double& w0, double& w1) {
   w0 = -h * (ja[0] * xa.x + ja[SP] * xa.y + ja[2 * SP] * xb.x) + jw[0] * xb.y + jw[SC] * xc.x + jw[2 * SC] * xc.y;
   w1 = -h * (ja[3 * SP] * xa.x + ja[4 * SP] * xa.y + ja[5 * SP] * xb.x) + jw[3 * SC] * xb.y + jw[4 * SC] * xc.x + jw[5 * SC] * xc.y;
 #pragma unroll
-  for (int j = 0; j < NI; ++j) { w0 += ji[j * SC] * xi[j]; w1 += ji[(NI + j) * SC] * xi[j]; }
+  for (int j = 0; j < NI; ++j) { w0 += ji[j * SI] * xi[j]; w1 += ji[(NI + j) * SI] * xi[j]; }
 }
 template <int SP>
 __device__ __forceinline__ void obs_JpT(const double* ja, const double* jh, double w0, double w1, double t[4]) {
@@ -236,7 +240,7 @@
 
 template <int NI>
 __device__ __forceinline__ void obs_settle(bool ok, bool is_fixed, double rho0, double& cost, double& fixed, double& failed, double Ja[6],
-                                           double Jw[6], double Jh[2], double Ji[], double r[2]) {
+                                           double Jw[6], double Jh[2], double Ji[], double uv[2], double r[2]) {
   if (!ok) failed += 1.0;
   else if (is_fixed) fixed += 0.5 * rho0;
   else cost += 0.5 * rho0;
@@ -246,19 +250,26 @@
     Jh[0] = Jh[1] = 0.0; r[0] = r[1] = 0.0;
 #pragma unroll
     for (int j = 0; j < 2 * NI; ++j) Ji[j] = 0.0;
-  }
-}
-template <int NI>
+    uv[0] = uv[1] = nan("");
+  }
+}
+template <uint32_t IMASK>
 __device__ __forceinline__ void obs_store(double* Jt, double* rt, const double Ja[6], const double Jw[6], const double Jh[2], const double Ji[],
-                                          const double r[2]) {
+                                          const double uv[2], const double r[2]) {
+  constexpr int NI = popcount10(IMASK);
 #pragma unroll
   for (int j = 0; j < 6; ++j) Jt[j * 32] = Ja[j];
 #pragma unroll
   for (int j = 0; j < 6; ++j) Jt[(6 + j) * 32] = Jw[j];
   Jt[12 * 32] = Jh[0];
   Jt[13 * 32] = Jh[1];
-#pragma unroll
-  for (int j = 0; j < 2 * NI; ++j) Jt[(14 + j) * 32] = Ji[j];
+  if (compact_intr(IMASK)) {
+    Jt[14 * 32] = uv[0];
+    Jt[15 * 32] = uv[1];
+  } else {
+#pragma unroll
+    for (int j = 0; j < 2 * NI; ++j) Jt[(14 + j) * 32] = Ji[j];
+  }
   rt[0] = r[0];
   rt[32] = r[1];
 }
@@ -288,12 +299,21 @@
   cn = Ji[j] * Ji[j] + Ji[NI + j] * Ji[NI + j];
 }
 
+template <uint32_t IMASK>
+__device__ __forceinline__ void obs_rebuild_Ji(int model, const double* k, double u, double v, double Ji[]) {
+  constexpr int NI = popcount10(IMASK);
+  obs_intr_cols<IMASK>(model, u, v, k, 1.0, 0.0, 0.0, 1.0, Ji);
+  const bool live = u == u;
+#pragma unroll
+  for (int j = 0; j < 2 * NI; ++j) Ji[j] = live ? Ji[j] : 0.0;
+}
+
 template <uint32_t IMASK, bool EXT = false>
 __global__ void __launch_bounds__(TILE, EXT ? 1 : 3) k_linearize(DevProblem P, double* __restrict__ g_cs, double* __restrict__ cn_cs,
                                                            double* __restrict__ rep, int tile0) {
   constexpr bool STAGED_RED = !EXT;
   constexpr int NI = popcount10(IMASK);
-  constexpr int NJ = 14 + 2 * NI;
+  constexpr int NJ = nj_of(IMASK);
   __shared__ double s_acc[MAXP][14];
   const int tile = tile0 + blockIdx.x, tid = threadIdx.x, lane = tid & 31, warp = tid >> 5;
   const bool long_tile = (P.tile_flags[tile] & 1) != 0;
@@ -307,7 +327,7 @@
   const bool valid = cam >= 0;
   double cost = 0.0, fixed = 0.0, failed = 0.0;
   double Ja[6] = {0, 0, 0, 0, 0, 0}, Jw[6] = {0, 0, 0, 0, 0, 0}, Jh[2] = {0, 0}, r[2] = {0, 0};
-  double Ji[2 * NI + 1];
+  double Ji[2 * NI + 1], uv[2] = {nan(""), nan("")};
 #pragma unroll
   for (int j = 0; j < 2 * NI; ++j) Ji[j] = 0.0;
   int pl = -1 - lane, grp = 0;
@@ -325,10 +345,10 @@
     gather_camera(P.ext, P.cam_s4, cam, Cw, rec);
     const bool ok = linearize_obs_any<IMASK, EXT>(P.group_model[grp], Cw, rec,
                                          P.intr + (size_t)grp * 10, X.x, X.y, X.z, X.w, x, y, P.loss_type, P.loss_width,
-                                         r, rho0, Ja, Jw, Jh, Ji);
-    obs_settle<NI>(ok, (P.slot_flags[slot] & 1) != 0, rho0, cost, fixed, failed, Ja, Jw, Jh, Ji, r);
-  }
-  obs_store<NI>(P.J + wslice(tile, warp, NJ) + lane, P.res + wslice(tile, warp, 2) + lane, Ja, Jw, Jh, Ji, r);
+                                         r, rho0, Ja, Jw, Jh, Ji, uv);
+    obs_settle<NI>(ok, (P.slot_flags[slot] & 1) != 0, rho0, cost, fixed, failed, Ja, Jw, Jh, Ji, uv, r);
+  }
+  obs_store<IMASK>(P.J + wslice(tile, warp, NJ) + lane, P.res + wslice(tile, warp, 2) + lane, Ja, Jw, Jh, Ji, uv, r);
   {
     double acc[14];
     obs_point_terms(Ja, Jh, r, acc);
@@ -661,10 +681,11 @@
 #endif
 
 template <uint32_t IMASK, int MODE>
-__global__ void __launch_bounds__(TILE, (14 + 2 * popcount10(IMASK)) <= 20 ? 4 : 2) k_schur(DevProblem P, const double* __restrict__ xs, double* __restrict__ y,
+__global__ void __launch_bounds__(TILE, popcount10(IMASK) <= 3 ? 4 : 2) k_schur(DevProblem P, const double* __restrict__ xs, double* __restrict__ y,
                                                 double* __restrict__ rep, const int* __restrict__ done_flag, int tile0) {
   constexpr int NI = popcount10(IMASK);
-  constexpr int NJ = 14 + 2 * NI;
+  constexpr int NJ = nj_of(IMASK);
+  constexpr bool CI = compact_intr(IMASK);
   constexpr int WS = (NJ + 2) * 32;
   if (done_flag != nullptr && *done_flag) return;
 #ifdef TBA_EMULATE
@@ -711,11 +732,14 @@
   const bool head = lane == 0 || prev != pl;
   __syncthreads();
   mbar_wait(&s_bar[warp], 0);
-  const double *ja = sJ + lane, *jw = ja + 6 * 32, *jh = ja + 12 * 32, *ji = ja + 14 * 32;
+  constexpr int SI = CI ? 1 : 32;
+  double jir[2 * NI + 1];
+  if (CI) obs_rebuild_Ji<IMASK>(P.group_model[0], P.intr, sJ[14 * 32 + lane], sJ[15 * 32 + lane], jir);
+  const double *ja = sJ + lane, *jw = ja + 6 * 32, *jh = ja + 12 * 32, *ji = CI ? jir : ja + 14 * 32;
   double w0 = 0.0, w1 = 0.0, r0 = 0.0, r1 = 0.0;
   if (valid) {
     if (MODE != 0) { r0 = sR[lane]; r1 = sR[32 + lane]; }
-    if (MODE != 1) obs_apply_F<NI, 32, 32>(ja, jw, ji, h, xa, xb, xc, xi, w0, w1);
+    if (MODE != 1) obs_apply_F<NI, 32, 32, SI>(ja, jw, ji, h, xa, xb, xc, xi, w0, w1);
     if (MODE == 1) { w0 = r0; w1 = r1; }
     if (MODE == 2) { w0 = r0 - w0; w1 = r1 - w1; }
   }
@@ -752,7 +776,7 @@
   } else {
     double yv[6], yi[NI + 1];
     obs_JcT<32, 32>(ja, jw, h, z0, z1, yv);
-    obs_JiT<NI, 32>(ji, z0, z1, yi);
+    obs_JiT<NI, SI>(ji, z0, z1, yi);
 #pragma unroll
     for (int j = 0; j < 6; ++j) yv[j] = valid ? yv[j] : 0.0;
 #pragma unroll
@@ -849,11 +873,12 @@
 template <uint32_t IMASK, int MODE>
 struct StreamCfg {
   static constexpr int NI = popcount10(IMASK);
-  static constexpr int NJ = 14 + 2 * NI;
+  static constexpr int NJ = nj_of(IMASK);
   static constexpr int STG = NJ * 32 + (MODE != 0 ? 64 : 0) + 32;
   static constexpr int NS = 3;
-  static constexpr int NW = (220 * 1024 / (NS * STG * 8)) > 12 ? 12 : (220 * 1024 / (NS * STG * 8));
-  static constexpr size_t SMEM = (size_t)NW * NS * STG * 8 + (size_t)NW * NS * 8;
+  static constexpr int NWMAX = compact_intr(IMASK) && NI > 3 ? 8 : 12;
+  static constexpr int NW = (220 * 1024 / (NS * STG * 8)) > NWMAX ? NWMAX : (220 * 1024 / (NS * STG * 8));
+  static constexpr size_t SMEM = (size_t)NW * NS * STG * 8 + (size_t)NW * NS * 8 + (compact_intr(IMASK) ? (size_t)NW * 10 * 8 : 0);
 };
 
 template <uint32_t IMASK, int MODE>
@@ -862,6 +887,7 @@
                const int* __restrict__ done_flag, int n_slices, P2pDev pp) {
   using Cfg = StreamCfg<IMASK, MODE>;
   constexpr int NI = Cfg::NI, NJ = Cfg::NJ, STG = Cfg::STG, NS = Cfg::NS, NW = Cfg::NW;
+  constexpr bool CI = compact_intr(IMASK);
   if (done_flag != nullptr && *done_flag) return;
 #ifdef TBA_EMULATE
   double* s_dyn = emu::dyn_smem<double>();
@@ -874,6 +900,7 @@
   const bool active = s_begin < s_end;
   double* ring = s_dyn + (size_t)warp * NS * STG;
   uint64_t* bars = reinterpret_cast<uint64_t*>(s_dyn + (size_t)NW * NS * STG) + warp * NS;
+  double* s_k = s_dyn + (size_t)NW * NS * STG + (size_t)NW * NS + warp * 10;
   constexpr uint32_t jbytes = NJ * 32 * 8, rbytes = (MODE != 0) ? 2 * 32 * 8 : 0;
   auto issue = [&](int stage, int slice) {
     double* st = ring + (size_t)stage * STG;
@@ -890,6 +917,9 @@
 #pragma unroll
     for (int k = 0; k < NS; ++k) if (s_begin + k < s_end) issue(k, s_begin + k);
   }
+  __syncwarp();
+  const int model0 = CI ? P.group_model[0] : 0;
+  if (CI && lane < 10) s_k[lane] = P.intr[lane];
   __syncwarp();
   double xi_u[NI + 1];
   if (NI > 0 && MODE != 1 && P.single_group) {
@@ -954,7 +984,10 @@
     const int stage = it % NS;
     double* sJ = ring + (size_t)stage * STG;
     const double* sR = sJ + NJ * 32;
-    const double *jw = sJ + lane + 6 * 32, *ji = sJ + lane + 14 * 32;
+    constexpr int SI = CI ? 1 : 32;
+    double jir[2 * NI + 1];
+    if (CI) obs_rebuild_Ji<IMASK>(model0, s_k, sJ[14 * 32 + lane], sJ[15 * 32 + lane], jir);
+    const double *jw = sJ + lane + 6 * 32, *ji = CI ? jir : sJ + lane + 14 * 32;
     double w0 = 0.0, w1 = 0.0, r0 = 0.0, r1 = 0.0;
     double ja[6], jh[2];
 #pragma unroll
@@ -962,7 +995,7 @@
     jh[0] = sJ[12 * 32 + lane]; jh[1] = sJ[13 * 32 + lane];
     if (valid) {
       if (MODE != 0) { r0 = sR[lane]; r1 = sR[32 + lane]; }
-      if (MODE != 1) obs_apply_F<NI, 1, 32>(ja, jw, ji, h, xa, xb, xc, xi, w0, w1);
+      if (MODE != 1) obs_apply_F<NI, 1, 32, SI>(ja, jw, ji, h, xa, xb, xc, xi, w0, w1);
       if (MODE == 1) { w0 = r0; w1 = r1; }
       if (MODE == 2) { w0 = r0 - w0; w1 = r1 - w1; }
     }
@@ -994,7 +1027,7 @@
     } else {
       double yv[6], yi[NI + 1];
       obs_JcT<1, 32>(ja, jw, h, z0, z1, yv);
-      obs_JiT<NI, 32>(ji, z0, z1, yi);
+      obs_JiT<NI, SI>(ji, z0, z1, yi);
 #pragma unroll
       for (int j = 0; j < 6; ++j) yv[j] = valid ? yv[j] : 0.0;
 #pragma unroll
@@ -1005,11 +1038,11 @@
       __syncwarp();
       if (!(MODE == 0 && (P.ablate & 1))) warp_red_rows<6>(y, sJ, sbase, lane);
       if (NI > 0) {
-        if (P.single_group) {
+        if (CI || P.single_group) {
 #pragma unroll
           for (int j = 0; j < NI; ++j) yi_acc[j] += yi[j];
         } else {
-          static_assert(32 * 6 + 16 + 32 * NI + 16 <= NJ * 32, "stage too small for the intrinsics staging");
+          static_assert(CI || 32 * 6 + 16 + 32 * NI + 16 <= NJ * 32, "stage too small for the intrinsics staging");
           double* si = sJ + 32 * 6 + 16;
           int* sibase = reinterpret_cast<int*>(si + 32 * NI);
           __syncwarp();
@@ -1083,13 +1116,14 @@
 template <uint32_t IMASK>
 struct PrepCfg {
   static constexpr int NI = popcount10(IMASK);
-  static constexpr int NJ = 14 + 2 * NI;
+  static constexpr int NJ = nj_of(IMASK);
   static constexpr int NSI = NI * (NI + 1) / 2;
   static constexpr int STG = NJ * 32 + 64 + 32;
   static constexpr int NS = 3;
-  static constexpr int NWMAX = NI <= 4 ? 10 : 6;
+  static constexpr int NWMAX = NI <= (compact_intr(IMASK) ? 3 : 4) ? 10 : 6;
   static constexpr int NW = (216 * 1024 / (NS * STG * 8)) > NWMAX ? NWMAX : (216 * 1024 / (NS * STG * 8));
-  static constexpr size_t SMEM = (size_t)NW * NS * STG * 8 + (size_t)NW * NS * 8 + (size_t)NW * (NSI + 1) * 8;
+  static constexpr size_t SMEM = (size_t)NW * NS * STG * 8 + (size_t)NW * NS * 8 + (size_t)NW * (NSI + 1) * 8 +
+                                 (compact_intr(IMASK) ? (size_t)NW * 10 * 8 : 0);
 };
 
 template <uint32_t IMASK>
@@ -1097,6 +1131,7 @@
 k_prepare_stream(DevProblem P, double* __restrict__ y, double* __restrict__ Sc, double* __restrict__ Si, double* __restrict__ rep, int n_slices) {
   using Cfg = PrepCfg<IMASK>;
   constexpr int NI = Cfg::NI, NJ = Cfg::NJ, STG = Cfg::STG, NS = Cfg::NS, NW = Cfg::NW, NSI = Cfg::NSI;
+  constexpr bool CI = compact_intr(IMASK);
 #ifdef TBA_EMULATE
   double* s_dyn = emu::dyn_smem<double>();
 #else
@@ -1108,6 +1143,7 @@
   double* ring = s_dyn + (size_t)warp * NS * STG;
   uint64_t* bars = reinterpret_cast<uint64_t*>(s_dyn + (size_t)NW * NS * STG) + warp * NS;
   double* s_si = s_dyn + (size_t)NW * NS * STG + (size_t)NW * NS;
+  double* s_k = s_si + (size_t)NW * (NSI + 1) + warp * 10;
   constexpr uint32_t jbytes = NJ * 32 * 8, rbytes = 2 * 32 * 8;
   auto issue = [&](int stage, int slice) {
     double* st = ring + (size_t)stage * STG;
@@ -1124,6 +1160,9 @@
 #pragma unroll
     for (int k = 0; k < NS; ++k) if (s_begin + k < s_end) issue(k, s_begin + k);
   }
+  __syncwarp();
+  const int model0 = CI ? P.group_model[0] : 0;
+  if (CI && lane < 10) s_k[lane] = P.intr[lane];
   __syncwarp();
   double yi_acc[NI + 1], si_acc[NSI + 1];
 #pragma unroll
@@ -1171,8 +1210,12 @@
 #pragma unroll
     for (int j = 0; j < 6; ++j) { ja[j] = Jt[j * 32]; jw[j] = Jt[(6 + j) * 32]; }
     jh[0] = Jt[12 * 32]; jh[1] = Jt[13 * 32];
-#pragma unroll
-    for (int j = 0; j < 2 * NI; ++j) ji[j] = Jt[(14 + j) * 32];
+    if (CI) {
+      obs_rebuild_Ji<IMASK>(model0, s_k, Jt[14 * 32], Jt[15 * 32], ji);
+    } else {
+#pragma unroll
+      for (int j = 0; j < 2 * NI; ++j) ji[j] = Jt[(14 + j) * 32];
+    }
     double r0 = 0.0, r1 = 0.0;
     if (valid) { r0 = sR[lane]; r1 = sR[32 + lane]; }
     if (!valid) {
@@ -1287,7 +1330,7 @@
 template <uint32_t IMASK>
 struct LinCfg {
   static constexpr int NI = popcount10(IMASK);
-  static constexpr int NJ = 14 + 2 * NI;
+  static constexpr int NJ = nj_of(IMASK);
   static constexpr int STG = 64 + 16 + 16 + 4;
   static constexpr int RSTG = 2 * 32 * 6 + 16;
   static constexpr int NS = 4;
@@ -1365,7 +1408,7 @@
     const int stage = it % NS;
     const double* st = ring + (size_t)stage * STG;
     double Ja[6] = {0, 0, 0, 0, 0, 0}, Jw[6] = {0, 0, 0, 0, 0, 0}, Jh[2] = {0, 0}, r[2] = {0, 0};
-    double Ji[2 * NI + 1];
+    double Ji[2 * NI + 1], uv[2] = {nan(""), nan("")};
 #pragma unroll
     for (int j = 0; j < 2 * NI; ++j) Ji[j] = 0.0;
     if (valid) {
@@ -1382,11 +1425,11 @@
 #endif
       double rho0 = 0.0;
       const bool ok = linearize_obs_any<IMASK, false>(P.group_model[grp], Cw, rec, P.intr + (size_t)grp * 10, X01.x, X01.y, X23.x,
-                                                      X23.y, st[lane], st[32 + lane], P.loss_type, P.loss_width, r, rho0, Ja, Jw, Jh, Ji);
+                                                      X23.y, st[lane], st[32 + lane], P.loss_type, P.loss_width, r, rho0, Ja, Jw, Jh, Ji, uv);
       obs_settle<NI>(ok, (reinterpret_cast<const uint8_t*>(st + 96)[lane] & 1) != 0, rho0, cost_acc, fixed_acc, failed_acc, Ja, Jw, Jh,
-                     Ji, r);
-    }
-    obs_store<NI>(P.J + (size_t)s * NJ * 32 + lane, P.res + (size_t)s * 64 + lane, Ja, Jw, Jh, Ji, r);
+                     Ji, uv, r);
+    }
+    obs_store<IMASK>(P.J + (size_t)s * NJ * 32 + lane, P.res + (size_t)s * 64 + lane, Ja, Jw, Jh, Ji, uv, r);
     {
       double acc[14];
       obs_point_terms(Ja, Jh, r, acc);
@@ -1456,8 +1499,7 @@
 
 template <uint32_t IMASK>
 __global__ void __launch_bounds__(TILE) k_precond_ext(DevProblem P, double* __restrict__ Sc, int tile0) {
-  constexpr int NI = popcount10(IMASK);
-  constexpr int NJ = 14 + 2 * NI;
+  constexpr int NJ = nj_of(IMASK);
   const int tile = tile0 + blockIdx.x, tid = threadIdx.x, lane = tid & 31, warp = tid >> 5;
   const size_t slot = (size_t)tile * TILE + tid;
   const int cam = P.slot_cam[slot];
@@ -1486,7 +1528,7 @@
 template <uint32_t IMASK>
 __global__ void __launch_bounds__(TILE) k_precond_intr(DevProblem P, double* __restrict__ Si, int tile0) {
   constexpr int NI = popcount10(IMASK);
-  constexpr int NJ = 14 + 2 * NI;
+  constexpr int NJ = nj_of(IMASK);
   constexpr int NW = 4 * NI;
   constexpr int NS = NI * (NI + 1) / 2;
 #ifdef TBA_EMULATE
@@ -1515,8 +1557,12 @@
     for (int j = 0; j < 3; ++j) { jp0[j] = Jt[j * 32]; jp1[j] = Jt[(3 + j) * 32]; }
     jp0[3] = Jt[12 * 32];
     jp1[3] = Jt[13 * 32];
-#pragma unroll
-    for (int j = 0; j < 2 * NI; ++j) Ji[j] = Jt[(14 + j) * 32];
+    if (compact_intr(IMASK)) {
+      obs_rebuild_Ji<IMASK>(P.group_model[0], P.intr, Jt[14 * 32], Jt[15 * 32], Ji);
+    } else {
+#pragma unroll
+      for (int j = 0; j < 2 * NI; ++j) Ji[j] = Jt[(14 + j) * 32];
+    }
     grp = P.cam_group[cam];
     const int run = P.slot_run[slot];
     if (run >= 0) {
@@ -1555,6 +1601,25 @@
       }
       ++n;
     }
+}
+
+template <uint32_t IMASK>
+__global__ void k_debug_intr_cols(DevProblem P, long long n_slots, double* __restrict__ out) {
+  constexpr int NI = popcount10(IMASK), NJ = nj_of(IMASK);
+  const long long s = (long long)blockIdx.x * blockDim.x + threadIdx.x;
+  if (s >= n_slots) return;
+  const long long slice = s >> 5;
+  const int lane = (int)(s & 31);
+  const double* Jt = P.J + (size_t)slice * NJ * 32 + lane;
+  double Ji[2 * NI + 1];
+  if (compact_intr(IMASK)) {
+    obs_rebuild_Ji<IMASK>(P.group_model[0], P.intr, Jt[14 * 32], Jt[15 * 32], Ji);
+  } else {
+#pragma unroll
+    for (int j = 0; j < 2 * NI; ++j) Ji[j] = Jt[(14 + j) * 32];
+  }
+#pragma unroll
+  for (int j = 0; j < 2 * NI; ++j) out[((size_t)slice * 2 * NI + j) * 32 + lane] = Ji[j];
 }
 
 template <int N>
diff --git a/theiasfm_b200/engine.py b/theiasfm_b200/engine.py
--- a/theiasfm_b200/engine.py
+++ b/theiasfm_b200/engine.py
@@ -12,7 +12,7 @@
 EXPORTED_SYMBOLS = [
     "tba_options_init", "tba_device_count", "tba_create", "tba_destroy", "tba_nccl_unique_id", "tba_last_error",
     "tba_solve", "tba_upload", "tba_minimize", "tba_download", "tba_shard_points", "tba_debug_linearize", "tba_debug_linearize_raw",
-    "tba_debug_stream_launch",
+    "tba_debug_stream_launch", "tba_debug_intr_cols",
     "tba_debug_prepare_linear_system", "tba_debug_schur_matvec", "tba_debug_solve_linear_system",
     "tba_debug_evaluate_step", "tba_debug_read", "tba_reset_parameters", "tba_set_max_iterations", "tba_set_profiling", "tba_get_profile", "tba_get_profile_stages", "tba_solve_multi", "tba_debug_pack", "tba_filter_tracks", "tba_adjust_tracks", "tba_adjust_views", "tba_estimate_tracks", "tba_two_view_ba_batch", "tba_two_view_ba_batch_multi",
 ]
@@ -47,6 +47,7 @@
         L.tba_debug_linearize.argtypes = [C.c_void_p, dp]
         L.tba_debug_linearize_raw.argtypes = [C.c_void_p, C.c_int, C.POINTER(C.c_int64), dp, dp, dp, dp, dp]
         L.tba_debug_stream_launch.argtypes = [C.c_void_p, C.POINTER(C.c_int32)]
+        L.tba_debug_intr_cols.argtypes = [C.c_void_p, C.POINTER(C.c_int64), dp]
         L.tba_debug_prepare_linear_system.argtypes = [C.c_void_p, C.c_double]
         L.tba_debug_schur_matvec.argtypes = [C.c_void_p, dp, dp, dp, dp]
         L.tba_debug_solve_linear_system.argtypes = [C.c_void_p, C.POINTER(C.c_int32), dp]
@@ -316,6 +317,14 @@
         return dict(J=J, res=res, Hpp=Hpp, gp=gp, g=lin[:ncs], cn=lin[ncs:2 * ncs], cost=lin[2 * ncs], fixed=lin[2 * ncs + 1],
                     failed=lin[2 * ncs + 2])
 
+    def intr_cols_raw(self):
+        sizes = np.zeros(2, np.int64)
+        self._check(lib().tba_debug_intr_cols(self._h, sizes.ctypes.data_as(C.POINTER(C.c_int64)), None))
+        n_slots, ni = (int(v) for v in sizes)
+        Ji = np.zeros((n_slots // 32, 2 * ni, 32))
+        self._check(lib().tba_debug_intr_cols(self._h, sizes.ctypes.data_as(C.POINTER(C.c_int64)), _dp(Ji)))
+        return Ji
+
     STREAM_KERNELS = ("linearize", "prepare", "matvec", "rhs_backsub")
 
     def stream_launch(self):
```

After: 718.8 million, median of 6. 1.1x the previous value.
